# batra-mlp-lab/visdial

Measured on NVIDIA H100. Metric: QA-rounds/sec mn-att-ques-im-hist+disc train step, higher is better.
Workload: dtype f16 operands + f16 saved state for the option LSTM, tf32 operands elsewhere; fp32 accumulate, fp32 cell state / gradients / optimiser

## Files before the change

include/visdial_b200.h:

```cpp
#ifndef VISDIAL_B200_H
#define VISDIAL_B200_H

#include <stddef.h>
#include <stdint.h>

#ifdef __cplusplus
extern "C" {
#endif

#define VD_OK 0
#define VD_E_BADARG (-1)
#define VD_E_SHAPE (-2)
#define VD_E_CUDA (-3)
#define VD_E_COMM (-4)
#define VD_E_OOM (-5)
#define VD_E_STATE (-6)

typedef struct vd_engine vd_engine;

typedef struct vd_params {
  const char* encoder;
  const char* decoder;
  int32_t vocabSize;
  int32_t embedSize;
  int32_t rnnHiddenSize;
  int32_t numLayers;
  int32_t imgFeatureSize;
  int32_t imgSpatialSize;
  int32_t imgEmbedSize;
  int32_t commonEmbeddingSize;
  int32_t numAttentionLayers;
  int32_t maxQuesCount;
  int32_t numOptions;
  float dropout;
  int32_t gpuid;
} vd_params;

typedef struct vd_batch {
  int32_t B;
  int32_t Tq, Th, Ta, To;
  const int32_t* ques_fwd;
  const int32_t* hist;
  const float* img_feat;
  const int32_t* options;
  const int32_t* answer_ind;
  const int32_t* answer_in;
  const int32_t* answer_out;
  const int32_t* option_in;
  const int32_t* option_out;
  int32_t on_device;
} vd_batch;

#define VD_INIT_EMBED 0
#define VD_INIT_LINEAR_W 1
#define VD_INIT_LINEAR_B 2
#define VD_INIT_LSTM_W 3
#define VD_INIT_LSTM_B 4
int vd_layout_count(const vd_params* p, int32_t* n_segments, int64_t* n_params);
int vd_layout_segment(const vd_params* p, int32_t idx, char* name, int32_t name_cap,
                      int64_t* offset, int64_t* rows, int64_t* cols, int32_t* init_kind,
                      int64_t* fan_in);

int vd_create(const vd_params* p, vd_engine** out);
int vd_destroy(vd_engine* e);
const char* vd_last_error(void);

int vd_num_params(vd_engine* e, int64_t* n);
int vd_param_buffers(vd_engine* e, float** W_dev, float** dW_dev);
int vd_optim_buffers(vd_engine* e, float** m_dev, float** v_dev, int64_t* t);
int vd_set_optim_state(vd_engine* e, const float* m_host, const float* v_host, int64_t t);
int vd_set_parameters(vd_engine* e, const float* host_src, int64_t n);
int vd_get_parameters(vd_engine* e, float* host_dst, int64_t n);
int vd_get_gradients(vd_engine* e, float* host_dst, int64_t n);
int vd_zero_grad(vd_engine* e);

int vd_set_training(vd_engine* e, int32_t training);
int vd_set_dropout_seed(vd_engine* e, uint64_t seed, uint64_t iteration);
#define VD_MATH_TF32 0
#define VD_MATH_FP32 1
#define VD_MATH_F16 2
int vd_set_math_mode(vd_engine* e, int32_t mode);
int vd_set_lazy_decout(vd_engine* e, int32_t on);
int vd_set_option_overlap(vd_engine* e, int32_t on, int32_t reserve_sms);

int vd_encoder_forward(vd_engine* e, const vd_batch* b, const float** encOut_dev);
int vd_forward_connect(vd_engine* e);
int vd_decoder_forward(vd_engine* e, const vd_batch* b, const float** decOut_dev);
int vd_criterion_forward(vd_engine* e, const vd_batch* b, float* loss_host);
int vd_criterion_backward(vd_engine* e, const vd_batch* b);
int vd_decoder_backward(vd_engine* e, const vd_batch* b);
int vd_backward_connect(vd_engine* e, const float** gradEncOut_dev);
int vd_encoder_backward(vd_engine* e, const vd_batch* b, const float* gradEncOut_dev);

int vd_forward_backward(vd_engine* e, const vd_batch* b, int32_t only_forward, float* loss_host);
int vd_forward_backward_dense(vd_engine* e, const vd_batch* b, const int32_t* round_host, const float* relevance_host,
                              float* loss_host);
int vd_retrieve(vd_engine* e, const vd_batch* b, int32_t use_gt, int32_t* ranks_host);
int vd_compute_ranks(vd_engine* e, const float* scores_dev, int32_t n_rows,
                     const int32_t* gt_dev_or_null, int32_t* ranks_dev);
int vd_gen_option_lhood(vd_engine* e, const vd_batch* b, const float** lhood_dev);
int vd_encoder_rnn_state(vd_engine* e, int32_t level, const float** h_last_dev, const float** c_last_dev);
int vd_gen_decoder_step(vd_engine* e, int32_t rows, const int32_t* tokens_host, const float* const* h_prev,
                        const float* const* c_prev, const float** logp_dev, const float** h_out, const float** c_out);
int vd_gen_beam_step(vd_engine* e, int32_t rows, const int32_t* tokens_host, const int32_t* parent_host,
                     const float* const* init_h_host, const float* const* init_c_host, int32_t k, float* topv_host,
                     int32_t* topi_host);
int vd_gen_beam_search(vd_engine* e, int32_t beam_size, int32_t beam_len, int32_t start_token, int32_t end_token,
                       int32_t* answer_host, int32_t* length_host, double* score_host);
int vd_gen_sample(vd_engine* e, int32_t beam_len, int32_t start_token, float temperature, uint64_t seed, int64_t row_offset,
                  int32_t* answer_host, float* logp_host);

int vd_clamp_adam_step(vd_engine* e, float learning_rate);

#define VD_COMM_ID_BYTES 128
int vd_comm_unique_id(void* id_out);
int vd_comm_init(vd_engine* e, const void* id, int32_t rank, int32_t world);
int vd_comm_allreduce_grads(vd_engine* e);

int vd_memcpy_d2h(vd_engine* e, void* host_dst, const void* dev_src, size_t bytes);
int vd_memcpy_h2d(vd_engine* e, void* dev_dst, const void* host_src, size_t bytes);
int vd_host_alloc(void** ptr, size_t bytes);
int vd_host_free(void* ptr);
int vd_device_alloc(vd_engine* e, void** ptr, size_t bytes);
int vd_device_free(vd_engine* e, void* ptr);
int vd_synchronize(vd_engine* e);
int vd_stream(vd_engine* e, void** cuda_stream);
int vd_timer_start(vd_engine* e);
int vd_timer_stop(vd_engine* e, float* ms);
int vd_profile_enable(vd_engine* e, int32_t on);
int vd_profile_reset(vd_engine* e);
int vd_launch_count(vd_engine* e, int64_t* n_launches);
int vd_kernel_stats(vd_engine* e, const char* name, int64_t* launches, double* total_ms,
                    double* total_flops, double* total_bytes);
int vd_gemm_tn(vd_engine* e, int32_t M, int32_t N, int32_t K, const float* A, int64_t lda, const float* B, int64_t ldb,
               float* C, int64_t ldc, float beta, const float* bias, int32_t act);
int vd_gemm_atb(vd_engine* e, int32_t M, int32_t N, int64_t K, const float* A, int64_t lda, const float* B, int64_t ldb,
                float* C, int64_t ldc);
int vd_gemm_atb16(vd_engine* e, int32_t M, int32_t N, int64_t K, const float* A, int64_t lda, const float* B, int64_t ldb,
                  float* C, int64_t ldc, float inv_scale);
int vd_lstm_step_fwd(vd_engine* e, int64_t R, int32_t H, const float* h_prev, const float* WhT, int64_t ldw, const float* bias,
                     float* gates, int32_t has_xproj, const float* ptable, int64_t ptable_rows, const int32_t* tok,
                     const float* c_prev, float* c_out, float* h_out, const int32_t* mask_ids, int32_t* path);
int vd_lstm_step_bwd(vd_engine* e, int64_t R, int32_t H, const float* da_next, const float* Wh, const float* gates,
                     const float* c_prev, const float* c_cur, const float* dh_ext, float* dc_carry, const int32_t* mask_ids,
                     float* da, int32_t* path);
int vd_lstm16_step_fwd(vd_engine* e, int64_t R, int32_t H, const void* h_prev16, const void* Wh16, const void* ptable16,
                       const int32_t* tok, const float* bias, const float* c_prev, const int32_t* mask_ids, void* gates16,
                       float* c_out, void* h16_out, float* h32_out);
int vd_lstm16_step_bwd(vd_engine* e, int64_t R, int32_t H, const void* da_next16, const void* Whb16, const void* gates16,
                       const float* c_prev, const float* c_cur, float* dc_carry, const int32_t* mask_ids, void* da16);
int vd_profiler_range(vd_engine* e, int32_t start);
int vd_flush_l2(vd_engine* e);

typedef struct vd_corpus vd_corpus;

typedef struct vd_corpus_desc {
  int32_t numThreads;
  int32_t numRounds;
  int32_t maxQuesLen;
  int32_t maxAnsLen;
  int32_t maxCapLen;
  int32_t numOptions;
  int32_t numOptList;
  int32_t numImages;
  int32_t useHistory;
  int32_t concatHistory;
  int32_t useIm;
  int32_t maxHistoryLen;
  int32_t imgNorm;
  int32_t imgAtt;
  int32_t imgChannels;
  int32_t imgSpatial;
  int32_t startToken, endToken;
  const int32_t* ques;
  const int32_t* ques_len;
  const int32_t* ans;
  const int32_t* ans_len;
  const int32_t* cap;
  const int32_t* cap_len;
  const int32_t* opt;
  const int32_t* opt_list;
  const int32_t* opt_len;
  const int32_t* ans_index;
  const int32_t* img_pos;
  const int32_t* num_rounds;
  const float* images;
} vd_corpus_desc;

int vd_corpus_create(vd_engine* e, const vd_corpus_desc* d, vd_corpus** out);
int vd_corpus_destroy(vd_corpus* c);
int vd_corpus_get_batch(vd_corpus* c, const int64_t* inds, int32_t n, int32_t decoder_gen, vd_batch* out);
int vd_corpus_read(vd_corpus* c, const char* name, void* host_dst, int64_t* elems);
int vd_corpus_batch_bytes(vd_corpus* c, int64_t* bytes, int32_t* launches);

#ifdef __cplusplus
}
#endif
#endif
```

visdial_b200/_lib.py:

```python
from __future__ import annotations

import ctypes as C
import os

_HERE = os.path.dirname(os.path.abspath(__file__))
LIB_PATH = os.path.join(_HERE, "lib", "libvisdial_b200.so")

VD_OK = 0
VD_E_BADARG = -1
VD_E_STATE = -6
VD_MATH_TF32 = 0
VD_MATH_FP32 = 1
VD_MATH_F16 = 2
VD_COMM_ID_BYTES = 128
INIT_EMBED, INIT_LINEAR_W, INIT_LINEAR_B, INIT_LSTM_W, INIT_LSTM_B = range(5)


class VdError(RuntimeError):
    def __init__(self, code, msg):
        super().__init__("visdial_b200 error %d: %s" % (code, msg))
        self.code = code


class vd_params(C.Structure):
    _fields_ = [
        ("encoder", C.c_char_p), ("decoder", C.c_char_p),
        ("vocabSize", C.c_int32), ("embedSize", C.c_int32), ("rnnHiddenSize", C.c_int32),
        ("numLayers", C.c_int32), ("imgFeatureSize", C.c_int32), ("imgSpatialSize", C.c_int32),
        ("imgEmbedSize", C.c_int32), ("commonEmbeddingSize", C.c_int32),
        ("numAttentionLayers", C.c_int32), ("maxQuesCount", C.c_int32), ("numOptions", C.c_int32),
        ("dropout", C.c_float), ("gpuid", C.c_int32),
    ]


class vd_batch(C.Structure):
    _fields_ = [
        ("B", C.c_int32), ("Tq", C.c_int32), ("Th", C.c_int32), ("Ta", C.c_int32), ("To", C.c_int32),
        ("ques_fwd", C.c_void_p), ("hist", C.c_void_p), ("img_feat", C.c_void_p),
        ("options", C.c_void_p), ("answer_ind", C.c_void_p), ("answer_in", C.c_void_p),
        ("answer_out", C.c_void_p), ("option_in", C.c_void_p), ("option_out", C.c_void_p),
        ("on_device", C.c_int32),
    ]


class vd_corpus_desc(C.Structure):
    _fields_ = ([(k, C.c_int32) for k in (
        "numThreads", "numRounds", "maxQuesLen", "maxAnsLen", "maxCapLen", "numOptions", "numOptList", "numImages",
        "useHistory", "concatHistory", "useIm", "maxHistoryLen", "imgNorm", "imgAtt", "imgChannels", "imgSpatial",
        "startToken", "endToken")] +
        [(k, C.c_void_p) for k in (
            "ques", "ques_len", "ans", "ans_len", "cap", "cap_len", "opt", "opt_list", "opt_len", "ans_index",
            "img_pos", "num_rounds", "images")])


_P = C.POINTER
_H = C.c_void_p

SIGNATURES = {
    "vd_layout_count": [_P(vd_params), _P(C.c_int32), _P(C.c_int64)],
    "vd_layout_segment": [_P(vd_params), C.c_int32, C.c_char_p, C.c_int32, _P(C.c_int64), _P(C.c_int64),
                          _P(C.c_int64), _P(C.c_int32), _P(C.c_int64)],
    "vd_create": [_P(vd_params), _P(_H)],
    "vd_destroy": [_H],
    "vd_num_params": [_H, _P(C.c_int64)],
    "vd_param_buffers": [_H, _P(C.c_void_p), _P(C.c_void_p)],
    "vd_optim_buffers": [_H, _P(C.c_void_p), _P(C.c_void_p), _P(C.c_int64)],
    "vd_set_optim_state": [_H, C.c_void_p, C.c_void_p, C.c_int64],
    "vd_set_parameters": [_H, C.c_void_p, C.c_int64],
    "vd_get_parameters": [_H, C.c_void_p, C.c_int64],
    "vd_get_gradients": [_H, C.c_void_p, C.c_int64],
    "vd_zero_grad": [_H],
    "vd_set_training": [_H, C.c_int32],
    "vd_set_dropout_seed": [_H, C.c_uint64, C.c_uint64],
    "vd_set_math_mode": [_H, C.c_int32],
    "vd_set_option_overlap": [_H, C.c_int32, C.c_int32],
    "vd_encoder_forward": [_H, _P(vd_batch), _P(C.c_void_p)],
    "vd_forward_connect": [_H],
    "vd_decoder_forward": [_H, _P(vd_batch), _P(C.c_void_p)],
    "vd_criterion_forward": [_H, _P(vd_batch), _P(C.c_float)],
    "vd_criterion_backward": [_H, _P(vd_batch)],
    "vd_decoder_backward": [_H, _P(vd_batch)],
    "vd_backward_connect": [_H, _P(C.c_void_p)],
    "vd_encoder_backward": [_H, _P(vd_batch), C.c_void_p],
    "vd_forward_backward": [_H, _P(vd_batch), C.c_int32, _P(C.c_float)],
    "vd_forward_backward_dense": [_H, _P(vd_batch), C.c_void_p, C.c_void_p, _P(C.c_float)],
    "vd_retrieve": [_H, _P(vd_batch), C.c_int32, C.c_void_p],
    "vd_compute_ranks": [_H, C.c_void_p, C.c_int32, C.c_void_p, C.c_void_p],
    "vd_gen_option_lhood": [_H, _P(vd_batch), _P(C.c_void_p)],
    "vd_encoder_rnn_state": [_H, C.c_int32, _P(C.c_void_p), _P(C.c_void_p)],
    "vd_gen_decoder_step": [_H, C.c_int32, C.c_void_p, _P(C.c_void_p), _P(C.c_void_p), _P(C.c_void_p), _P(C.c_void_p),
                            _P(C.c_void_p)],
    "vd_clamp_adam_step": [_H, C.c_float],
    "vd_comm_unique_id": [C.c_void_p],
    "vd_comm_init": [_H, C.c_void_p, C.c_int32, C.c_int32],
    "vd_comm_allreduce_grads": [_H],
    "vd_memcpy_d2h": [_H, C.c_void_p, C.c_void_p, C.c_size_t],
    "vd_memcpy_h2d": [_H, C.c_void_p, C.c_void_p, C.c_size_t],
    "vd_host_alloc": [_P(C.c_void_p), C.c_size_t],
    "vd_host_free": [C.c_void_p],
    "vd_device_alloc": [_H, _P(C.c_void_p), C.c_size_t],
    "vd_device_free": [_H, C.c_void_p],
    "vd_synchronize": [_H],
    "vd_stream": [_H, _P(C.c_void_p)],
    "vd_timer_start": [_H],
    "vd_timer_stop": [_H, _P(C.c_float)],
    "vd_profile_enable": [_H, C.c_int32],
    "vd_profile_reset": [_H],
    "vd_launch_count": [_H, _P(C.c_int64)],
    "vd_kernel_stats": [_H, C.c_char_p, _P(C.c_int64), _P(C.c_double), _P(C.c_double), _P(C.c_double)],
    "vd_gemm_tn": [_H, C.c_int32, C.c_int32, C.c_int32, C.c_void_p, C.c_int64, C.c_void_p, C.c_int64, C.c_void_p,
                   C.c_int64, C.c_float, C.c_void_p, C.c_int32],
    "vd_gemm_atb": [_H, C.c_int32, C.c_int32, C.c_int64, C.c_void_p, C.c_int64, C.c_void_p, C.c_int64, C.c_void_p,
                    C.c_int64],
    "vd_set_lazy_decout": [_H, C.c_int32],
    "vd_gen_beam_step": [_H, C.c_int32, C.c_void_p, C.c_void_p, C.c_void_p, C.c_void_p, C.c_int32, C.c_void_p, C.c_void_p],
    "vd_gen_beam_search": [_H, C.c_int32, C.c_int32, C.c_int32, C.c_int32, C.c_void_p, C.c_void_p, C.c_void_p],
    "vd_gen_sample": [_H, C.c_int32, C.c_int32, C.c_float, C.c_uint64, C.c_int64, C.c_void_p, C.c_void_p],
    "vd_gemm_atb16": [_H, C.c_int32, C.c_int32, C.c_int64, C.c_void_p, C.c_int64, C.c_void_p, C.c_int64, C.c_void_p,
                      C.c_int64, C.c_float],
    "vd_lstm_step_fwd": [_H, C.c_int64, C.c_int32, C.c_void_p, C.c_void_p, C.c_int64, C.c_void_p, C.c_void_p, C.c_int32,
                         C.c_void_p, C.c_int64, C.c_void_p, C.c_void_p, C.c_void_p, C.c_void_p, C.c_void_p, _P(C.c_int32)],
    "vd_lstm_step_bwd": [_H, C.c_int64, C.c_int32, C.c_void_p, C.c_void_p, C.c_void_p, C.c_void_p, C.c_void_p, C.c_void_p,
                         C.c_void_p, C.c_void_p, C.c_void_p, _P(C.c_int32)],
    "vd_lstm16_step_fwd": [_H, C.c_int64, C.c_int32] + [C.c_void_p] * 11,
    "vd_lstm16_step_bwd": [_H, C.c_int64, C.c_int32] + [C.c_void_p] * 8,
    "vd_profiler_range": [_H, C.c_int32],
    "vd_flush_l2": [_H],
    "vd_corpus_create": [_H, _P(vd_corpus_desc), _P(C.c_void_p)],
    "vd_corpus_destroy": [C.c_void_p],
    "vd_corpus_get_batch": [C.c_void_p, C.c_void_p, C.c_int32, C.c_int32, _P(vd_batch)],
    "vd_corpus_read": [C.c_void_p, C.c_char_p, C.c_void_p, _P(C.c_int64)],
    "vd_corpus_batch_bytes": [C.c_void_p, _P(C.c_int64), _P(C.c_int32)],
}

_lib = None


def load() -> C.CDLL:
    global _lib
    if _lib is not None:
        return _lib
    if not os.path.exists(LIB_PATH):
        raise VdError(-3, "%s not found: build it with `python __graft_entry__.py` "
                          "(there is no CPU fallback)" % LIB_PATH)
    lib = C.CDLL(LIB_PATH)
    for name, argtypes in SIGNATURES.items():
        fn = getattr(lib, name)
        fn.argtypes = argtypes
        fn.restype = C.c_int
    lib.vd_last_error.argtypes = []
    lib.vd_last_error.restype = C.c_char_p
    _lib = lib
    return lib


def check(rc: int):
    if rc != VD_OK:
        raise VdError(rc, load().vd_last_error().decode("utf-8", "replace"))
```

visdial_b200/csrc/api.cu:

```cuda
#include "engine.h"
#include <string.h>
#include <cuda_profiler_api.h>

namespace vd {
void comm_unique_id(void* out);
void comm_init(Engine* e, const void* idbytes, int rank, int world);
void comm_destroy(Engine* e);
struct Corpus;
Corpus* corpus_create(Engine* eng, const vd_corpus_desc* d);
void corpus_destroy(Corpus* c);
void corpus_get_batch(Corpus* c, const int64_t* inds, int n, int decoder_gen, vd_batch* out);
void corpus_read(Corpus* c, const char* name, void* host_dst, int64_t* elems);
void corpus_batch_bytes(Corpus* c, int64_t* bytes, int32_t* launches);
}

using vd::Engine;

static thread_local char g_err[1024] = "";

static int fail(int code, const char* msg) {
  snprintf(g_err, sizeof(g_err), "%s", msg);
  return code;
}

// ... 3 lines not shown
    return VD_OK;                                               \
  } catch (const vd::CudaError& ex) {                           \
    return fail(ex.code, ex.what());                            \
  } catch (const std::exception& ex) {                          \
    return fail(VD_E_CUDA, ex.what());                          \
  } catch (...) {                                               \
    return fail(VD_E_CUDA, "unknown error");                    \
  }

struct vd_engine { Engine* e; };
#define ENG(h) ((h) ? (h)->e : (throw vd::CudaError(VD_E_BADARG, "engine handle is null"), (Engine*)nullptr))
#define NOTNULL(p) VD_REQUIRE((p) != nullptr, VD_E_BADARG, "null output pointer")

extern "C" {

const char* vd_last_error(void) { return g_err; }

int vd_layout_count(const vd_params* p, int32_t* n_segments, int64_t* n_params) {
  VD_TRY({
    vd::Layout l = vd::build_layout(vd::parse_cfg(p));
    if (n_segments) *n_segments = (int32_t)l.segs.size();
    if (n_params) *n_params = l.total;
  })
}

int vd_layout_segment(const vd_params* p, int32_t idx, char* name, int32_t name_cap, int64_t* offset, int64_t* rows,
                      int64_t* cols, int32_t* init_kind, int64_t* fan_in) {
  VD_TRY({
    vd::Layout l = vd::build_layout(vd::parse_cfg(p));
    VD_REQUIRE(idx >= 0 && idx < (int)l.segs.size(), VD_E_BADARG, "segment index out of range");
    const vd::Seg& s = l.segs[idx];
    if (name && name_cap > 0) snprintf(name, name_cap, "%s", s.name.c_str());
    if (offset) *offset = s.off;
    if (rows) *rows = s.rows;
    if (cols) *cols = s.cols;
    if (init_kind) *init_kind = s.init;
    if (fan_in) *fan_in = s.fan_in;
  })
}

int vd_create(const vd_params* p, vd_engine** out) {
  VD_TRY({
    NOTNULL(out);
    *out = nullptr;
    Engine* e = new Engine(p);
    vd_engine* h = new vd_engine;
    h->e = e;
    *out = h;
  })
}

int vd_destroy(vd_engine* h) {
  VD_TRY({
    if (h) { vd::comm_destroy(h->e); delete h->e; delete h; }
  })
}

int vd_num_params(vd_engine* h, int64_t* n) { VD_TRY({ NOTNULL(n); *n = ENG(h)->nparams; }) }
int vd_param_buffers(vd_engine* h, float** W, float** dW) {
  VD_TRY({ Engine* e = ENG(h); if (W) *W = e->W; if (dW) *dW = e->dW; })
}
int vd_optim_buffers(vd_engine* h, float** m, float** v, int64_t* t) {
  VD_TRY({ Engine* e = ENG(h); if (m) *m = e->m; if (v) *v = e->v; if (t) *t = e->adam_t; })
}
int vd_set_optim_state(vd_engine* h, const float* m_host, const float* v_host, int64_t t) {
  VD_TRY({
    Engine* e = ENG(h);
    VD_REQUIRE(m_host && v_host && t >= 0, VD_E_BADARG, "vd_set_optim_state: m / v null or t < 0");
    VD_CUDA_CHECK(cudaSetDevice(e->cfg.gpuid));
    const size_t bytes = (size_t)e->nparams * sizeof(float);
    VD_CUDA_CHECK(cudaMemcpyAsync(e->m, m_host, bytes, cudaMemcpyHostToDevice, e->cx.stream));
    VD_CUDA_CHECK(cudaMemcpyAsync(e->v, v_host, bytes, cudaMemcpyHostToDevice, e->cx.stream));
    VD_CUDA_CHECK(cudaStreamSynchronize(e->cx.stream));
    e->adam_t = t;
  })
}
int vd_set_parameters(vd_engine* h, const float* src, int64_t n) {
  VD_TRY({
    Engine* e = ENG(h);
    VD_REQUIRE(src && n == e->nparams, VD_E_SHAPE, "vd_set_parameters: n must equal vd_num_params");
    VD_CUDA_CHECK(cudaSetDevice(e->cfg.gpuid));
    VD_CUDA_CHECK(cudaMemcpyAsync(e->W, src, (size_t)n * sizeof(float), cudaMemcpyHostToDevice, e->cx.stream));
    VD_CUDA_CHECK(cudaStreamSynchronize(e->cx.stream));
  })
}
static void copy_out(Engine* e, float* dst, const float* src, int64_t n) {
  VD_REQUIRE(dst && n == e->nparams, VD_E_SHAPE, "n must equal vd_num_params");
  VD_CUDA_CHECK(cudaSetDevice(e->cfg.gpuid));
  e->join_options_backward();
  if (src == e->dW && e->world > 1) {
    bool any = false;
    for (char c : e->seg_reduced) any = any || c;
    if (any) e->reduce_remaining();
  }
  VD_CUDA_CHECK(cudaMemcpyAsync(dst, src, (size_t)n * sizeof(float), cudaMemcpyDeviceToHost, e->cx.stream));
  VD_CUDA_CHECK(cudaStreamSynchronize(e->cx.stream));
}
int vd_get_parameters(vd_engine* h, float* dst, int64_t n) { VD_TRY({ Engine* e = ENG(h); copy_out(e, dst, e->W, n); }) }
int vd_get_gradients(vd_engine* h, float* dst, int64_t n) { VD_TRY({ Engine* e = ENG(h); copy_out(e, dst, e->dW, n); }) }
int vd_zero_grad(vd_engine* h) {
  VD_TRY({
    Engine* e = ENG(h);
    VD_CUDA_CHECK(cudaSetDevice(e->cfg.gpuid));
    e->join_options_backward();
    if (e->comm_pending) e->reduce_remaining();
    VD_CUDA_CHECK(cudaMemsetAsync(e->dW, 0, (size_t)e->nparams * sizeof(float), e->cx.stream));
    e->arm_grad_sync();
  })
}

int vd_set_training(vd_engine* h, int32_t training) {
  VD_TRY({ VD_REQUIRE(training >= 0 && training <= 2, VD_E_BADARG, "training must be 0, 1 or 2"); ENG(h)->training = training; })
}
int vd_set_dropout_seed(vd_engine* h, uint64_t seed, uint64_t iteration) {
  VD_TRY({ Engine* e = ENG(h); e->drop_seed = seed; e->drop_iter = iteration; })
}
int vd_set_option_overlap(vd_engine* h, int32_t on, int32_t reserve_sms) {
  VD_TRY({
    Engine* e = ENG(h);
    e->join_options_backward();
    if (e->opt_fwd_pending) { VD_CUDA_CHECK(cudaStreamSynchronize(e->opt_stream)); e->opt_fwd_pending = false; }
    e->opt_overlap = on != 0;
    if (reserve_sms >= 0) {
      VD_REQUIRE(reserve_sms <= e->cx.sm_count - 16, VD_E_BADARG, "reserve_sms leaves fewer than 16 SMs to the option stream");
      e->opt_reserve_sms = reserve_sms & ~1;
    }
  })
}
int vd_set_math_mode(vd_engine* h, int32_t mode) {
  VD_TRY({ VD_REQUIRE(mode == VD_MATH_TF32 || mode == VD_MATH_FP32 || mode == VD_MATH_F16, VD_E_BADARG, "unknown math mode"); ENG(h)->math_mode = mode; })
}

int vd_encoder_forward(vd_engine* h, const vd_batch* b, const float** encOut) {
  VD_TRY({ Engine* e = ENG(h); e->encoder_forward(b); if (encOut) *encOut = e->encOut; })
}
int vd_forward_connect(vd_engine* h) { VD_TRY({ ENG(h)->forward_connect(); }) }
int vd_decoder_forward(vd_engine* h, const vd_batch* b, const float** decOut) {
  VD_TRY({
    (void)b;
    Engine* e = ENG(h);
    e->decoder_forward();
    if (decOut) *decOut = e->cfg.dec == vd::DEC_DISC ? e->scores : e->logp;
  })
}
int vd_set_lazy_decout(vd_engine* h, int32_t on) { VD_TRY({ ENG(h)->want_logp = on == 0; }) }
int vd_criterion_forward(vd_engine* h, const vd_batch* b, float* loss) {
  VD_TRY({ (void)b; NOTNULL(loss); *loss = ENG(h)->criterion_forward(); })
}
int vd_criterion_backward(vd_engine* h, const vd_batch* b) { VD_TRY({ (void)b; ENG(h)->criterion_backward(); }) }
int vd_decoder_backward(vd_engine* h, const vd_batch* b) { VD_TRY({ (void)b; ENG(h)->decoder_backward(); }) }
int vd_backward_connect(vd_engine* h, const float** gradEncOut) {
  VD_TRY({ const float* g = ENG(h)->backward_connect(); if (gradEncOut) *gradEncOut = g; })
}
int vd_encoder_backward(vd_engine* h, const vd_batch* b, const float* gradEncOut) {
  VD_TRY({ (void)b; ENG(h)->encoder_backward(gradEncOut); })
}

int vd_forward_backward(vd_engine* h, const vd_batch* b, int32_t only_forward, float* loss) {
  VD_TRY({
    Engine* e = ENG(h);
    e->encoder_forward(b);
    e->forward_connect();
    const bool saved_want = e->want_logp;
    e->want_logp = false;
    try { e->decoder_forward(); } catch (...) { e->want_logp = saved_want; throw; }
    e->want_logp = saved_want;
    float l = e->criterion_forward();
    if (loss) *loss = l;
    if (!only_forward) {
      e->criterion_backward();
      e->decoder_backward();
      const float* g = e->backward_connect();
      e->encoder_backward(g);
    }
  })
}

int vd_forward_backward_dense(vd_engine* h, const vd_batch* b, const int32_t* round_host, const float* relevance_host,
                              float* loss_host) {
  VD_TRY({
    const float l = ENG(h)->forward_backward_dense(b, round_host, relevance_host);
    if (loss_host) *loss_host = l;
  })
}

int vd_retrieve(vd_engine* h, const vd_batch* b, int32_t use_gt, int32_t* ranks_host) {
  VD_TRY({ ENG(h)->retrieve(b, use_gt, ranks_host); })
}
int vd_compute_ranks(vd_engine* h, const float* scores_dev, int32_t n_rows, const int32_t* gt_dev, int32_t* ranks_dev) {
  VD_TRY({
    Engine* e = ENG(h);
    VD_REQUIRE(scores_dev && ranks_dev && n_rows >= 0, VD_E_BADARG, "null scores / ranks");
    vd::rank_rows(e->cx, scores_dev, gt_dev, ranks_dev, n_rows, e->cfg.K);
  })
}
int vd_gen_option_lhood(vd_engine* h, const vd_batch* b, const float** lhood_dev) {
  VD_TRY({ (void)b; Engine* e = ENG(h); e->gen_option_lhood(); if (lhood_dev) *lhood_dev = e->lhood; })
}

int vd_encoder_rnn_state(vd_engine* h, int32_t level, const float** h_last, const float** c_last) {
  VD_TRY({
    Engine* e = ENG(h);
    VD_REQUIRE(e->have_fwd, VD_E_STATE, "vd_encoder_rnn_state before vd_encoder_forward");
    VD_REQUIRE(level == 0 || level == 1, VD_E_BADARG, "level must be 0 or 1");
    const bool has_layers = e->cfg.rnn_layers;
    const vd::LstmRun& r = level == 0 ? e->ques1 : e->ques2;
    if (h_last) *h_last = has_layers ? r.h_last() : nullptr;
    if (c_last) *c_last = has_layers ? r.c_last() : nullptr;
  })
}
int vd_gen_decoder_step(vd_engine* h, int32_t rows, const int32_t* tokens_host, const float* const* h_prev,
                        const float* const* c_prev, const float** logp_dev, const float** h_out, const float** c_out) {
  VD_TRY({
    Engine* e = ENG(h);
    e->gen_decoder_step(rows, tokens_host, h_prev, c_prev);
    if (logp_dev) *logp_dev = e->gstep_logp;
    if (h_out) { h_out[0] = e->gstep1.h; h_out[1] = e->gstep2.h; }
    if (c_out) { c_out[0] = e->gstep1.c; c_out[1] = e->gstep2.c; }
  })
}

int vd_gen_beam_step(vd_engine* h, int32_t rows, const int32_t* tokens_host, const int32_t* parent_host,
                     const float* const* init_h_host, const float* const* init_c_host, int32_t k, float* topv_host,
                     int32_t* topi_host) {
  VD_TRY({ ENG(h)->gen_beam_step(rows, tokens_host, parent_host, init_h_host, init_c_host, k, topv_host, topi_host); })
}

int vd_gen_beam_search(vd_engine* h, int32_t beam_size, int32_t beam_len, int32_t start_token, int32_t end_token,
                       int32_t* answer_host, int32_t* length_host, double* score_host) {
  VD_TRY({ ENG(h)->gen_beam_search(beam_size, beam_len, start_token, end_token, answer_host, length_host, score_host); })
}

int vd_gen_sample(vd_engine* h, int32_t beam_len, int32_t start_token, float temperature, uint64_t seed, int64_t row_offset,
                  int32_t* answer_host, float* logp_host) {
  VD_TRY({ ENG(h)->gen_sample(beam_len, start_token, temperature, seed, row_offset, answer_host, logp_host); })
}

int vd_clamp_adam_step(vd_engine* h, float lr) { VD_TRY({ ENG(h)->clamp_adam_step(lr); }) }

int vd_comm_unique_id(void* id_out) { VD_TRY({ NOTNULL(id_out); vd::comm_unique_id(id_out); }) }
int vd_comm_init(vd_engine* h, const void* id, int32_t rank, int32_t world) {
  VD_TRY({ VD_REQUIRE(id != nullptr || world == 1, VD_E_BADARG, "id is null"); vd::comm_init(ENG(h), id, rank, world); })
}
int vd_comm_allreduce_grads(vd_engine* h) { VD_TRY({ ENG(h)->allreduce_grads(); }) }

int vd_memcpy_d2h(vd_engine* h, void* dst, const void* src, size_t bytes) {
  VD_TRY({
    Engine* e = ENG(h);
    VD_REQUIRE(dst && src, VD_E_BADARG, "null pointer");
    VD_CUDA_CHECK(cudaSetDevice(e->cfg.gpuid));
    VD_CUDA_CHECK(cudaMemcpyAsync(dst, src, bytes, cudaMemcpyDeviceToHost, e->cx.stream));
    VD_CUDA_CHECK(cudaStreamSynchronize(e->cx.stream));
  })
}
int vd_memcpy_h2d(vd_engine* h, void* dst, const void* src, size_t bytes) {
  VD_TRY({
    Engine* e = ENG(h);
    VD_REQUIRE(dst && src, VD_E_BADARG, "null pointer");
    VD_CUDA_CHECK(cudaSetDevice(e->cfg.gpuid));
    VD_CUDA_CHECK(cudaMemcpyAsync(dst, src, bytes, cudaMemcpyHostToDevice, e->cx.stream));
    VD_CUDA_CHECK(cudaStreamSynchronize(e->cx.stream));
  })
}
int vd_host_alloc(void** ptr, size_t bytes) {
  VD_TRY({ NOTNULL(ptr); *ptr = nullptr; VD_CUDA_CHECK(cudaHostAlloc(ptr, bytes ? bytes : 1, cudaHostAllocDefault)); })
}
int vd_host_free(void* ptr) { VD_TRY({ if (ptr) VD_CUDA_CHECK(cudaFreeHost(ptr)); }) }
int vd_device_alloc(vd_engine* h, void** ptr, size_t bytes) {
  VD_TRY({
    Engine* e = ENG(h);
    NOTNULL(ptr);
    *ptr = nullptr;
    VD_CUDA_CHECK(cudaSetDevice(e->cfg.gpuid));
    VD_CUDA_CHECK(cudaMalloc(ptr, bytes ? bytes : 1));
  })
}
int vd_device_free(vd_engine* h, void* ptr) {
  VD_TRY({ Engine* e = ENG(h); VD_CUDA_CHECK(cudaSetDevice(e->cfg.gpuid)); if (ptr) VD_CUDA_CHECK(cudaFree(ptr)); })
}
int vd_synchronize(vd_engine* h) {
  VD_TRY({
    Engine* e = ENG(h);
    e->join_options_backward();
    VD_CUDA_CHECK(cudaStreamSynchronize(e->cx.stream));
    if (e->opt_fwd_pending) VD_CUDA_CHECK(cudaStreamSynchronize(e->opt_stream));
  })
}
int vd_stream(vd_engine* h, void** s) { VD_TRY({ NOTNULL(s); *s = (void*)ENG(h)->cx.stream; }) }
int vd_timer_start(vd_engine* h) { VD_TRY({ Engine* e = ENG(h); VD_CUDA_CHECK(cudaEventRecord(e->t0, e->cx.stream)); }) }
int vd_timer_stop(vd_engine* h, float* ms) {
  VD_TRY({
    Engine* e = ENG(h);
    NOTNULL(ms);
    VD_CUDA_CHECK(cudaEventRecord(e->t1, e->cx.stream));
    VD_CUDA_CHECK(cudaEventSynchronize(e->t1));
    VD_CUDA_CHECK(cudaEventElapsedTime(ms, e->t0, e->t1));
  })
}
int vd_profile_enable(vd_engine* h, int32_t on) { VD_TRY({ ENG(h)->cx.profiling = on; }) }
int vd_profile_reset(vd_engine* h) {
  VD_TRY({ Engine* e = ENG(h); e->cx.collect(); e->cx.stats.clear(); e->cx.launches = 0; })
}
int vd_launch_count(vd_engine* h, int64_t* n) { VD_TRY({ NOTNULL(n); *n = ENG(h)->cx.launches; }) }
int vd_kernel_stats(vd_engine* h, const char* name, int64_t* launches, double* total_ms, double* total_flops,
                    double* total_bytes) {
  VD_TRY({
    Engine* e = ENG(h);
    VD_REQUIRE(name != nullptr, VD_E_BADARG, "name is null");
    e->cx.collect();
    auto it = e->cx.stats.find(name);
    vd::KStat z;
    const vd::KStat& s = it == e->cx.stats.end() ? z : it->second;
    if (launches) *launches = s.launches;
    if (total_ms) *total_ms = s.ms;
    if (total_flops) *total_flops = s.flops;
    if (total_bytes) *total_bytes = s.bytes;
  })
}
int vd_gemm_tn(vd_engine* h, int32_t M, int32_t N, int32_t K, const float* A, int64_t lda, const float* B, int64_t ldb,
               float* C, int64_t ldc, float beta, const float* bias, int32_t act) {
  VD_TRY({
    Engine* e = ENG(h);
    VD_REQUIRE(A && B && C, VD_E_BADARG, "null operand");
    VD_CUDA_CHECK(cudaSetDevice(e->cfg.gpuid));
    e->gemm_tn(M, N, K, A, lda, nullptr, B, ldb, C, ldc, beta, bias, act);
  })
}
int vd_gemm_atb(vd_engine* h, int32_t M, int32_t N, int64_t K, const float* A, int64_t lda, const float* B, int64_t ldb,
                float* C, int64_t ldc) {
  VD_TRY({
    Engine* e = ENG(h);
    VD_REQUIRE(A && B && C, VD_E_BADARG, "null operand");
    VD_CUDA_CHECK(cudaSetDevice(e->cfg.gpuid));
    e->gemm_atb(M, N, K, A, lda, nullptr, B, ldb, C, ldc);
  })
}
int vd_gemm_atb16(vd_engine* h, int32_t M, int32_t N, int64_t K, const float* A, int64_t lda, const float* B, int64_t ldb,
                  float* C, int64_t ldc, float inv_scale) {
  VD_TRY({
    Engine* e = ENG(h);
    VD_REQUIRE(A && B && C, VD_E_BADARG, "null operand");
    VD_CUDA_CHECK(cudaSetDevice(e->cfg.gpuid));
    __half* A16 = nullptr; __half* B16 = nullptr; float* sc = nullptr;
    VD_CUDA_CHECK(cudaMalloc((void**)&A16, (size_t)K * M * sizeof(__half)));
    VD_CUDA_CHECK(cudaMalloc((void**)&B16, (size_t)K * N * sizeof(__half)));
    VD_CUDA_CHECK(cudaMalloc((void**)&sc, sizeof(float)));
    VD_CUDA_CHECK(cudaMemcpyAsync(sc, &inv_scale, sizeof(float), cudaMemcpyHostToDevice, e->cx.stream));
    cvt_f32_to_f16(e->cx, A16, M, A, lda, K, M);
    cvt_f32_to_f16(e->cx, B16, N, B, ldb, K, N);
    gemm_atb16(e->cx, M, N, K, A16, M, B16, N, C, ldc, sc);
    VD_CUDA_CHECK(cudaStreamSynchronize(e->cx.stream));
    cudaFree(A16); cudaFree(B16); cudaFree(sc);
  })
}
int vd_lstm_step_fwd(vd_engine* h, int64_t R, int32_t H, const float* h_prev, const float* WhT, int64_t ldw, const float* bias,
                     float* gates, int32_t has_xproj, const float* ptable, int64_t ptable_rows, const int32_t* tok,
                     const float* c_prev, float* c_out, float* h_out, const int32_t* mask_ids, int32_t* path) {
  VD_TRY({
    Engine* e = ENG(h);
    NOTNULL(path);
    VD_REQUIRE(R >= 1 && H > 0 && H % 4 == 0 && WhT && bias && gates && c_out && h_out, VD_E_BADARG, "vd_lstm_step_fwd: arguments");
    VD_REQUIRE((has_xproj != 0) != (ptable != nullptr) && (!ptable || (tok && ptable_rows > 0)), VD_E_BADARG,
               "vd_lstm_step_fwd: the x side is either a dense projection (has_xproj) or a table gather (ptable + tok)");
    VD_CUDA_CHECK(cudaSetDevice(e->cfg.gpuid));
    *path = 0;
    const vd::LstmRoute rt = e->route_lstm(R, H, ptable != nullptr, false, WhT, ldw, nullptr);
    VD_REQUIRE(rt.fwd != vd::LstmPath::Opt16, VD_E_BADARG, "vd_lstm_step_fwd: the fp16 option-LSTM steps (lstm16.cu) have no test hook");
    VD_REQUIRE(rt.fwd == vd::LstmPath::Tc || !ptable, VD_E_BADARG, "vd_lstm_step_fwd: a table gather runs on the tensor-core route only");
    vd::LstmFwdStep s;
    s.R = R; s.H = H; s.WhT = WhT; s.ldw = ldw; s.bias = bias;
    s.h_prev = h_prev; s.c_prev = c_prev; s.gates = gates; s.mask = mask_ids; s.c_out = c_out; s.h_out = h_out;
    float* pt = nullptr;
    if (rt.fwd == vd::LstmPath::Tc) {
      const int64_t n = (ptable ? ptable_rows : R) * 4 * H;
      VD_CUDA_CHECK(cudaMalloc((void**)&pt, (size_t)n * sizeof(float)));
      vd::repeat_rows(e->cx, pt, bias, 1, (int)(n / (4 * H)), 4 * H);
      vd::add_inplace(e->cx, ptable ? pt : gates, ptable ? ptable : pt, n);
      if (ptable) { s.ptable = pt; s.tok = tok; }
    }
    if (rt.fwd == vd::LstmPath::Tc) *path = e->lstm_tc_fwd_step(s); else e->lstm_simt_fwd_step(s);
    VD_CUDA_CHECK(cudaStreamSynchronize(e->cx.stream));
    if (pt) cudaFree(pt);
  })
}

int vd_lstm_step_bwd(vd_engine* h, int64_t R, int32_t H, const float* da_next, const float* Wh, const float* gates,
                     const float* c_prev, const float* c_cur, const float* dh_ext, float* dc_carry, const int32_t* mask_ids,
                     float* da, int32_t* path) {
  VD_TRY({
    Engine* e = ENG(h);
    NOTNULL(path);
    VD_REQUIRE(R >= 1 && H > 0 && Wh && gates && c_cur && dc_carry && da, VD_E_BADARG, "vd_lstm_step_bwd: arguments");
    VD_CUDA_CHECK(cudaSetDevice(e->cfg.gpuid));
    *path = 0;
    const vd::LstmRoute rt = e->route_lstm(R, H, false, false, nullptr, H, Wh);
    vd::LstmBwdStep s;
    s.R = R; s.H = H; s.Wh = Wh; s.da_next = da_next; s.dh_ext = dh_ext;
    s.gates = gates; s.c_prev = c_prev; s.c_cur = c_cur; s.mask = mask_ids; s.dc_carry = dc_carry; s.da = da;
    if (rt.bwd == vd::LstmPath::Simt && da_next) VD_CUDA_CHECK(cudaMalloc((void**)&s.dh_rec, (size_t)R * H * sizeof(float)));
    if (rt.bwd == vd::LstmPath::Tc) *path = e->lstm_tc_bwd_step(s); else e->lstm_simt_bwd_step(s);
    VD_CUDA_CHECK(cudaStreamSynchronize(e->cx.stream));
    if (s.dh_rec) cudaFree(s.dh_rec);
  })
}
int vd_lstm16_step_fwd(vd_engine* h, int64_t R, int32_t H, const void* h_prev16, const void* Wh16, const void* ptable16,
                       const int32_t* tok, const float* bias, const float* c_prev, const int32_t* mask_ids, void* gates16,
                       float* c_out, void* h16_out, float* h32_out) {
  VD_TRY({
    Engine* e = ENG(h);
    VD_REQUIRE(h_prev16 && Wh16 && ptable16 && tok && bias && c_out && h16_out, VD_E_BADARG, "vd_lstm16_step_fwd: arguments");
    VD_REQUIRE(vd::lstm16_shape_ok(R, H), VD_E_BADARG, "vd_lstm16_step_fwd: shape");
    VD_CUDA_CHECK(cudaSetDevice(e->cfg.gpuid));
    vd::lstm16_step_fwd(e->cx, R, H, (const __half*)h_prev16, (const __half*)Wh16, (const __half*)ptable16, tok, bias, c_prev,
                        mask_ids, (__half*)gates16, c_out, (__half*)h16_out, h32_out);
    VD_CUDA_CHECK(cudaStreamSynchronize(e->cx.stream));
  })
}
int vd_lstm16_step_bwd(vd_engine* h, int64_t R, int32_t H, const void* da_next16, const void* Whb16, const void* gates16,
                       const float* c_prev, const float* c_cur, float* dc_carry, const int32_t* mask_ids, void* da16) {
  VD_TRY({
    Engine* e = ENG(h);
    VD_REQUIRE(da_next16 && Whb16 && gates16 && c_cur && dc_carry && da16, VD_E_BADARG, "vd_lstm16_step_bwd: arguments");
    VD_REQUIRE(vd::lstm16_shape_ok(R, H), VD_E_BADARG, "vd_lstm16_step_bwd: shape");
    VD_CUDA_CHECK(cudaSetDevice(e->cfg.gpuid));
    vd::lstm16_step_bwd(e->cx, R, H, (const __half*)da_next16, (const __half*)Whb16, (const __half*)gates16, c_prev, c_cur,
                        dc_carry, mask_ids, (__half*)da16);
    VD_CUDA_CHECK(cudaStreamSynchronize(e->cx.stream));
  })
}

int vd_profiler_range(vd_engine* h, int32_t start) {
  VD_TRY({
    Engine* e = ENG(h);
    VD_CUDA_CHECK(cudaStreamSynchronize(e->cx.stream));
    if (start) VD_CUDA_CHECK(cudaProfilerStart()); else VD_CUDA_CHECK(cudaProfilerStop());
  })
}
int vd_flush_l2(vd_engine* h) {
  VD_TRY({
    Engine* e = ENG(h);
    if (!e->flush_buf) {
      e->flush_n = (int64_t)(192u << 20) / 4;
      VD_CUDA_CHECK(cudaMalloc((void**)&e->flush_buf, (size_t)e->flush_n * 4));
    }
    vd::fill_l2_flush(e->cx, e->flush_buf, e->flush_n);
  })
}

struct vd_corpus { vd::Corpus* c; };
#define CORP(h) ((h) ? (h)->c : (throw vd::CudaError(VD_E_BADARG, "corpus handle is null"), (vd::Corpus*)nullptr))

int vd_corpus_create(vd_engine* h, const vd_corpus_desc* d, vd_corpus** out) {
  VD_TRY({
    NOTNULL(out);
    Engine* e = ENG(h);
    VD_CUDA_CHECK(cudaSetDevice(e->cfg.gpuid));
    vd::Corpus* c = vd::corpus_create(e, d);
    *out = new vd_corpus{c};
  })
}
int vd_corpus_destroy(vd_corpus* h) {
  VD_TRY({
    if (h) { vd::corpus_destroy(h->c); delete h; }
  })
}
int vd_corpus_get_batch(vd_corpus* h, const int64_t* inds, int32_t n, int32_t decoder_gen, vd_batch* out) {
  VD_TRY({ vd::corpus_get_batch(CORP(h), inds, n, decoder_gen, out); })
}
int vd_corpus_read(vd_corpus* h, const char* name, void* host_dst, int64_t* elems) {
  VD_TRY({ vd::corpus_read(CORP(h), name, host_dst, elems); })
}
int vd_corpus_batch_bytes(vd_corpus* h, int64_t* bytes, int32_t* launches) {
  VD_TRY({ vd::corpus_batch_bytes(CORP(h), bytes, launches); })
}

}
```

visdial_b200/csrc/common.cuh:

```cuda
#pragma once
#include <cuda_runtime.h>
#include <stdint.h>
#include <stdio.h>
#include <string.h>
#include <string>
#include <stdexcept>
#include <vector>
#include <map>

namespace vd {

struct CudaError : std::runtime_error {
  int code;
  CudaError(int c, const std::string& m) : std::runtime_error(m), code(c) {}
};

#define VD_CUDA_CHECK(expr)                                                              \
  do {                                                                                   \
    cudaError_t _e = (expr);                                                             \
    if (_e != cudaSuccess) {                                                             \
      char _buf[512];                                                                    \
      snprintf(_buf, sizeof(_buf), "%s:%d: %s -> %s", __FILE__, __LINE__, #expr,         \
               cudaGetErrorString(_e));                                                  \
      throw vd::CudaError(_e == cudaErrorMemoryAllocation ? -5 : -3, _buf);              \
    }                                                                                    \
  } while (0)

#define VD_REQUIRE(cond, code, msg)                                                      \
  do {                                                                                   \
    if (!(cond)) {                                                                       \
      char _buf[512];                                                                    \
      snprintf(_buf, sizeof(_buf), "%s:%d: %s (%s)", __FILE__, __LINE__, msg, #cond);    \
      throw vd::CudaError(code, _buf);                                                   \
    }                                                                                    \
  } while (0)

struct DropCfg {
  uint32_t seed_lo, seed_hi, iter, thresh;
  float scale;
};

__host__ __device__ __forceinline__ void philox4x32_10(uint32_t c0, uint32_t c1, uint32_t c2,
                                                       uint32_t c3, uint32_t k0, uint32_t k1,
                                                       uint32_t out[4]) {
  const uint32_t M0 = 0xD2511F53u, M1 = 0xCD9E8D57u, W0 = 0x9E3779B9u, W1 = 0xBB67AE85u;
#pragma unroll
  for (int r = 0; r < 10; ++r) {
    uint64_t p0 = (uint64_t)M0 * c0, p1 = (uint64_t)M1 * c2;
    uint32_t hi0 = (uint32_t)(p0 >> 32), lo0 = (uint32_t)p0;
    uint32_t hi1 = (uint32_t)(p1 >> 32), lo1 = (uint32_t)p1;
    uint32_t n0 = hi1 ^ c1 ^ k0, n1 = lo1, n2 = hi0 ^ c3 ^ k1, n3 = lo0;
    c0 = n0; c1 = n1; c2 = n2; c3 = n3;
    k0 += W0; k1 += W1;
  }
  out[0] = c0; out[1] = c1; out[2] = c2; out[3] = c3;
}

__device__ __forceinline__ float drop_factor(const DropCfg& d, uint32_t site, uint64_t idx) {
  if (d.thresh == 0) return 1.f;
  uint64_t q = idx >> 2;
  uint32_t o[4];
  philox4x32_10((uint32_t)q, (uint32_t)(q >> 32), site, d.iter, d.seed_lo, d.seed_hi, o);
  return o[idx & 3] >= d.thresh ? d.scale : 0.f;
}
__device__ __forceinline__ void drop_factor4(const DropCfg& d, uint32_t site, uint64_t idx4, float f[4]) {
  if (d.thresh == 0) { f[0] = f[1] = f[2] = f[3] = 1.f; return; }
  uint32_t o[4];
  philox4x32_10((uint32_t)idx4, (uint32_t)(idx4 >> 32), site, d.iter, d.seed_lo, d.seed_hi, o);
#pragma unroll
  for (int i = 0; i < 4; ++i) f[i] = o[i] >= d.thresh ? d.scale : 0.f;
}

enum : uint32_t {
  SITE_QEMBED = 0, SITE_HEMBED = 1, SITE_HATT = 2, SITE_IMG_TR = 3, SITE_U_OUT = 5,
  SITE_FUSION = 6, SITE_IMG_FC7 = 7, SITE_HOP0 = 16,
  SITE_SAMPLE = 64
};

struct SampleCfg {
  uint32_t seed_lo, seed_hi, step;
  float temperature;
  int64_t row_offset;
};
constexpr float GUMBEL_MAX = 17.5f;

__device__ __forceinline__ float gumbel_of_word(uint32_t w) {
  const uint32_t m = w >> 8;
  const float t = m < (1u << 23) ? -logf(((float)m + 0.5f) * 0x1p-24f)
                                 : -log1pf(-(((float)((1u << 24) - m) - 0.5f) * 0x1p-24f));
  return -logf(t);
}
__device__ __forceinline__ void sample_words(const SampleCfg& s, uint64_t q, uint32_t o[4]) {
  philox4x32_10((uint32_t)q, (uint32_t)(q >> 32), SITE_SAMPLE, s.step, s.seed_lo, s.seed_hi, o);
}
__device__ __forceinline__ bool sample_before(float k, int c, float k2, int c2) { return k > k2 || (k == k2 && c < c2); }

struct KStat {
  int64_t launches = 0;
  double flops = 0, bytes = 0;
  std::vector<std::pair<cudaEvent_t, cudaEvent_t>> pending;
  double ms = 0;
};

struct LaunchCtx {
  cudaStream_t stream = nullptr;
  int64_t launches = 0;
  int profiling = 0;
  int sm_count = 132;
  int sm_budget = 0;
  int sms() const { return sm_budget > 0 ? sm_budget : sm_count; }
  std::map<std::string, KStat> stats;
  std::vector<cudaEvent_t> free_events;

  cudaEvent_t get_event() {
    if (!free_events.empty()) { cudaEvent_t e = free_events.back(); free_events.pop_back(); return e; }
    cudaEvent_t e; VD_CUDA_CHECK(cudaEventCreate(&e)); return e;
  }
  struct Scope {
    LaunchCtx* cx; KStat* st; cudaEvent_t a = nullptr, b = nullptr;
    Scope(LaunchCtx* c, const char* name, double flops, double bytes) : cx(c), st(nullptr) {
      if (!cx->profiling) return;
      if (cx->profiling == 2 && strcmp(name, "lstm_step") != 0 && strcmp(name, "lstm_step_bwd") != 0) return;
      st = &cx->stats[name];
      st->launches++; st->flops += flops; st->bytes += bytes;
      a = cx->get_event(); b = cx->get_event();
      cudaEventRecord(a, cx->stream);
    }
    ~Scope() {
      if (!st) return;
      cudaEventRecord(b, cx->stream);
      st->pending.emplace_back(a, b);
    }
  };
  void collect() {
    for (auto& kv : stats) {
      for (auto& p : kv.second.pending) {
        cudaEventSynchronize(p.second);
        float ms = 0; cudaEventElapsedTime(&ms, p.first, p.second);
        kv.second.ms += ms;
        free_events.push_back(p.first); free_events.push_back(p.second);
      }
      kv.second.pending.clear();
    }
  }
};

inline void check_launch(LaunchCtx& cx, const char* what) {
  cx.launches++;
  cudaError_t e = cudaGetLastError();
  if (e != cudaSuccess) {
    char buf[512];
    snprintf(buf, sizeof(buf), "kernel launch failed: %s -> %s", what, cudaGetErrorString(e));
    throw CudaError(-3, buf);
  }
}

static inline int cdiv(int64_t a, int64_t b) { return (int)((a + b - 1) / b); }

}
```

visdial_b200/csrc/enc_lstm.cu:

```cuda
#include <cuda.h>
#include <cuda_fp16.h>
#include "../../include/visdial_b200.h"
#include "kernels.cuh"
#include "tc_ptx.cuh"

namespace vd {
namespace tc {

constexpr int EP_THREADS = 288;
constexpr int EP_STAGES = 5;
constexpr int EP_STAGE_BYTES = 128 * 64 * 2;
constexpr int EP_W_BYTES_MAX = 131072;
constexpr int EP_ACC_BYTES = 32 * ACC_LD * 4;
constexpr int EP_SMEM = EP_W_BYTES_MAX + EP_STAGES * EP_STAGE_BYTES + EP_ACC_BYTES + 1024 + 256;
constexpr int EP_HS = 32;
static_assert(EP_SMEM <= 227 * 1024, "persistent encoder LSTM: shared memory budget");

__device__ __forceinline__ uint32_t ep_pack2(float a, float b) {
  uint32_t r;
  asm("{\n .reg .f16 lo, hi;\n cvt.rn.satfinite.f16.f32 lo, %1;\n cvt.rn.satfinite.f16.f32 hi, %2;\n mov.b32 %0, {lo, hi};\n}"
      : "=r"(r) : "f"(a), "f"(b));
  return r;
}
__device__ __forceinline__ void wait_flag_generic(const int* flag, int want) {
  uint32_t spins = 0;
  for (;;) {
    int v;
    asm volatile("ld.acquire.gpu.global.s32 %0, [%1];" : "=r"(v) : "l"(flag) : "memory");
    if (v >= want) break;
    if (++spins > 64) __nanosleep(40);
    if (spins > (1u << 27)) __trap();
  }
}
__device__ __forceinline__ void wait_flag(const int* flag, int want) {
  wait_flag_generic(flag, want);
  asm volatile("fence.proxy.async;" ::: "memory");
}
constexpr int EP_HW = 16;
__device__ __forceinline__ void ld16g(const float* p, float* d) {
#pragma unroll
  for (int i = 0; i < 4; ++i) {
    const float4 v = *reinterpret_cast<const float4*>(p + 4 * i);
    d[4 * i] = v.x; d[4 * i + 1] = v.y; d[4 * i + 2] = v.z; d[4 * i + 3] = v.w;
  }
}
__device__ __forceinline__ void st16g(float* p, const float* v) {
#pragma unroll
  for (int i = 0; i < 4; ++i) reinterpret_cast<float4*>(p)[i] = make_float4(v[4 * i], v[4 * i + 1], v[4 * i + 2], v[4 * i + 3]);
}
__device__ __forceinline__ void st16h(__half* p, const float* v) {
#pragma unroll
  for (int i = 0; i < 2; ++i)
    reinterpret_cast<uint4*>(p)[i] = make_uint4(ep_pack2(v[8 * i], v[8 * i + 1]), ep_pack2(v[8 * i + 2], v[8 * i + 3]),
                                                ep_pack2(v[8 * i + 4], v[8 * i + 5]), ep_pack2(v[8 * i + 6], v[8 * i + 7]));
}
__device__ __forceinline__ void zero16(float* d) {
#pragma unroll
  for (int e = 0; e < EP_HW; ++e) d[e] = 0.f;
}

enum { EP_CELL1 = 0, EP_PROJ = 1, EP_CELL2 = 2 };

struct EncFwdParams {
  int T, R, H, RB;
  int nS, groups;
  float* gates1; float* c1; float* h1; __half* h1_16;
  float* gates2; float* c2; float* h2; __half* h2_16;
  const float* bias2;
  const int32_t* mask;
  int* flags;
};

struct EpSmem {
  uint8_t* wsm; uint8_t* stages; float* acc; uint64_t* full; uint64_t* empty; uint64_t* wbar;
  __device__ explicit EpSmem(uint8_t* raw) {
    uint8_t* smem = (uint8_t*)(((uintptr_t)raw + 1023) & ~(uintptr_t)1023);
    wsm = smem;
    stages = smem + EP_W_BYTES_MAX;
    acc = (float*)(stages + EP_STAGES * EP_STAGE_BYTES);
    full = (uint64_t*)(stages + EP_STAGES * EP_STAGE_BYTES + EP_ACC_BYTES);
    empty = full + EP_STAGES;
    wbar = empty + EP_STAGES;
  }
  __device__ void init_barriers() {
    for (int s = 0; s < EP_STAGES; ++s) { mbar_init(&full[s], 1); mbar_init(&empty[s], 2); }
    mbar_init(wbar, 1);
    asm volatile("fence.mbarrier_init.release.cluster;" ::: "memory");
  }
};

__device__ __forceinline__ int ep_koff(int role, int slice, int nS, int KB) {
  const int stride = KB >= 2 * nS ? KB / (2 * nS) : 1;
  return ((2 * slice + (role == EP_PROJ ? 1 : 0)) * stride) % KB;
}
template <int N> __device__ __forceinline__ void ep_wgmma(float (&d)[N / 2], uint64_t a, uint64_t b, uint32_t acc) {
  if constexpr (N == 128) wgmma_f16_n128(d, a, b, acc);
  else { static_assert(N == 32, "accumulator width"); wgmma_f16_n32(d, a, b, acc); }
}
template <int N>
__device__ __forceinline__ void ep_mma_step(const EpSmem& sm, float (&d)[N / 2], int wg, int KB, int koff, int& s, uint32_t& ph) {
  int prev = -1;
  for (int kb = 0; kb < KB; ++kb) {
    mbar_wait(&sm.full[s], ph);
    int kr = kb + koff; if (kr >= KB) kr -= KB;
    const uint32_t sa = smem_u32(sm.stages + s * EP_STAGE_BYTES) + wg * 64 * 128;
    const uint32_t sb = smem_u32(sm.wsm + kr * N * 128);
    const uint64_t adesc = make_desc(sa, 16, 1024), bdesc = make_desc(sb, 16, 1024);
    wgmma_fence();
#pragma unroll
    for (int k = 0; k < 4; ++k) ep_wgmma<N>(d, adesc + (uint64_t)(k * 2), bdesc + (uint64_t)(k * 2), (kb | k) ? 1u : 0u);
    wgmma_commit();
    wgmma_wait<1>();
    if (prev >= 0 && (threadIdx.x & 127) == 0) mbar_arrive(&sm.empty[prev]);
    prev = s;
    if (++s == EP_STAGES) { s = 0; ph ^= 1; }
  }
  wgmma_wait<0>();
  wgmma_hold(d);
  if (prev >= 0 && (threadIdx.x & 127) == 0) mbar_arrive(&sm.empty[prev]);
}
template <int NR>
__device__ __forceinline__ void ep_chunk(float* acc, const float (&d)[NR], int wg, int C) {
  bar_named(2 + wg, 128);
  const int lane = threadIdx.x & 31, w = (threadIdx.x >> 5) & 3;
  const int r = wg * 64 + 16 * w + (lane >> 2), c = 2 * (lane & 3);
#pragma unroll
  for (int jj = 0; jj < 4; ++jj) {
    const int j = 4 * C + jj;
    float* p = acc + (c + 8 * jj) * ACC_LD + r;
    p[0] = d[4 * j]; p[ACC_LD] = d[4 * j + 1]; p[8] = d[4 * j + 2]; p[ACC_LD + 8] = d[4 * j + 3];
  }
  bar_named(2 + wg, 128);
}
__device__ __forceinline__ void ep_ld16(const float* arow, float* v) {
#pragma unroll
  for (int e = 0; e < EP_HW; ++e) v[e] = arow[e * ACC_LD];
}

__device__ __forceinline__ void ep_publish(int* flag) {
  bar_named(1, 256);
  if (threadIdx.x == 0) asm volatile("red.release.gpu.global.add.s32 [%0], 1;" ::"l"(flag) : "memory");
}

__global__ void __launch_bounds__(EP_THREADS, 1)
k_enc_pair_fwd(const __grid_constant__ CUtensorMap tmH1, const __grid_constant__ CUtensorMap tmH2,
               const __grid_constant__ CUtensorMap tmW1, const __grid_constant__ CUtensorMap tmW2, const EncFwdParams p) {
  extern __shared__ uint8_t smem_raw[];
  EpSmem sm(smem_raw);
  const int warp = threadIdx.x >> 5, lane = threadIdx.x & 31;
  const int H = p.H, T = p.T;
  const int per_group = 3 * p.nS;
  const int group = blockIdx.x / per_group, idx = blockIdx.x % per_group;
  const int role = idx / p.nS, slice = idx % p.nS;
  constexpr int HS = EP_HS, N = 4 * EP_HS;
  const int KB = H / 64;
  const int koff = ep_koff(role, slice, p.nS, KB);
  int* flagL1 = p.flags;
  int* flagX = p.flags + (size_t)p.RB * T;
  int* flagL2 = p.flags + 2 * (size_t)p.RB * T;

  if (threadIdx.x == 0) sm.init_barriers();
  __syncthreads();

  if (warp == 8) {
    if (lane == 0) {
      const CUtensorMap* tw = role == EP_CELL1 ? &tmW1 : &tmW2;
      const int kofs = role == EP_CELL2 ? H : 0;
      mbar_expect_tx(sm.wbar, (uint32_t)(KB * N * 128));
      for (int kb = 0; kb < KB; ++kb)
        for (int g = 0; g < 4; ++g) tma_load_2d(sm.wsm + kb * N * 128 + g * HS * 128, tw, sm.wbar, kofs + kb * 64, g * H + slice * HS);
      int s = 0; uint32_t ph = 0;
      for (int rb = group; rb < p.RB; rb += p.groups) {
        for (int t = 0; t < T; ++t) {
          const CUtensorMap* tm; int ts;
          if (role == EP_PROJ) { wait_flag(flagL1 + (size_t)rb * T + t, p.nS); tm = &tmH1; ts = t; }
          else {
            if (t == 0) continue;
            wait_flag((role == EP_CELL1 ? flagL1 : flagL2) + (size_t)rb * T + (t - 1), p.nS);
            tm = role == EP_CELL1 ? &tmH1 : &tmH2; ts = t - 1;
          }
          for (int kb = 0; kb < KB; ++kb) {
            int kr = kb + koff; if (kr >= KB) kr -= KB;
            mbar_wait(&sm.empty[s], ph ^ 1);
            mbar_expect_tx(&sm.full[s], EP_STAGE_BYTES);
            tma_load_2d(sm.stages + s * EP_STAGE_BYTES, tm, &sm.full[s], kr * 64, ts * p.R + rb * 128);
            if (++s == EP_STAGES) { s = 0; ph ^= 1; }
          }
        }
      }
    }
  } else if (warp < 8) {
    const int wg = warp >> 2;
    const int hh = (warp >> 1) & 1;
    const int rloc = wg * 64 + (warp & 1) * 32 + lane;
    const float* arow = sm.acc + hh * EP_HW * ACC_LD + rloc;
    const int u0 = slice * HS + hh * EP_HW;
    mbar_wait(sm.wbar, 0);
    int s = 0; uint32_t ph = 0;
    if (role == EP_PROJ) {
      for (int rb = group; rb < p.RB; rb += p.groups) {
        const int64_t row = (int64_t)rb * 128 + rloc;
        const bool row_ok = row < p.R;
        for (int t = 0; t < T; ++t) {
          const int64_t tr = (int64_t)t * p.R + row;
          float d[N / 2];
          ep_mma_step<N>(sm, d, wg, KB, koff, s, ph);
#pragma unroll
          for (int g = 0; g < 4; ++g) {
            ep_chunk(sm.acc, d, wg, g);
            if (row_ok) {
              float a[EP_HW], bb[EP_HW];
              ep_ld16(arow, a);
              ld16g(p.bias2 + g * H + u0, bb);
#pragma unroll
              for (int e = 0; e < EP_HW; ++e) a[e] += bb[e];
              st16g(p.gates2 + tr * 4 * H + g * H + u0, a);
            }
          }
          ep_publish(flagX + (size_t)rb * T + t);
        }
      }
    } else {
      const bool l1 = role == EP_CELL1;
      float* gates = l1 ? p.gates1 : p.gates2;
      float* cst = l1 ? p.c1 : p.c2;
      float* hst = l1 ? p.h1 : p.h2;
      __half* h16 = l1 ? p.h1_16 : p.h2_16;
      int* flag = l1 ? flagL1 : flagL2;
      for (int rb = group; rb < p.RB; rb += p.groups) {
        const int64_t row = (int64_t)rb * 128 + rloc;
        const bool row_ok = row < p.R;
        float c[EP_HW];
        zero16(c);
        for (int t = 0; t < T; ++t) {
          const bool has_acc = t > 0;
          const int64_t tr = (int64_t)t * p.R + row;
          const float keep = (row_ok && p.mask && p.mask[tr] == 0) ? 0.f : 1.f;
          if (!l1 && row_ok) wait_flag_generic(flagX + (size_t)rb * T + t, p.nS);
          float* xrow = gates + tr * 4 * H + u0;
          if (l1 && row_ok && t + 1 < T) {
#pragma unroll
            for (int g = 0; g < 4; ++g) asm volatile("prefetch.global.L2 [%0];" ::"l"(xrow + (int64_t)p.R * 4 * H + g * H) : "memory");
          }
          float d[N / 2];
          if (has_acc) ep_mma_step<N>(sm, d, wg, KB, koff, s, ph);
          float x[EP_HW], a[EP_HW], ig[EP_HW];
          if (has_acc) ep_chunk(sm.acc, d, wg, 0);
          if (row_ok) {
            if (has_acc) ep_ld16(arow, a); else zero16(a);
            ld16g(xrow + 0 * H, x);
#pragma unroll
            for (int e = 0; e < EP_HW; ++e) { a[e] = fsigmoid(a[e] + x[e]) * keep; ig[e] = a[e]; }
            st16g(xrow + 0 * H, a);
          }
          if (has_acc) ep_chunk(sm.acc, d, wg, 3);
          if (row_ok) {
            if (has_acc) ep_ld16(arow, a); else zero16(a);
            ld16g(xrow + 3 * H, x);
#pragma unroll
            for (int e = 0; e < EP_HW; ++e) { a[e] = ftanh(a[e] + x[e]) * keep; ig[e] *= a[e]; }
            st16g(xrow + 3 * H, a);
          }
          if (has_acc) ep_chunk(sm.acc, d, wg, 1);
          if (row_ok) {
            if (has_acc) ep_ld16(arow, a); else zero16(a);
            ld16g(xrow + 1 * H, x);
#pragma unroll
            for (int e = 0; e < EP_HW; ++e) { a[e] = fsigmoid(a[e] + x[e]) * keep; c[e] = (a[e] * c[e] + ig[e]) * keep; }
            st16g(xrow + 1 * H, a);
          }
          if (has_acc) ep_chunk(sm.acc, d, wg, 2);
          if (row_ok) {
            if (has_acc) ep_ld16(arow, a); else zero16(a);
            ld16g(xrow + 2 * H, x);
#pragma unroll
            for (int e = 0; e < EP_HW; ++e) { a[e] = fsigmoid(a[e] + x[e]) * keep; ig[e] = a[e] * ftanh(c[e]) * keep; }
            st16g(xrow + 2 * H, a);
            st16h(h16 + tr * H + u0, ig);
          }
          ep_publish(flag + (size_t)rb * T + t);
          if (row_ok) { st16g(cst + tr * H + u0, c); st16g(hst + tr * H + u0, ig); }
        }
      }
    }
  }
}


struct EncBwdParams {
  int T, R, H, RB;
  int nS, groups;
  const float* gates1; const float* c1; float* da1; __half* da1_16;
  const float* gates2; const float* c2; float* da2; __half* da2_16;
  const float* dh_last1; const float* dc_last1; const float* dh_last2; const float* dc_last2;
  const int32_t* mask;
  int* flags;
  float* dh2; float* dh1;
};

template <bool GS>
__global__ void __launch_bounds__(EP_THREADS, 1)
k_enc_pair_bwd(const __grid_constant__ CUtensorMap tmA1, const __grid_constant__ CUtensorMap tmA2,
               const __grid_constant__ CUtensorMap tmW1, const __grid_constant__ CUtensorMap tmW2, const EncBwdParams p) {
  extern __shared__ uint8_t smem_raw[];
  EpSmem sm(smem_raw);
  const int warp = threadIdx.x >> 5, lane = threadIdx.x & 31;
  const int H = p.H, T = p.T;
  const int per_group = 3 * p.nS;
  const int group = blockIdx.x / per_group, idx = blockIdx.x % per_group;
  const int role = idx / p.nS, slice = idx % p.nS;
  constexpr int HS = EP_HS;
  constexpr int N = GS ? 128 : EP_HS;
  const int nU = H / 128;
  const int gq = GS ? slice / nU : 0, us = GS ? slice % nU : 0;
  const int j0 = GS ? us * 128 + gq * HS : slice * HS;
  const int KB = (GS ? H : 4 * H) / 64;
  const int koff = ep_koff(role, slice, p.nS, KB);
  int* flagT = p.flags;
  int* flagX = p.flags + (size_t)p.RB * T;
  int* flagB = p.flags + 2 * (size_t)p.RB * T;
  int* cntT = p.flags + 3 * (size_t)p.RB * T;
  int* cntB = cntT + (size_t)p.RB * T * nU;

  if (threadIdx.x == 0) sm.init_barriers();
  __syncthreads();

  if (warp == 8) {
    if (lane == 0) {
      const CUtensorMap* tw = role == EP_CELL1 ? &tmW2 : &tmW1;
      const int kofs = role == EP_CELL2 ? 4 * H : 0;
      mbar_expect_tx(sm.wbar, (uint32_t)(KB * N * 128));
      for (int kb = 0; kb < KB; ++kb)
        tma_load_2d(sm.wsm + kb * N * 128, tw, sm.wbar, kofs + (GS ? gq * H : 0) + kb * 64, GS ? us * 128 : slice * HS);
      int s = 0; uint32_t ph = 0;
      for (int rb = group; rb < p.RB; rb += p.groups) {
        for (int t = T - 1; t >= 0; --t) {
          const CUtensorMap* tm; int ts;
          if (role == EP_PROJ) { wait_flag(flagT + (size_t)rb * T + t, p.nS); tm = &tmA2; ts = t; }
          else {
            if (t == T - 1) continue;
            wait_flag((role == EP_CELL1 ? flagT : flagB) + (size_t)rb * T + (t + 1), p.nS);
            tm = role == EP_CELL1 ? &tmA2 : &tmA1; ts = t + 1;
          }
          for (int kb = 0; kb < KB; ++kb) {
            int kr = kb + koff; if (kr >= KB) kr -= KB;
            mbar_wait(&sm.empty[s], ph ^ 1);
            mbar_expect_tx(&sm.full[s], EP_STAGE_BYTES);
            tma_load_2d(sm.stages + s * EP_STAGE_BYTES, tm, &sm.full[s], (GS ? gq * H : 0) + kr * 64, ts * p.R + rb * 128);
            if (++s == EP_STAGES) { s = 0; ph ^= 1; }
          }
        }
      }
    }
  } else if (warp < 8) {
    const int wg = warp >> 2;
    const int hh = (warp >> 1) & 1;
    const int rloc = wg * 64 + (warp & 1) * 32 + lane;
    const float* arow = sm.acc + hh * EP_HW * ACC_LD + rloc;
    const int u0 = j0 + hh * EP_HW;
    mbar_wait(sm.wbar, 0);
    int s = 0; uint32_t ph = 0;
    auto add_partial = [&](const float (&d)[N / 2], float* dhbuf, int* cnt, int rb, int t, int64_t tr, bool row_ok) {
#pragma unroll
      for (int sb = 0; sb < N / 32; ++sb) {
        ep_chunk(sm.acc, d, wg, sb);
        if (row_ok) {
          float a[EP_HW];
          ep_ld16(arow, a);
          float* dst = dhbuf + tr * H + us * 128 + sb * 32 + hh * EP_HW;
#pragma unroll
          for (int e = 0; e < EP_HW; e += 4) red_add_v4(dst + e, a[e], a[e + 1], a[e + 2], a[e + 3]);
        }
      }
      bar_named(1, 256);
      if (threadIdx.x == 0) asm volatile("red.release.gpu.global.add.s32 [%0], 1;" ::"l"(cnt + ((size_t)rb * T + t) * nU + us) : "memory");
    };
    if (role == EP_PROJ) {
      for (int rb = group; rb < p.RB; rb += p.groups) {
        const int64_t row = (int64_t)rb * 128 + rloc;
        const bool row_ok = row < p.R;
        for (int t = T - 1; t >= 0; --t) {
          const int64_t tr = (int64_t)t * p.R + row;
          float d[N / 2];
          ep_mma_step<N>(sm, d, wg, KB, koff, s, ph);
          if constexpr (GS) {
            add_partial(d, p.dh1, cntB, rb, t, tr, row_ok);
          } else {
            ep_chunk(sm.acc, d, wg, 0);
            if (row_ok) { float a[EP_HW]; ep_ld16(arow, a); st16g(p.da1 + tr * 4 * H + u0, a); }
            ep_publish(flagX + (size_t)rb * T + t);
          }
        }
      }
    } else {
      const bool top = role == EP_CELL1;
      const float* gates = top ? p.gates2 : p.gates1;
      const float* cst = top ? p.c2 : p.c1;
      float* da = top ? p.da2 : p.da1;
      __half* da16 = top ? p.da2_16 : p.da1_16;
      const float* dh_last = top ? p.dh_last2 : p.dh_last1;
      const float* dc_last = top ? p.dc_last2 : p.dc_last1;
      int* flag = top ? flagT : flagB;
      float* dhbuf = top ? p.dh2 : p.dh1;
      int* cnt = top ? cntT : cntB;
      for (int rb = group; rb < p.RB; rb += p.groups) {
        const int64_t row = (int64_t)rb * 128 + rloc;
        const bool row_ok = row < p.R;
        float dc[EP_HW];
        zero16(dc);
        for (int t = T - 1; t >= 0; --t) {
          const bool has_acc = t < T - 1;
          const int64_t tr = (int64_t)t * p.R + row;
          const float keep = (row_ok && p.mask && p.mask[tr] == 0) ? 0.f : 1.f;
          const float* grow = gates + tr * 4 * H + u0;
          float* darow = da + tr * 4 * H + u0;
          __half* da16row = da16 + tr * 4 * H + u0;
          float va[EP_HW], vb[EP_HW], dh[EP_HW];
          float d[N / 2];
          if (has_acc) ep_mma_step<N>(sm, d, wg, KB, koff, s, ph);
          if constexpr (GS) {
            if (has_acc) add_partial(d, dhbuf, cnt, rb, t, tr, row_ok);
            const int want = top ? 4 : (has_acc ? 8 : 4);
            if (!row_ok || (top && !has_acc)) zero16(dh);
            else {
              wait_flag_generic(cnt + ((size_t)rb * T + t) * nU + us, want);
              ld16g(dhbuf + tr * H + u0, dh);
            }
          } else {
            if (has_acc) ep_chunk(sm.acc, d, wg, 0);
            if (has_acc && row_ok) ep_ld16(arow, dh); else zero16(dh);
            if (!top && row_ok) {
              wait_flag_generic(flagX + (size_t)rb * T + t, p.nS);
              ld16g(darow, va);
#pragma unroll
              for (int e = 0; e < EP_HW; ++e) dh[e] += va[e];
            }
          }
          if (row_ok) {
            if (t == T - 1) {
              if (dh_last) { ld16g(dh_last + row * H + u0, va);
#pragma unroll
                for (int e = 0; e < EP_HW; ++e) dh[e] += va[e]; }
              if (dc_last) ld16g(dc_last + row * H + u0, dc);
            }
            ld16g(grow + 2 * H, va); ld16g(cst + tr * H + u0, vb);
#pragma unroll
            for (int e = 0; e < EP_HW; ++e) {
              const float tcv = ftanh(vb[e]), go = va[e], dhe = dh[e] * keep;
              dc[e] = (dc[e] + dhe * go * (1.f - tcv * tcv)) * keep;
              dh[e] = dhe * tcv * go * (1.f - go);
            }
            st16h(da16row + 2 * H, dh); st16g(darow + 2 * H, dh);
            ld16g(grow, va); ld16g(grow + 3 * H, vb);
#pragma unroll
            for (int e = 0; e < EP_HW; ++e) dh[e] = dc[e] * vb[e] * va[e] * (1.f - va[e]);
            st16h(da16row, dh); st16g(darow, dh);
#pragma unroll
            for (int e = 0; e < EP_HW; ++e) dh[e] = dc[e] * va[e] * (1.f - vb[e] * vb[e]);
            st16h(da16row + 3 * H, dh); st16g(darow + 3 * H, dh);
            ld16g(grow + 1 * H, va);
            if (t > 0) ld16g(cst + (tr - p.R) * H + u0, vb); else zero16(vb);
#pragma unroll
            for (int e = 0; e < EP_HW; ++e) { dh[e] = dc[e] * vb[e] * va[e] * (1.f - va[e]); dc[e] *= va[e]; }
            st16h(da16row + 1 * H, dh); st16g(darow + 1 * H, dh);
          }
          ep_publish(flag + (size_t)rb * T + t);
        }
      }
    }
  }
}

static CUtensorMap ep_tmap_h(const __half* base, int64_t rows, int64_t cols, int64_t ld, int box_rows) {
  CUtensorMap tm;
  cuuint64_t dims[2] = {(cuuint64_t)cols, (cuuint64_t)rows};
  cuuint64_t strides[1] = {(cuuint64_t)ld * 2};
  cuuint32_t box[2] = {64u, (cuuint32_t)box_rows};
  cuuint32_t estr[2] = {1, 1};
  CUresult r = get_encode()(&tm, CU_TENSOR_MAP_DATA_TYPE_FLOAT16, 2, (void*)base, dims, strides, box, estr, CU_TENSOR_MAP_INTERLEAVE_NONE,
                            CU_TENSOR_MAP_SWIZZLE_128B, CU_TENSOR_MAP_L2_PROMOTION_L2_256B, CU_TENSOR_MAP_FLOAT_OOB_FILL_NONE);
  if (r != CUDA_SUCCESS) {
    char buf[256];
    snprintf(buf, sizeof(buf), "cuTensorMapEncodeTiled (enc_lstm) failed (%d): rows %lld cols %lld ld %lld box %d", (int)r, (long long)rows,
             (long long)cols, (long long)ld, box_rows);
    throw CudaError(-3, buf);
  }
  return tm;
}

}

bool enc_pair_shape_ok(int64_t R, int H, int sm_count) {
  return H % 64 == 0 && H <= 512 && R >= 64 && 3 * (H / 32) <= sm_count;
}

void enc_pair_forward(LaunchCtx& cx, int T, int64_t R, int H, const __half* W1h16, const __half* W2cat16, const float* bias2,
                      const int32_t* mask, float* gates1, float* c1, float* h1, __half* h1_16, float* gates2, float* c2, float* h2,
                      __half* h2_16, int* flags) {
  using namespace tc;
  VD_REQUIRE(enc_pair_shape_ok(R, H, cx.sm_count), VD_E_STATE, "enc_pair_forward: shape");
  EncFwdParams p = {};
  p.T = T; p.R = (int)R; p.H = H; p.RB = cdiv(R, 128);
  p.nS = H / 32;
  p.groups = std::max(1, std::min(p.RB, cx.sm_count / (3 * p.nS)));
  p.gates1 = gates1; p.c1 = c1; p.h1 = h1; p.h1_16 = h1_16;
  p.gates2 = gates2; p.c2 = c2; p.h2 = h2; p.h2_16 = h2_16;
  p.bias2 = bias2; p.mask = mask; p.flags = flags;
  VD_CUDA_CHECK(cudaMemsetAsync(flags, 0, (size_t)3 * p.RB * T * sizeof(int), cx.stream));
  const int64_t TR = (int64_t)T * R;
  CUtensorMap tH1 = ep_tmap_h(h1_16, TR, H, H, 128), tH2 = ep_tmap_h(h2_16, TR, H, H, 128);
  CUtensorMap tW1 = ep_tmap_h(W1h16, 4 * (int64_t)H, H, H, EP_HS), tW2 = ep_tmap_h(W2cat16, 4 * (int64_t)H, 2 * (int64_t)H, 2 * (int64_t)H, EP_HS);
  static bool attr_set = false;
  if (!attr_set) {
    VD_CUDA_CHECK(cudaFuncSetAttribute(k_enc_pair_fwd, cudaFuncAttributeMaxDynamicSharedMemorySize, EP_SMEM));
    attr_set = true;
  }
  k_enc_pair_fwd<<<p.groups * 3 * p.nS, EP_THREADS, EP_SMEM, cx.stream>>>(tH1, tH2, tW1, tW2, p);
  check_launch(cx, "k_enc_pair_fwd");
}


int64_t enc_pair_bwd_flag_ints(int T, int64_t R, int H) { return (int64_t)cdiv(R, 128) * T * (3 + 2 * std::max(1, H / 128)); }
bool enc_pair_gate_split(int H) { return H % 128 == 0; }
void enc_pair_backward(LaunchCtx& cx, int T, int64_t R, int H, const __half* B1cat16, const __half* Whb2_16, const int32_t* mask,
                       const float* gates1, const float* c1, const float* gates2, const float* c2, const float* dh_last1,
                       const float* dc_last1, const float* dh_last2, const float* dc_last2, float* da1, __half* da1_16, float* da2,
                       __half* da2_16, int* flags, float* dh1, float* dh2) {
  using namespace tc;
  VD_REQUIRE(enc_pair_shape_ok(R, H, cx.sm_count), VD_E_STATE, "enc_pair_backward: shape");
  const bool gs = dh1 && dh2 && enc_pair_gate_split(H);
  EncBwdParams p = {};
  p.T = T; p.R = (int)R; p.H = H; p.RB = cdiv(R, 128);
  p.nS = H / 32;
  p.groups = std::max(1, std::min(p.RB, cx.sm_count / (3 * p.nS)));
  p.gates1 = gates1; p.c1 = c1; p.da1 = da1; p.da1_16 = da1_16;
  p.gates2 = gates2; p.c2 = c2; p.da2 = da2; p.da2_16 = da2_16;
  p.dh_last1 = dh_last1; p.dc_last1 = dc_last1; p.dh_last2 = dh_last2; p.dc_last2 = dc_last2;
  p.mask = mask; p.flags = flags; p.dh1 = dh1; p.dh2 = dh2;
  VD_CUDA_CHECK(cudaMemsetAsync(flags, 0, (size_t)enc_pair_bwd_flag_ints(T, R, H) * sizeof(int), cx.stream));
  const int64_t TR = (int64_t)T * R;
  const int64_t G = 4 * (int64_t)H;
  if (gs) {
    VD_CUDA_CHECK(cudaMemsetAsync(dh1, 0, (size_t)TR * H * sizeof(float), cx.stream));
    VD_CUDA_CHECK(cudaMemsetAsync(dh2, 0, (size_t)TR * H * sizeof(float), cx.stream));
  }
  CUtensorMap tA1 = ep_tmap_h(da1_16, TR, G, G, 128), tA2 = ep_tmap_h(da2_16, TR, G, G, 128);
  const int wbox = gs ? 128 : EP_HS;
  CUtensorMap tW1 = ep_tmap_h(B1cat16, H, 2 * G, 2 * G, wbox), tW2 = ep_tmap_h(Whb2_16, H, G, G, wbox);
  static bool attr_set = false;
  if (!attr_set) {
    VD_CUDA_CHECK(cudaFuncSetAttribute(k_enc_pair_bwd<false>, cudaFuncAttributeMaxDynamicSharedMemorySize, EP_SMEM));
    VD_CUDA_CHECK(cudaFuncSetAttribute(k_enc_pair_bwd<true>, cudaFuncAttributeMaxDynamicSharedMemorySize, EP_SMEM));
    attr_set = true;
  }
  if (gs) k_enc_pair_bwd<true><<<p.groups * 3 * p.nS, EP_THREADS, EP_SMEM, cx.stream>>>(tA1, tA2, tW1, tW2, p);
  else k_enc_pair_bwd<false><<<p.groups * 3 * p.nS, EP_THREADS, EP_SMEM, cx.stream>>>(tA1, tA2, tW1, tW2, p);
  check_launch(cx, "k_enc_pair_bwd");
}

}
```

visdial_b200/csrc/engine.cu:

```cuda
#include "engine.h"
#include <string.h>
#include <math.h>
#include <cmath>

namespace vd {

Cfg parse_cfg(const vd_params* p) {
  VD_REQUIRE(p && p->encoder && p->decoder, VD_E_BADARG, "params / encoder / decoder is null");
  Cfg c;
  c.encoder = p->encoder; c.decoder = p->decoder;
  struct { const char* name; int enc; } known[] = {
      {"lf-ques", ENC_LF_QUES}, {"lf-ques-im-hist", ENC_LF_QIH}, {"hrea-ques-im-hist", ENC_HREA}, {"mn-att-ques-im-hist", ENC_MN_ATT},
      {"lf-ques-im", ENC_LF_QI}, {"lf-ques-hist", ENC_LF_QH}, {"hre-ques-hist", ENC_HRE_QH}, {"hre-ques-im-hist", ENC_HRE_QIH},
      {"mn-ques-hist", ENC_MN_QH}, {"mn-ques-im-hist", ENC_MN_QIH}, {"lf-att-ques-im-hist", ENC_LF_ATT}};
  c.enc = -1;
  for (auto& k : known)
    if (c.encoder == k.name) c.enc = k.enc;
  VD_REQUIRE(c.enc >= 0, VD_E_BADARG, "unknown encoder (one of the eleven names of encoders/*.lua)");
  if (c.decoder == "disc") c.dec = DEC_DISC;
  else if (c.decoder == "gen") c.dec = DEC_GEN;
  else VD_REQUIRE(false, VD_E_BADARG, "unknown decoder (disc | gen)");
  c.V = p->vocabSize; c.E = p->embedSize; c.H = p->rnnHiddenSize; c.L = p->numLayers; c.F = p->imgFeatureSize;
  c.S = p->imgSpatialSize; c.IE = p->imgEmbedSize; c.Cm = p->commonEmbeddingSize; c.hops = p->numAttentionLayers;
  c.R = p->maxQuesCount; c.K = p->numOptions; c.dropout = p->dropout; c.gpuid = p->gpuid;
  c.useHist = c.encoder.find("hist") != std::string::npos;
  c.useIm = c.encoder.find("im") != std::string::npos;
  c.att = c.encoder.find("att") != std::string::npos;
  c.fam_lf = c.encoder.compare(0, 3, "lf-") == 0;
  c.fam_hre = c.encoder.compare(0, 3, "hre") == 0;
  c.fam_mn = c.encoder.compare(0, 3, "mn-") == 0;
  c.hre_att = c.enc == ENC_HREA;
  c.san = c.att;
  c.img_in_q = c.fam_hre && c.useIm;
  c.img_drop = c.enc == ENC_HREA;
  c.mn_qi = c.enc == ENC_MN_QIH;
  c.embdrop = c.fam_mn || c.enc == ENC_LF_ATT;
  c.rnn_layers = (c.fam_lf && !c.att) || c.fam_hre;
  if (c.enc == ENC_LF_ATT) c.hops = 1;
  VD_REQUIRE(c.V > 2 && c.E > 0 && c.H > 0, VD_E_BADARG, "vocabSize / embedSize / rnnHiddenSize must be positive");
  VD_REQUIRE(c.L == 2, VD_E_BADARG, "numLayers must be 2");
  VD_REQUIRE(c.E % 4 == 0 && c.H % 32 == 0 && c.IE % 4 == 0 && c.Cm % 4 == 0 && c.F % 4 == 0, VD_E_BADARG,
             "embedSize/imgEmbedSize/commonEmbeddingSize/imgFeatureSize must be multiples of 4, rnnHiddenSize of 32");
  VD_REQUIRE(c.R >= 1 && c.R <= 32 && c.K >= 1 && c.K <= 1024 && c.hops >= 1, VD_E_BADARG, "maxQuesCount/numOptions/numAttentionLayers out of range");
  VD_REQUIRE(c.dropout >= 0.f && c.dropout < 1.f, VD_E_BADARG, "dropout must be in [0,1)");
  return c;
}

int Layout::find(const std::string& name) const {
  for (size_t i = 0; i < segs.size(); ++i)
    if (segs[i].name == name) return (int)i;
  return -1;
}

static void add_seg(Layout& l, const std::string& name, int64_t rows, int64_t cols, int init, int64_t fan_in) {
  Seg s; s.name = name; s.rows = rows; s.cols = cols; s.init = init; s.fan_in = fan_in; s.off = l.total;
  l.segs.push_back(s);
  l.total += (rows * cols + 31) / 32 * 32;
}
static void add_lstm(Layout& l, const std::string& n, int D, int H) {
  add_seg(l, n + ".weight", D + H, 4 * H, VD_INIT_LSTM_W, D + H);
  add_seg(l, n + ".bias", 1, 4 * H, VD_INIT_LSTM_B, D + H);
}
static void add_linear(Layout& l, const std::string& n, int out, int in) {
  add_seg(l, n + ".weight", out, in, VD_INIT_LINEAR_W, in);
  add_seg(l, n + ".bias", 1, out, VD_INIT_LINEAR_B, in);
}

Layout build_layout(const Cfg& c) {
  Layout l;
  add_seg(l, "wordEmbed.weight", c.V + 1, c.E, VD_INIT_EMBED, 0);
  auto add_san = [&]() {
    add_linear(l, "san.img", c.H, c.F);
    for (int h = 1; h <= c.hops; ++h) {
      std::string p = "san.hop" + std::to_string(h) + ".";
      add_linear(l, p + "img_common", c.Cm, c.H);
      add_linear(l, p + "ques_common", c.Cm, c.H);
      add_linear(l, p + "score", 1, c.Cm);
    }
    add_linear(l, "san.out", c.H, c.H);
  };
  if (c.fam_lf && !c.san) {
    add_lstm(l, "ques.lstm1", c.E, c.H); add_lstm(l, "ques.lstm2", c.H, c.H);
    if (c.useHist) { add_lstm(l, "hist.lstm1", c.E, c.H); add_lstm(l, "hist.lstm2", c.H, c.H); }
    add_linear(l, "fusion", c.H, c.H + (c.useIm ? c.F : 0) + (c.useHist ? c.H : 0));
  } else if (c.fam_hre) {
    if (c.img_in_q) add_linear(l, "img.embed", c.IE, c.F);
    add_lstm(l, "hist.lstm1", c.E, c.H); add_lstm(l, "hist.lstm2", c.H, c.H);
    add_lstm(l, "ques.lstm1", c.E + (c.img_in_q ? c.IE : 0), c.H); add_lstm(l, "ques.lstm2", c.H, c.H);
    if (c.hre_att) { add_linear(l, "att.q", 1, c.H); add_linear(l, "att.h", 1, c.H); }
    add_lstm(l, "dialog.lstm", 2 * c.H, c.H);
  } else {
    add_lstm(l, "hist.lstm1", c.E, c.H); add_lstm(l, "hist.lstm2", c.H, c.H);
    add_lstm(l, "ques.lstm1", c.E, c.H); add_lstm(l, "ques.lstm2", c.H, c.H);
    if (c.fam_lf) add_linear(l, "fusion", c.H, 2 * c.H);
    if (c.mn_qi) add_linear(l, "mn.qi", c.H, c.H + c.F);
    if (c.fam_mn) { add_linear(l, "mn.fact", c.H, c.H); add_linear(l, "mn.query", c.H, c.H); }
    if (c.san) add_san();
  }
  if (c.dec == DEC_DISC) {
    add_lstm(l, "opt.lstm", c.E, c.H);
  } else {
    add_lstm(l, "dec.lstm1", c.E, c.H); add_lstm(l, "dec.lstm2", c.H, c.H);
    add_linear(l, "dec.out", c.V, c.H);
  }
  return l;
}

void* Arena::alloc(size_t bytes) {
  bytes = (bytes + 255) & ~(size_t)255;
  if (bytes == 0) bytes = 256;
  while (cur < chunks.size()) {
    Chunk& c = chunks[cur];
    if (c.used + bytes <= c.cap) { void* p = c.p + c.used; c.used += bytes; return p; }
    ++cur;
  }
  Chunk c; c.cap = std::max<size_t>(bytes, (size_t)256 << 20); c.used = bytes;
  VD_CUDA_CHECK(cudaMalloc((void**)&c.p, c.cap));
  chunks.push_back(c);
  cur = chunks.size() - 1;
  return c.p;
}
void Arena::reset() { for (auto& c : chunks) c.used = 0; cur = 0; }
void Arena::release() { for (auto& c : chunks) cudaFree(c.p); chunks.clear(); cur = 0; }
void Arena::rewind(const Mark& m) {
  for (size_t i = m.chunk; i < chunks.size(); ++i) chunks[i].used = i == m.chunk ? m.used : 0;
  cur = m.chunk;
}

void* GrowBuf::ensure(size_t bytes) {
  if (bytes > cap) {
    if (p) cudaFree(p);
    p = nullptr; cap = 0;
    VD_CUDA_CHECK(cudaMalloc(&p, bytes));
    cap = bytes;
  }
  return p;
}
void GrowBuf::release() { if (p) cudaFree(p); p = nullptr; cap = 0; }

Engine::Engine(const vd_params* p) {
  cfg = parse_cfg(p);
  lay = build_layout(cfg);
  nparams = lay.total;
  int ndev = 0;
  VD_CUDA_CHECK(cudaGetDeviceCount(&ndev));
  VD_REQUIRE(cfg.gpuid >= 0 && cfg.gpuid < ndev, VD_E_BADARG, "gpuid out of range");
  VD_CUDA_CHECK(cudaSetDevice(cfg.gpuid));
  cudaDeviceProp prop;
  VD_CUDA_CHECK(cudaGetDeviceProperties(&prop, cfg.gpuid));
  VD_REQUIRE(prop.major == 9 && prop.minor == 0, VD_E_CUDA, "visdial_b200 is built for sm_90a (H100) only");
  cx.sm_count = prop.multiProcessorCount;
  int prio_lo = 0, prio_hi = 0;
  VD_CUDA_CHECK(cudaDeviceGetStreamPriorityRange(&prio_lo, &prio_hi));
  VD_CUDA_CHECK(cudaStreamCreateWithPriority(&cx.stream, cudaStreamNonBlocking, prio_hi));
  main_stream = cx.stream;
  VD_CUDA_CHECK(cudaStreamCreateWithPriority(&side_stream, cudaStreamNonBlocking, prio_hi));
  main_chain.a = main_stream; side_chain.a = side_stream;
  for (cudaStream_t* s : {&main_chain.b, &side_chain.b, &main_chain.c, &side_chain.c})
    VD_CUDA_CHECK(cudaStreamCreateWithPriority(s, cudaStreamNonBlocking, prio_hi));
  VD_CUDA_CHECK(cudaStreamCreateWithPriority(&opt_stream, cudaStreamNonBlocking, prio_lo));
  VD_CUDA_CHECK(cudaEventCreateWithFlags(&ev_fork, cudaEventDisableTiming));
  VD_CUDA_CHECK(cudaEventCreateWithFlags(&ev_join, cudaEventDisableTiming));
  VD_CUDA_CHECK(cudaEventCreateWithFlags(&ev_opt_fork, cudaEventDisableTiming));
  VD_CUDA_CHECK(cudaEventCreateWithFlags(&ev_opt_done, cudaEventDisableTiming));
  size_t bytes = (size_t)nparams * sizeof(float);
  VD_CUDA_CHECK(cudaMalloc((void**)&W, bytes));
  VD_CUDA_CHECK(cudaMalloc((void**)&dW, bytes));
  VD_CUDA_CHECK(cudaMalloc((void**)&m, bytes));
  VD_CUDA_CHECK(cudaMalloc((void**)&v, bytes));
  VD_CUDA_CHECK(cudaMalloc((void**)&Wt, bytes));
  VD_CUDA_CHECK(cudaMemsetAsync(W, 0, bytes, cx.stream));
  VD_CUDA_CHECK(cudaMemsetAsync(dW, 0, bytes, cx.stream));
  VD_CUDA_CHECK(cudaMemsetAsync(m, 0, bytes, cx.stream));
  VD_CUDA_CHECK(cudaMemsetAsync(v, 0, bytes, cx.stream));
  VD_CUDA_CHECK(cudaMemsetAsync(Wt, 0, bytes, cx.stream));
  VD_CUDA_CHECK(cudaMalloc((void**)&scalars_dev, 64 * sizeof(float)));
  std::vector<int64_t> tab;
  for (auto& s : lay.segs) {
    if (s.init == VD_INIT_LSTM_W || s.init == VD_INIT_LINEAR_W) {
      tab.push_back(s.off); tab.push_back(s.rows); tab.push_back(s.cols);
      max2d = std::max(max2d, s.rows * s.cols);
    }
  }
  nseg2d = (int)tab.size() / 3;
  VD_CUDA_CHECK(cudaMalloc((void**)&segtab_dev, tab.size() * sizeof(int64_t)));
  VD_CUDA_CHECK(cudaMemcpyAsync(segtab_dev, tab.data(), tab.size() * sizeof(int64_t), cudaMemcpyHostToDevice, cx.stream));
  VD_CUDA_CHECK(cudaStreamSynchronize(cx.stream));
  VD_CUDA_CHECK(cudaEventCreate(&t0));
  VD_CUDA_CHECK(cudaEventCreate(&t1));
}

Engine::~Engine() {
  cudaSetDevice(cfg.gpuid);
  cudaStreamSynchronize(cx.stream);
  if (opt_stream) cudaStreamSynchronize(opt_stream);
  arena.release();
  for (auto& g : stage) g.release();
  for (auto& g : dense_buf) g.release();
  if (copy_stream) {
    cudaStreamSynchronize(copy_stream); cudaStreamDestroy(copy_stream);
    cudaEventDestroy(ev_img_ready); cudaEventDestroy(ev_copy_fork);
    for (auto ev : ev_img_free) cudaEventDestroy(ev);
  }
  for (auto& g : stage_img) g.release();
  cudaFree(W); cudaFree(dW); cudaFree(m); cudaFree(v); cudaFree(Wt); cudaFree(scalars_dev); cudaFree(segtab_dev);
  if (flush_buf) cudaFree(flush_buf);
  cx.collect();
  for (auto e : cx.free_events) cudaEventDestroy(e);
  if (t0) cudaEventDestroy(t0);
  if (t1) cudaEventDestroy(t1);
  if (ev_fork) cudaEventDestroy(ev_fork);
  if (ev_join) cudaEventDestroy(ev_join);
  if (side_stream) { cudaStreamSynchronize(side_stream); cudaStreamDestroy(side_stream); }
  for (cudaStream_t s : {main_chain.b, side_chain.b, main_chain.c, side_chain.c})
    if (s) { cudaStreamSynchronize(s); cudaStreamDestroy(s); }
  if (opt_stream) { cudaStreamSynchronize(opt_stream); cudaStreamDestroy(opt_stream); }
  if (ev_opt_fork) cudaEventDestroy(ev_opt_fork);
  if (ev_opt_done) cudaEventDestroy(ev_opt_done);
  for (auto e : ev_pool) cudaEventDestroy(e);
  cudaStreamDestroy(main_stream);
}

int Engine::seg(const char* name) const {
  int i = lay.find(name);
  VD_REQUIRE(i >= 0, VD_E_STATE, name);
  return i;
}

DropCfg Engine::dropcfg(float p) const {
  DropCfg d;
  d.seed_lo = (uint32_t)drop_seed; d.seed_hi = (uint32_t)(drop_seed >> 32); d.iter = (uint32_t)drop_iter;
  if (training == 1 && p > 0.f) {
    double t = (double)p * 4294967296.0;
    d.thresh = (uint32_t)std::min(t, 4294967295.0);
    d.scale = 1.f / (1.f - p);
  } else { d.thresh = 0; d.scale = 1.f; }
  return d;
}

void Engine::gemm_tn(int M, int N, int K, const float* A, int64_t lda, const int32_t* gather, const float* B, int64_t ldb,
                     float* C, int64_t ldc, float beta, const float* bias, int act) {
  LaunchCtx::Scope sc(&cx, "gemm", 2.0 * M * N * K, 4.0 * ((double)M * K + (double)N * K + (double)M * N));
  if (tcmode() && gemm_tn_tc(cx, M, N, K, A, lda, gather, B, ldb, C, ldc, beta, bias, act)) return;
  gemm_tn_simt(cx, M, N, K, A, lda, gather, B, ldb, C, ldc, beta, bias, act);
}
void Engine::gemm_atb(int M, int N, int64_t K, const float* A, int64_t lda, const int32_t* gather, const float* B,
                      int64_t ldb, float* C, int64_t ldc) {
  LaunchCtx::Scope sc(&cx, "gemm_wgrad", 2.0 * M * N * K, 4.0 * ((double)M * K + (double)N * K + (double)M * N));
  if (tcmode() && gemm_atb_tc(cx, M, N, K, A, lda, gather, B, ldb, C, ldc)) return;
  gemm_atb_simt(cx, M, N, K, A, lda, gather, B, ldb, C, ldc);
}

void Engine::linear_fwd(int wseg, const float* x, int64_t rows, float* y, int act) {
  const Seg& s = lay.segs[wseg];
  gemm_tn((int)rows, (int)s.rows, (int)s.cols, x, s.cols, nullptr, Wp(wseg), s.cols, y, s.rows, 0.f, Wp(wseg + 1), act);
}
void Engine::linear_bwd(int wseg, const float* x, const float* dy, int64_t rows, float* dx, float beta_dx) {
  const Seg& s = lay.segs[wseg];
  int out = (int)s.rows, in = (int)s.cols;
  gemm_atb(out, in, rows, dy, out, nullptr, x, in, dWp(wseg), in);
  colsum_add(cx, dWp(wseg + 1), dy, rows, out, out);
  if (dx) gemm_tn((int)rows, in, out, dy, out, nullptr, Wtp(wseg), out, dx, in, beta_dx, nullptr, 0);
}

void Engine::refresh_shadows() {
  VD_CUDA_CHECK(cudaMemsetAsync(W, 0, (size_t)cfg.E * sizeof(float), cx.stream));
  transpose_segments(cx, W, Wt, segtab_dev, nseg2d, max2d);
}

void Engine::stage_batch(const vd_batch* b) {
  VD_REQUIRE(b != nullptr, VD_E_BADARG, "batch is null");
  VD_REQUIRE(b->B > 0, VD_E_SHAPE, "batch B must be > 0");
  db = DevBatch();
  db.B = b->B; db.N = (int64_t)b->B * cfg.R;
  db.Tq = b->Tq; db.Th = b->Th; db.Ta = b->Ta; db.To = b->To;
  VD_REQUIRE(b->ques_fwd && b->Tq > 0, VD_E_SHAPE, "ques_fwd / Tq missing");
  if (cfg.useHist) VD_REQUIRE(b->hist && b->Th > 0, VD_E_SHAPE, "encoder uses history: hist / Th missing");
  if (cfg.useIm) VD_REQUIRE(b->img_feat, VD_E_SHAPE, "encoder uses the image: img_feat missing");
  int64_t img_elems = cfg.att ? (int64_t)b->B * cfg.S * cfg.S * cfg.F : (int64_t)b->B * cfg.F;
  struct Item { const void* src; size_t bytes; const void** dst; } items[9] = {
      {b->ques_fwd, (size_t)db.N * b->Tq * 4, (const void**)&db.ques},
      {cfg.useHist ? b->hist : nullptr, (size_t)db.N * b->Th * 4, (const void**)&db.hist},
      {cfg.useIm ? b->img_feat : nullptr, (size_t)img_elems * 4, (const void**)&db.img},
      {b->options, (size_t)db.N * cfg.K * b->To * 4, (const void**)&db.options},
      {b->answer_ind, (size_t)db.N * 4, (const void**)&db.answer_ind},
      {b->answer_in, (size_t)db.N * b->Ta * 4, (const void**)&db.answer_in},
      {b->answer_out, (size_t)db.N * b->Ta * 4, (const void**)&db.answer_out},
      {b->option_in, (size_t)db.N * cfg.K * b->To * 4, (const void**)&db.option_in},
      {b->option_out, (size_t)db.N * cfg.K * b->To * 4, (const void**)&db.option_out}};
  img_copy_pending = false;
  for (int i = 0; i < 9; ++i) {
    if (!items[i].src || items[i].bytes == 0) { *items[i].dst = nullptr; continue; }
    if (b->on_device) { *items[i].dst = items[i].src; continue; }
    if (i == 2 && items[i].bytes >= ((size_t)1 << 20)) {
      if (!copy_stream) {
        VD_CUDA_CHECK(cudaStreamCreateWithFlags(&copy_stream, cudaStreamNonBlocking));
        VD_CUDA_CHECK(cudaEventCreateWithFlags(&ev_img_ready, cudaEventDisableTiming));
        VD_CUDA_CHECK(cudaEventCreateWithFlags(&ev_copy_fork, cudaEventDisableTiming));
        for (int k = 0; k < 2; ++k) VD_CUDA_CHECK(cudaEventCreateWithFlags(&ev_img_free[k], cudaEventDisableTiming));
      }
      img_slot ^= 1;
      if (items[i].bytes > stage_img[img_slot].cap) VD_CUDA_CHECK(cudaStreamSynchronize(copy_stream));
      void* d = stage_img[img_slot].ensure(items[i].bytes);
      VD_CUDA_CHECK(cudaEventRecord(ev_copy_fork, cx.stream));
      VD_CUDA_CHECK(cudaStreamWaitEvent(copy_stream, ev_copy_fork, 0));
      if (img_free_recorded[img_slot]) VD_CUDA_CHECK(cudaStreamWaitEvent(copy_stream, ev_img_free[img_slot], 0));
      VD_CUDA_CHECK(cudaMemcpyAsync(d, items[i].src, items[i].bytes, cudaMemcpyHostToDevice, copy_stream));
      VD_CUDA_CHECK(cudaEventRecord(ev_img_ready, copy_stream));
      img_copy_pending = true;
      *items[i].dst = d;
      continue;
    }
    void* d = stage[i].ensure(items[i].bytes);
    VD_CUDA_CHECK(cudaMemcpyAsync(d, items[i].src, items[i].bytes, cudaMemcpyHostToDevice, cx.stream));
    *items[i].dst = d;
  }
}

void Engine::wait_img() {
  if (!img_copy_pending) return;
  VD_CUDA_CHECK(cudaStreamWaitEvent(cx.stream, ev_img_ready, 0));
  if (cx.stream != main_stream) VD_CUDA_CHECK(cudaStreamWaitEvent(main_stream, ev_img_ready, 0));
  img_copy_pending = false;
}
void Engine::release_img() {
  if (!copy_stream || !db.img || db.img != stage_img[img_slot].p) return;
  VD_CUDA_CHECK(cudaEventRecord(ev_img_free[img_slot], cx.stream));
  img_free_recorded[img_slot] = true;
}

constexpr int64_t kWavefrontMinRows = 64;

LstmRoute Engine::route_lstm(int64_t R, int H, bool gathered, bool has_h0, const float* WhT, int64_t ldw, const float* Wh) const {
  LstmRoute rt;
  if (math_mode == VD_MATH_F16 && gathered && !has_h0 && lstm16_shape_ok(R, H)) {
    rt.fwd = rt.bwd = LstmPath::Opt16;
  } else {
    rt.fwd = tcmode() && lstm_step_fwd_tc_ok(H, WhT, ldw) ? LstmPath::Tc : LstmPath::Simt;
    rt.bwd = tcmode() && lstm_step_bwd_tc_ok(H, Wh) ? LstmPath::Tc : LstmPath::Simt;
  }
  rt.table_grad = gathered && tcmode();
  return rt;
}

void Engine::route_lstm_pair(LstmRun& l1, LstmRun& l2) const {
  if (math_mode == VD_MATH_F16 && !l1.h0 && !l1.c0 && !l2.h0 && !l2.c0 && !l1.gather && l1.x && l1.H == l2.H &&
      l2.D == l1.H && l1.R == l2.R && l1.T == l2.T && l1.mask == l2.mask && enc_pair_shape_ok(l1.R, l1.H, cx.sm_count)) {
    l1.route = l2.route = LstmRoute();
    l1.route.fwd = l1.route.bwd = l2.route.fwd = l2.route.bwd = LstmPath::Pair16;
    return;
  }
  l1.route = route_lstm(l1);
  l2.route = route_lstm(l2);
  l1.route.wave_fwd = l2.route.wave_fwd = l2.route.fwd == LstmPath::Tc && l2.R >= kWavefrontMinRows;
  l1.route.wave_bwd = l2.route.wave_bwd = l1.route.bwd == LstmPath::Tc && l2.route.bwd == LstmPath::Tc && l2.R >= kWavefrontMinRows;
}

void Engine::lstm_simt_fwd_step(const LstmFwdStep& s) {
  const int G = 4 * s.H;
  if (s.h_prev) gemm_tn((int)s.R, G, s.H, s.h_prev, s.H, nullptr, s.WhT, s.ldw, s.gates, G, 1.f, nullptr, 0);
  lstm_pointwise_fwd(cx, s.gates, s.bias, s.c_prev, s.mask, s.c_out, s.h_out, s.R, s.H);
}

int Engine::lstm_tc_fwd_step(const LstmFwdStep& s) {
  if (!s.h_prev) {
    lstm_first_step_fwd(cx, s.gates, s.ptable, s.tok, nullptr, s.c_prev, s.mask, s.c_out, s.h_out, s.R, s.H);
    return 0;
  }
  int tile = 0;
  const bool ok = lstm_step_fwd_tc(cx, s.R, s.H, s.h_prev, s.WhT, s.ldw, nullptr, s.gates, s.ptable == nullptr, s.ptable, s.tok,
                                   s.c_prev, s.c_out, s.h_out, s.mask, &tile);
  VD_REQUIRE(ok, VD_E_STATE, "lstm_step_fwd_tc refused a shape the engine routed to it");
  return tile;
}

void Engine::lstm_simt_bwd_step(const LstmBwdStep& s) {
  const int G = 4 * s.H;
  if (s.da_next) gemm_tn((int)s.R, s.H, G, s.da_next, G, nullptr, s.Wh, G, s.dh_rec, s.H, 0.f, nullptr, 0);
  lstm_pointwise_bwd(cx, s.gates, s.c_prev, s.c_cur, s.da_next ? s.dh_rec : s.dh_last, s.dh_ext, nullptr, s.dc_carry, s.mask, s.da,
                     s.R, s.H);
}

int Engine::lstm_tc_bwd_step(const LstmBwdStep& s) {
  if (!s.da_next) { lstm_simt_bwd_step(s); return 0; }
  int tile = 0;
  const bool ok = lstm_step_bwd_tc(cx, s.R, s.H, s.da_next, s.Wh, s.gates, s.c_prev, s.c_cur, s.dh_ext, s.dc_carry, s.mask,
                                   s.da, &tile);
  VD_REQUIRE(ok, VD_E_STATE, "lstm_step_bwd_tc refused a shape the engine routed to it");
  return tile;
}

void Engine::lstm_xproj(const LstmRun& r, int t0, int nt, float* gates) {
  const int64_t off = (int64_t)t0 * r.R;
  gemm_tn((int)(nt * r.R), 4 * r.H, r.D, r.x ? r.x + off * r.D : Wp(0), r.x ? r.D : cfg.E, r.gather ? r.gather + off : nullptr,
          Wtp(r.wseg), r.D + r.H, gates, 4 * r.H, 0.f, r.route.fwd == LstmPath::Simt ? nullptr : Wp(r.wseg + 1), 0);
}

void Engine::lstm_forward_begin(LstmRun& r, bool save, bool xproj_by_caller) {
  const Seg& ws = lay.segs[r.wseg];
  VD_REQUIRE(ws.rows == r.D + r.H && ws.cols == 4 * r.H, VD_E_STATE, "lstm weight shape");
  VD_REQUIRE(!r.gather || r.D == cfg.E, VD_E_STATE, "gathered LSTM input must be the word embedding");
  const int H = r.H, D = r.D, G = 4 * r.H;
  const int64_t R = r.R;
  const float* WtS = Wtp(r.wseg);
  r.saved = save;
  r.ptable = nullptr;
  if (r.route.fwd == LstmPath::Opt16) {
    float* pt = arena.get<float>((int64_t)(cfg.V + 1) * G);
    gemm_tn(cfg.V + 1, G, D, Wp(0), cfg.E, nullptr, WtS, D + H, pt, G, 0.f, nullptr, 0);
    r.P16 = arena.get<__half>((int64_t)(cfg.V + 1) * G);
    cvt_f32_to_f16(cx, r.P16, G, pt, G, cfg.V + 1, G);
    r.Wh16 = arena.get<__half>((int64_t)G * H);
    cvt_f32_to_f16(cx, r.Wh16, H, WtS + D, D + H, G, H);
    r.Whb16 = nullptr;
    if (save) {
      r.Whb16 = arena.get<__half>((int64_t)H * G);
      cvt_f32_to_f16(cx, r.Whb16, G, Wp(r.wseg) + (int64_t)D * G, G, H, G);
    }
    const int64_t slots = save ? r.T : 2;
    r.h16 = arena.get<__half>(slots * R * H);
    r.c = arena.get<float>(slots * R * H);
    r.gates16 = save ? arena.get<__half>((int64_t)r.T * R * G) : nullptr;
    r.h32_last = arena.get<float>(R * H);
    r.h = nullptr; r.gates = nullptr;
    return;
  }
  if (r.route.fwd == LstmPath::Tc && r.gather) {
    float* pt = arena.get<float>((int64_t)(cfg.V + 1) * G);
    gemm_tn(cfg.V + 1, G, D, Wp(0), cfg.E, nullptr, WtS, D + H, pt, G, 0.f, Wp(r.wseg + 1), 0);
    r.ptable = pt;
  }
  const int64_t slots = save ? r.T : 2;
  r.h = arena.get<float>(slots * R * H);
  r.c = arena.get<float>(slots * R * H);
  r.gates = arena.get<float>((save ? r.T : 1) * R * G);
  if (save && !r.ptable && !xproj_by_caller) lstm_xproj(r, 0, r.T, r.gates);
}

void Engine::lstm_forward_step(LstmRun& r, int t, bool xproj_by_caller) {
  const int H = r.H, G = 4 * r.H;
  const int64_t R = r.R, RH = R * H;
  const int64_t slot = r.saved ? t : (t & 1), pslot = r.saved ? t - 1 : ((t - 1) & 1);
  const float* bias = Wp(r.wseg + 1);
  const float* cp = t > 0 ? r.c + pslot * RH : r.c0;
  const int32_t* mk = r.mask ? r.mask + (int64_t)t * R : nullptr;
  if (r.route.fwd == LstmPath::Opt16) {
    __half* g16 = r.saved ? r.gates16 + (int64_t)t * R * G : nullptr;
    const int32_t* tok = r.gather + (int64_t)t * R;
    float* h32 = t == r.T - 1 ? r.h32_last : nullptr;
    if (t == 0) {
      LaunchCtx::Scope sc(&cx, "lstm_step_first", 0.0, R * (2.0 * G + 2.0 * G + 6.0 * H));
      lstm16_first_step(cx, R, H, r.P16, tok, bias, cp, mk, g16, r.c + slot * RH, r.h16 + slot * RH, h32);
    } else {
      LaunchCtx::Scope sc(&cx, "lstm_step", 2.0 * R * G * H, R * (2.0 * G + 4.0 * H + 4.0 * H + 2.0 * H + 2.0 * H));
      lstm16_step_fwd(cx, R, H, r.h16 + pslot * RH, r.Wh16, r.P16, tok, bias, cp, mk, g16, r.c + slot * RH, r.h16 + slot * RH, h32);
    }
    return;
  }
  LstmFwdStep s;
  s.R = R; s.H = H; s.WhT = Wtp(r.wseg) + r.D; s.ldw = r.D + H; s.bias = bias; s.c_prev = cp; s.mask = mk;
  s.h_prev = t > 0 ? r.h + pslot * RH : r.h0;
  s.gates = r.saved ? r.gates + (int64_t)t * R * G : r.ptable ? nullptr : r.gates;
  if (r.ptable) { s.ptable = r.ptable; s.tok = r.gather + (int64_t)t * R; }
  s.c_out = r.c + slot * RH; s.h_out = r.h + slot * RH;
  const bool tc = r.route.fwd == LstmPath::Tc;
  const bool x_per_step = !r.ptable && (!r.saved || xproj_by_caller);
  const bool first_no_rec = tc && !s.h_prev;
  LaunchCtx::Scope sc(&cx, first_no_rec ? "lstm_step_first" : (R >= 4096 ? "lstm_step" : "lstm_step_small"),
                      first_no_rec ? 0.0 : 2.0 * R * G * (H + (x_per_step ? r.D : 0)), 4.0 * R * (G + 4.0 * H));
  if (x_per_step && !r.saved) lstm_xproj(r, t, 1, s.gates);
  if (tc) lstm_tc_fwd_step(s); else lstm_simt_fwd_step(s);
}

void Engine::lstm_forward(LstmRun& r, bool save) {
  r.route = route_lstm(r);
  lstm_forward_begin(r, save);
  for (int t = 0; t < r.T; ++t) lstm_forward_step(r, t);
}

cudaEvent_t Engine::pool_event(size_t i) {
  while (ev_pool.size() <= i) {
    cudaEvent_t e;
    VD_CUDA_CHECK(cudaEventCreateWithFlags(&e, cudaEventDisableTiming));
    ev_pool.push_back(e);
  }
  return ev_pool[i];
}

void Engine::lstm_pair_forward(LstmRun& l1, LstmRun& l2, const PairStreams& s) {
  cx.stream = s.a;
  if (l1.route.fwd == LstmPath::Pair16) {
    const int H = l1.H, G = 4 * H, T = l1.T;
    const int64_t R = l1.R;
    lstm_forward_begin(l1, true);
    l2.x = l1.h;
    lstm_forward_begin(l2, true, true);
    l1.h16 = arena.get<__half>((int64_t)T * R * H);
    l2.h16 = arena.get<__half>((int64_t)T * R * H);
    l2.x16 = l1.h16;
    __half* W1h = arena.get<__half>((int64_t)G * H);
    __half* W2c = arena.get<__half>((int64_t)G * 2 * H);
    cvt_f32_to_f16(cx, W1h, H, Wtp(l1.wseg) + l1.D, l1.D + H, G, H);
    cvt_f32_to_f16(cx, W2c, 2 * H, Wtp(l2.wseg), 2 * H, G, 2 * H);
    int* flags = arena.get<int>(3 * (int64_t)cdiv(R, 128) * T);
    LaunchCtx::Scope sc2(&cx, "enc_pair_fwd", 2.0 * T * R * G * 3.0 * H, 4.0 * T * R * (2.0 * G + 2.0 * G + 6.0 * H));
    enc_pair_forward(cx, T, R, H, W1h, W2c, Wp(l2.wseg + 1), l1.mask, l1.gates, l1.c, l1.h, l1.h16, l2.gates, l2.c, l2.h, l2.h16, flags);
    return;
  }
  if (!l1.route.wave_fwd) {
    lstm_forward_begin(l1, true);
    for (int t = 0; t < l1.T; ++t) lstm_forward_step(l1, t);
    l2.x = l1.h;
    lstm_forward_begin(l2, true);
    for (int t = 0; t < l2.T; ++t) lstm_forward_step(l2, t);
    return;
  }
  lstm_forward_begin(l1, true);
  l2.x = l1.h;
  cudaEvent_t e0 = pool_event(0);
  VD_CUDA_CHECK(cudaEventRecord(e0, s.a));
  VD_CUDA_CHECK(cudaStreamWaitEvent(s.b, e0, 0));
  cx.stream = s.b;
  lstm_forward_begin(l2, true, true);
  for (int t = 0; t < l1.T; ++t) {
    cx.stream = s.a;
    lstm_forward_step(l1, t);
    cudaEvent_t e = pool_event(1 + t);
    VD_CUDA_CHECK(cudaEventRecord(e, s.a));
    VD_CUDA_CHECK(cudaStreamWaitEvent(s.c, e, 0));
    if (t == 0) VD_CUDA_CHECK(cudaStreamWaitEvent(s.c, e0, 0));
    cx.stream = s.c;
    lstm_xproj(l2, t, 1, l2.gates + (int64_t)t * l2.R * 4 * l2.H);
    cudaEvent_t ex = pool_event(1 + l1.T + t);
    VD_CUDA_CHECK(cudaEventRecord(ex, s.c));
    VD_CUDA_CHECK(cudaStreamWaitEvent(s.b, ex, 0));
    cx.stream = s.b;
    lstm_forward_step(l2, t, true);
  }
  VD_CUDA_CHECK(cudaEventRecord(e0, s.b));
  VD_CUDA_CHECK(cudaStreamWaitEvent(s.a, e0, 0));
  cx.stream = s.a;
}

void Engine::lstm_backward_begin(LstmRun& r, const float* dh_all, const float* dh_last, const float* dc_last) {
  VD_REQUIRE(r.saved, VD_E_STATE, "lstm_backward needs a forward run in training mode");
  const int H = r.H, G = 4 * r.H;
  const int64_t R = r.R, TR = (int64_t)r.T * R;
  r.dc_carry = arena.get<float>(R * H);
  r.bw_dh_all = dh_all; r.bw_dh_last = dh_last;
  if (r.route.bwd == LstmPath::Opt16) {
    VD_REQUIRE(dh_last && !dh_all && !dc_last, VD_E_STATE, "fp16 BPTT takes its gradient from the last step only");
    r.da16 = arena.get<__half>(TR * G);
    r.scale2 = arena.get<float>(4);
    pick_grad_scale(cx, dh_last, R * H, reinterpret_cast<uint32_t*>(r.scale2 + 2), r.scale2);
    return;
  }
  r.da = arena.get<float>(TR * G);
  r.dh_rec = arena.get<float>(R * H);
  if (dc_last)
    VD_CUDA_CHECK(cudaMemcpyAsync(r.dc_carry, dc_last, (size_t)R * H * sizeof(float), cudaMemcpyDeviceToDevice, cx.stream));
  else
    VD_CUDA_CHECK(cudaMemsetAsync(r.dc_carry, 0, (size_t)R * H * sizeof(float), cx.stream));
}

void Engine::lstm_backward_step(LstmRun& r, int t) {
  const int H = r.H, G = 4 * r.H;
  const int64_t R = r.R, RH = R * H, RG = R * G;
  const bool last = t == r.T - 1;
  const float* cp = t > 0 ? r.c + (t - 1) * RH : r.c0;
  const int32_t* mk = r.mask ? r.mask + (int64_t)t * R : nullptr;
  if (r.route.bwd == LstmPath::Opt16) {
    const __half* g16 = r.gates16 + t * RG;
    __half* da16_t = r.da16 + t * RG;
    if (last) {
      LaunchCtx::Scope sc(&cx, "lstm_step_bwd_last", 0.0, R * (2.0 * G + 2.0 * G + 16.0 * H));
      lstm16_bwd_last(cx, R, H, g16, cp, r.c + t * RH, r.bw_dh_last, r.scale2, mk, r.dc_carry, da16_t);
    } else {
      LaunchCtx::Scope sc(&cx, "lstm_step_bwd", 2.0 * R * G * H, R * (3.0 * 2.0 * G + 16.0 * H));
      lstm16_step_bwd(cx, R, H, r.da16 + (t + 1) * RG, r.Whb16, g16, cp, r.c + t * RH, r.dc_carry, mk, da16_t);
    }
    return;
  }
  LstmBwdStep s;
  s.R = R; s.H = H; s.Wh = Wp(r.wseg) + (int64_t)r.D * G; s.dc_carry = r.dc_carry; s.dh_rec = r.dh_rec; s.mask = mk;
  s.da_next = last ? nullptr : r.da + (t + 1) * RG; s.dh_last = last ? r.bw_dh_last : nullptr;
  s.dh_ext = r.bw_dh_all ? r.bw_dh_all + t * RH : nullptr;
  s.gates = r.gates + t * RG; s.c_prev = cp; s.c_cur = r.c + t * RH; s.da = r.da + t * RG;
  const bool tc = r.route.bwd == LstmPath::Tc;
  LaunchCtx::Scope sc(&cx, (last && tc) ? "lstm_step_bwd_last" : (R >= 4096 ? "lstm_step_bwd" : "lstm_step_bwd_small"),
                      last ? 0.0 : 2.0 * R * G * H, 4.0 * R * (2.0 * G + 5.0 * H));
  if (tc) lstm_tc_bwd_step(s); else lstm_simt_bwd_step(s);
}

void Engine::lstm_backward_end(LstmRun& r, float* dx_out, float* dh0_out, float* dc0_out) {
  const int H = r.H, D = r.D, G = 4 * r.H;
  const int64_t R = r.R, TR = (int64_t)r.T * R;
  const float* Ws = Wp(r.wseg);
  float* dWs = dWp(r.wseg);
  const bool opt16 = r.route.bwd == LstmPath::Opt16;
  if (opt16) VD_REQUIRE(!dh0_out && !dc0_out && !dx_out && !r.h0, VD_E_STATE, "fp16 BPTT: no initial-state / input gradients");
  if (dh0_out) gemm_tn((int)R, H, G, r.da, G, nullptr, Ws + (int64_t)D * G, G, dh0_out, H, 0.f, nullptr, 0);
  if (dc0_out) VD_CUDA_CHECK(cudaMemcpyAsync(dc0_out, r.dc_carry, (size_t)R * H * sizeof(float), cudaMemcpyDeviceToDevice, cx.stream));
  const bool wgrad16 = opt16 || (r.route.bwd == LstmPath::Pair16 && TR - R >= 256);
  if (r.T > 1) {
    if (wgrad16) {
      LaunchCtx::Scope sc(&cx, "gemm_wgrad", 2.0 * H * G * (double)(TR - R), 2.0 * (double)(TR - R) * (H + G));
      gemm_atb16(cx, H, G, TR - R, r.h16, H, r.da16 + R * G, G, dWs + (int64_t)D * G, G, opt16 ? r.scale2 + 1 : nullptr);
    } else gemm_atb(H, G, TR - R, r.h, H, nullptr, r.da + R * G, G, dWs + (int64_t)D * G, G);
  }
  if (r.h0) gemm_atb(H, G, R, r.h0, H, nullptr, r.da, G, dWs + (int64_t)D * G, G);
  if (r.route.table_grad) {
    VD_REQUIRE(dx_out == nullptr, VD_E_STATE, "projected-space embedding gradient: caller must not ask for dx");
    const int V1 = cfg.V + 1;
    float* dP = arena.get<float>((int64_t)V1 * G);
    VD_CUDA_CHECK(cudaMemsetAsync(dP, 0, (size_t)V1 * G * sizeof(float), cx.stream));
    int32_t* scratch = arena.get<int32_t>(3 * (int64_t)V1);
    int32_t* perm = arena.get<int32_t>(TR);
    int32_t* stok = arena.get<int32_t>(TR);
    {
      LaunchCtx::Scope sc(&cx, "embed_grad_segsum", 0.0, (opt16 ? 2.0 : 4.0) * TR * G);
      group_rows_by_token(cx, r.gather, TR, V1, scratch, perm, stok);
      if (opt16) segsum_rows16(cx, r.da16, G, perm, stok, TR, dP, G, r.scale2 + 1);
      else segsum_rows(cx, r.da, G, perm, stok, TR, dP, G);
    }
    gemm_atb(D, G, V1, Wp(0), cfg.E, nullptr, dP, G, dWs, G);
    colsum_add(cx, dWp(r.wseg + 1), dP, V1, G, G);
    if (r.demb_out) gemm_tn(V1, D, G, dP, G, nullptr, Ws, G, r.demb_out, cfg.E, 0.f, nullptr, 0);
    else gemm_tn(V1, D, G, dP, G, nullptr, Ws, G, dWp(0), cfg.E, 1.f, nullptr, 0);
    return;
  }
  if (wgrad16 && r.x16) {
    LaunchCtx::Scope sc(&cx, "gemm_wgrad", 2.0 * D * G * (double)TR, 2.0 * (double)TR * (D + G));
    gemm_atb16(cx, D, G, TR, r.x16, D, r.da16, G, dWs, G, nullptr);
  } else gemm_atb(D, G, TR, r.x ? r.x : Wp(0), r.x ? D : cfg.E, r.gather, r.da, G, dWs, G);
  colsum_add(cx, dWp(r.wseg + 1), r.da, TR, G, G);
  if (dx_out) gemm_tn((int)TR, D, G, r.da, G, nullptr, Ws, G, dx_out, D, 0.f, nullptr, 0);
}

void Engine::lstm_backward(LstmRun& r, const float* dh_all, const float* dh_last, const float* dc_last, float* dx_out,
                           float* dh0_out, float* dc0_out) {
  lstm_backward_begin(r, dh_all, dh_last, dc_last);
  for (int t = r.T - 1; t >= 0; --t) lstm_backward_step(r, t);
  lstm_backward_end(r, dx_out, dh0_out, dc0_out);
}

void Engine::lstm_pair_backward(LstmRun& l1, LstmRun& l2, const float* dh_last2, const float* dc_last2, const float* dh_last1,
                                const float* dc_last1, float* dx1_out, const PairStreams& s) {
  const int H = l2.H, G = 4 * l2.H;
  const int64_t R = l2.R;
  cx.stream = s.a;
  if (l1.route.bwd == LstmPath::Pair16) {
    const int T = l2.T;
    const int64_t TR = (int64_t)T * R;
    l1.da = arena.get<float>(TR * G); l2.da = arena.get<float>(TR * G);
    l1.da16 = arena.get<__half>(TR * G); l2.da16 = arena.get<__half>(TR * G);
    __half* Whb2 = arena.get<__half>((int64_t)H * G);
    __half* B1cat = arena.get<__half>((int64_t)H * 2 * G);
    cvt_f32_to_f16(cx, Whb2, G, Wp(l2.wseg) + (int64_t)l2.D * G, G, H, G);
    cvt_f32_to_f16(cx, B1cat, 2 * G, Wp(l2.wseg), G, H, G);
    cvt_f32_to_f16(cx, B1cat + G, 2 * G, Wp(l1.wseg) + (int64_t)l1.D * G, G, H, G);
    int* flags = arena.get<int>(enc_pair_bwd_flag_ints(T, R, H));
    float* dh1 = nullptr; float* dh2 = nullptr;
    if (enc_pair_gate_split(H)) { dh1 = arena.get<float>(TR * H); dh2 = arena.get<float>(TR * H); }
    {
      LaunchCtx::Scope sc2(&cx, "enc_pair_bwd", 2.0 * T * R * (double)H * 3.0 * G, 4.0 * T * R * (4.0 * G + 4.0 * H));
      enc_pair_backward(cx, T, R, H, B1cat, Whb2, l1.mask, l1.gates, l1.c, l2.gates, l2.c, dh_last1, dc_last1, dh_last2, dc_last2,
                        l1.da, l1.da16, l2.da, l2.da16, flags, dh1, dh2);
    }
    lstm_backward_end(l2, nullptr, nullptr, nullptr);
    lstm_backward_end(l1, dx1_out, nullptr, nullptr);
    return;
  }
  float* dx2 = arena.get<float>((int64_t)l2.T * R * l2.D);
  if (!l1.route.wave_bwd) {
    lstm_backward(l2, nullptr, dh_last2, dc_last2, dx2, nullptr, nullptr);
    lstm_backward(l1, dx2, dh_last1, dc_last1, dx1_out, nullptr, nullptr);
    return;
  }
  const float* Wx2 = Wp(l2.wseg);
  cudaEvent_t e0 = pool_event(0);
  VD_CUDA_CHECK(cudaEventRecord(e0, s.a));
  VD_CUDA_CHECK(cudaStreamWaitEvent(s.b, e0, 0));
  cx.stream = s.b;
  lstm_backward_begin(l2, nullptr, dh_last2, dc_last2);
  cx.stream = s.a;
  lstm_backward_begin(l1, dx2, dh_last1, dc_last1);
  for (int t = l2.T - 1; t >= 0; --t) {
    cx.stream = s.b;
    lstm_backward_step(l2, t);
    cudaEvent_t e = pool_event(1 + t);
    VD_CUDA_CHECK(cudaEventRecord(e, s.b));
    VD_CUDA_CHECK(cudaStreamWaitEvent(s.c, e, 0));
    cx.stream = s.c;
    gemm_tn((int)R, l2.D, G, l2.da + (int64_t)t * R * G, G, nullptr, Wx2, G, dx2 + (int64_t)t * R * l2.D, l2.D, 0.f, nullptr, 0);
    cudaEvent_t ex = pool_event(1 + l2.T + t);
    VD_CUDA_CHECK(cudaEventRecord(ex, s.c));
    VD_CUDA_CHECK(cudaStreamWaitEvent(s.a, ex, 0));
    cx.stream = s.a;
    lstm_backward_step(l1, t);
  }
  cx.stream = s.b;
  lstm_backward_end(l2, nullptr, nullptr, nullptr);
  VD_CUDA_CHECK(cudaEventRecord(e0, s.b));
  cx.stream = s.a;
  lstm_backward_end(l1, dx1_out, nullptr, nullptr);
  VD_CUDA_CHECK(cudaStreamWaitEvent(s.a, e0, 0));
}

static LstmRun make_run(int T, int64_t R, int D, int H, int wseg, const float* x, const int32_t* gather, const int32_t* mask) {
  LstmRun r; r.T = T; r.R = R; r.D = D; r.H = H; r.wseg = wseg; r.x = x; r.gather = gather; r.mask = mask;
  return r;
}

void Engine::mn_block_fwd(const float* qin, const float* h3, float* out) {
  const int H = cfg.H, R = cfg.R, B = db.B;
  const int64_t N = db.N;
  const DropCfg d05 = dropcfg(0.5f);
  probs = arena.get<float>((int64_t)B * R * R);
  hAtt = arena.get<float>(N * H);
  mn_attention_fwd(cx, qin, h3, probs, hAtt, B, R, H);
  hAtt_d = arena.get<float>(N * H);
  dropout_apply(cx, hAtt_d, hAtt, N * H, d05, SITE_HATT);
  hAttTr = arena.get<float>(N * H);
  linear_fwd(seg("mn.fact.weight"), hAtt_d, N, hAttTr, 1);
  sum1 = arena.get<float>(N * H);
  add_out(cx, sum1, hAttTr, qin, N * H);
  linear_fwd(seg("mn.query.weight"), sum1, N, out, 1);
}
void Engine::mn_block_bwd(const float* dout, const float* out, float* dqin, float* dh3) {
  const int H = cfg.H, R = cfg.R, B = db.B;
  const int64_t N = db.N;
  const DropCfg d05 = dropcfg(0.5f);
  float* dpre = arena.get<float>(N * H);
  tanh_bwd(cx, dpre, dout, out, N * H);
  float* dsum1 = arena.get<float>(N * H);
  linear_bwd(seg("mn.query.weight"), sum1, dpre, N, dsum1, 0.f);
  tanh_bwd(cx, dpre, dsum1, hAttTr, N * H);
  float* dhAtt = arena.get<float>(N * H);
  linear_bwd(seg("mn.fact.weight"), hAtt_d, dpre, N, dhAtt, 0.f);
  dropout_apply(cx, dhAtt, dhAtt, N * H, d05, SITE_HATT);
  mn_attention_bwd(cx, mn_query_in, hist2.h_last(), probs, dhAtt, dqin, dh3, B, R, H);
  add_inplace(cx, dqin, dsum1, N * H);
}
void Engine::san_block_fwd(const float* u0) {
  const int H = cfg.H, R = cfg.R, B = db.B;
  const int64_t N = db.N;
  const int P = cfg.S * cfg.S, Cm = cfg.Cm;
  const DropCfg d05 = dropcfg(0.5f);
  t_img = arena.get<float>((int64_t)B * P * H);
  wait_img();
  linear_fwd(seg("san.img.weight"), db.img, (int64_t)B * P, t_img, 1);
  img_tr = arena.get<float>(N * P * H);
  san_expand_dropout(cx, img_tr, t_img, B, R, P, H, d05, SITE_IMG_TR);
  img_common.assign(cfg.hops, nullptr); ques_common.assign(cfg.hops, nullptr);
  sc.assign(cfg.hops, nullptr); pr.assign(cfg.hops, nullptr); u_hop.assign(cfg.hops + 1, nullptr);
  u_hop[0] = const_cast<float*>(u0);
  for (int hop = 0; hop < cfg.hops; ++hop) {
    std::string pre = "san.hop" + std::to_string(hop + 1) + ".";
    int w_ic = seg((pre + "img_common.weight").c_str()), w_qc = seg((pre + "ques_common.weight").c_str()),
        w_s = seg((pre + "score.weight").c_str());
    img_common[hop] = arena.get<float>(N * P * Cm);
    linear_fwd(w_ic, img_tr, N * P, img_common[hop], 0);
    ques_common[hop] = arena.get<float>(N * Cm);
    linear_fwd(w_qc, u_hop[hop], N, ques_common[hop], 0);
    sc[hop] = arena.get<float>(N * P);
    san_score_fwd(cx, img_common[hop], ques_common[hop], Wp(w_s), Wp(w_s + 1), sc[hop], N, P, Cm, d05, SITE_HOP0 + hop);
    pr[hop] = arena.get<float>(N * P);
    u_hop[hop + 1] = arena.get<float>(N * H);
    san_softmax_att_fwd(cx, sc[hop], pr[hop], img_tr, u_hop[hop], u_hop[hop + 1], N, P, H);
  }
  u_d = arena.get<float>(N * H);
  dropout_apply(cx, u_d, u_hop[cfg.hops], N * H, d05, SITE_U_OUT);
  linear_fwd(seg("san.out.weight"), u_d, N, encOut, 1);
}
void Engine::san_block_bwd(const float* dEnc, float* du) {
  const int H = cfg.H, R = cfg.R, B = db.B;
  const int64_t N = db.N;
  const int P = cfg.S * cfg.S, Cm = cfg.Cm;
  const DropCfg d05 = dropcfg(0.5f);
  float* dpre = arena.get<float>(N * H);
  tanh_bwd(cx, dpre, dEnc, encOut, N * H);
  linear_bwd(seg("san.out.weight"), u_d, dpre, N, du, 0.f);
  dropout_apply(cx, du, du, N * H, d05, SITE_U_OUT);
  float* dimg_tr = arena.get<float>(N * P * H);
  float* ds = arena.get<float>(N * P);
  float* dic = arena.get<float>(N * P * Cm);
  float* dqc = arena.get<float>(N * Cm);
  for (int hop = cfg.hops - 1; hop >= 0; --hop) {
    std::string pre = "san.hop" + std::to_string(hop + 1) + ".";
    int w_ic = seg((pre + "img_common.weight").c_str()), w_qc = seg((pre + "ques_common.weight").c_str()),
        w_s = seg((pre + "score.weight").c_str());
    if (hop == cfg.hops - 1) {
      san_att_bwd(cx, du, pr[hop], img_tr, ds, dimg_tr, N, P, H);
    } else {
      float* tmp = arena.get<float>(N * P * H);
      san_att_bwd(cx, du, pr[hop], img_tr, ds, tmp, N, P, H);
      add_inplace(cx, dimg_tr, tmp, N * P * H);
    }
    san_score_bwd(cx, ds, img_common[hop], ques_common[hop], Wp(w_s), dic, dqc, dWp(w_s), dWp(w_s + 1), N, P, Cm, d05,
                  SITE_HOP0 + hop);
    linear_bwd(w_ic, img_tr, dic, N * P, dimg_tr, 1.f);
    linear_bwd(w_qc, u_hop[hop], dqc, N, du, 1.f);
  }
  float* dt_pre = arena.get<float>((int64_t)B * P * H);
  san_collapse_bwd(cx, dimg_tr, t_img, dt_pre, B, R, P, H, d05, SITE_IMG_TR);
  linear_bwd(seg("san.img.weight"), db.img, dt_pre, (int64_t)B * P, nullptr, 0.f);
  release_img();
// ... 766 lines not shown
```

visdial_b200/csrc/kernels.cuh:

```cuda
#pragma once
#include <algorithm>
#include <cuda_fp16.h>
#include "common.cuh"

namespace vd {

void gemm_tn_simt(LaunchCtx& cx, int M, int N, int K, const float* A, int64_t lda, const int32_t* a_gather,
                  const float* B, int64_t ldb, float* C, int64_t ldc, float beta, const float* bias, int act);
void gemm_atb_simt(LaunchCtx& cx, int M, int N, int64_t K, const float* A, int64_t lda, const int32_t* a_gather,
                   const float* B, int64_t ldb, float* C, int64_t ldc);
bool gemm_tn_tc(LaunchCtx& cx, int M, int N, int K, const float* A, int64_t lda, const int32_t* a_gather,
                const float* B, int64_t ldb, float* C, int64_t ldc, float beta, const float* bias, int act);
bool gemm_atb_tc(LaunchCtx& cx, int M, int N, int64_t K, const float* A, int64_t lda, const int32_t* a_gather,
                 const float* B, int64_t ldb, float* C, int64_t ldc);

int vocab_lse_nparts(int N);
bool vocab_tc_ok(int M, int N, int K, const float* A, int64_t lda, const float* B, int64_t ldb);
bool vocab_lse_tc(LaunchCtx& cx, int M, int N, int K, const float* A, int64_t lda, const float* B, int64_t ldb, const float* bias,
                  const int32_t* tgt, float* part_max, float* part_sum, float* tgt_logit);
bool vocab_dlogits_tc(LaunchCtx& cx, int M, int N, int K, const float* A, int64_t lda, const float* B, int64_t ldb, const float* bias,
                      const int32_t* tgt, const int32_t* row_ids, const float* lse, float* C, int64_t ldc);
void vocab_lse_finish(LaunchCtx& cx, const float* part_max, const float* part_sum, int nparts, const float* tgt_logit,
                      const int32_t* tgt, const int32_t* row_ids, float* lse, float* out, float sign, int accumulate, int64_t rows);
bool vocab_sample_tc(LaunchCtx& cx, int M, int N, int K, const float* A, int64_t lda, const float* B, int64_t ldb, const float* bias,
                     const SampleCfg& smp, float* part_max, float* part_sum, float* part_key, int32_t* part_cls, float* part_x);
void vocab_sample_finish(LaunchCtx& cx, const float* part_max, const float* part_sum, const float* part_key, const int32_t* part_cls,
                         const float* part_x, int nparts, int64_t rows, int step, int L, int32_t* tokens, int32_t* answer, float* logp);

void transpose_ids(LaunchCtx& cx, const int32_t* src, int32_t* dst, int64_t rows, int T);
void transpose_ids_rounds(LaunchCtx& cx, const int32_t* src, const int32_t* round, int32_t* dst, int64_t B, int R, int K, int T);
void gather_round_rows(LaunchCtx& cx, const float* src, const int32_t* round, float* dst, int64_t B, int R, int H);
void scatter_round_rows(LaunchCtx& cx, const float* src, const int32_t* round, float* dst, int64_t B, int R, int H);
void embed_rows(LaunchCtx& cx, float* out, const float* emb, const int32_t* ids, int64_t rows, int E,
                DropCfg d, uint32_t site);
void embed_scatter_add(LaunchCtx& cx, float* demb, const float* dx, int64_t ldx, const int32_t* ids,
                       int64_t rows, int E, DropCfg d, uint32_t site);

void lstm_pointwise_fwd(LaunchCtx& cx, float* gates, const float* bias, const float* c_prev,
                        const int32_t* mask_ids, float* c_out, float* h_out, int64_t R, int H);
void lstm_first_step_fwd(LaunchCtx& cx, float* gates, const float* ptable, const int32_t* tok, const float* bias,
                         const float* c_prev, const int32_t* mask_ids, float* c_out, float* h_out, int64_t R, int H);
void lstm_pointwise_bwd(LaunchCtx& cx, const float* gates, const float* c_prev, const float* c,
                        const float* dh_rec, const float* dh_ext, const float* dc_ext, float* dc_carry,
                        const int32_t* mask_ids, float* da, int64_t R, int H);

void colsum_add(LaunchCtx& cx, float* out, const float* X, int64_t rows, int cols, int64_t ldx);
void dropout_apply(LaunchCtx& cx, float* out, const float* in, int64_t n, DropCfg d, uint32_t site);
void tanh_bwd(LaunchCtx& cx, float* dpre, const float* dy, const float* y, int64_t n);
void add_inplace(LaunchCtx& cx, float* a, const float* b, int64_t n);
void add_out(LaunchCtx& cx, float* out, const float* a, const float* b, int64_t n);
void copy_cols(LaunchCtx& cx, float* dst, int64_t ldd, const float* src, int64_t lds, int64_t rows, int cols);
void repeat_rows(LaunchCtx& cx, float* dst, const float* src, int64_t B, int R, int64_t cols);
void sum_repeated_rows(LaunchCtx& cx, float* dst, const float* src, int64_t B, int R, int64_t cols);
void transpose_segments(LaunchCtx& cx, const float* W, float* Wt, const int64_t* seg_table_dev, int nseg,
                        int64_t max_elems);
void rowdot_fwd(LaunchCtx& cx, float* out, const float* x, const float* w, const float* b, int64_t rows, int H);
void rowdot_bwd(LaunchCtx& cx, const float* ds, const float* x, const float* w, float* dx, int accumulate_dx,
                float* dw, float* db, int64_t rows, int H);

void mn_attention_fwd(LaunchCtx& cx, const float* q, const float* h, float* probs, float* hAtt, int B, int R, int H);
void mn_attention_bwd(LaunchCtx& cx, const float* q, const float* h, const float* probs, const float* dhAtt,
                      float* dq, float* dh, int B, int R, int H);
void hrea_attention_fwd(LaunchCtx& cx, const float* sq, const float* sh, const float* Hs, float* probs, float* att,
                        int B, int R, int H);
void hrea_attention_bwd(LaunchCtx& cx, const float* sq, const float* sh, const float* Hs, const float* probs,
                        const float* datt, float* dsq, float* dsh, float* dHs, int B, int R, int H);
void masktime_concat_fwd(LaunchCtx& cx, float* out, const float* wemb, const float* img, const int32_t* ids_tm,
                         int T, int64_t N, int E, int I);
void masktime_bwd(LaunchCtx& cx, const float* dx, int64_t ldx, int off, const int32_t* ids_tm, float* dimg,
                  int T, int64_t N, int I);

void san_expand_dropout(LaunchCtx& cx, float* img_tr, const float* t, int B, int R, int P, int H, DropCfg d, uint32_t site);
void san_score_fwd(LaunchCtx& cx, const float* img_common, const float* ques_common, const float* w, const float* b,
                   float* s, int64_t N, int P, int Cm, DropCfg d, uint32_t site);
void san_softmax_att_fwd(LaunchCtx& cx, const float* s, float* p, const float* img_tr, const float* u_in, float* u_out,
                         int64_t N, int P, int H);
void san_att_bwd(LaunchCtx& cx, const float* du, const float* p, const float* img_tr, float* ds, float* dimg_tr,
                 int64_t N, int P, int H);
void san_score_bwd(LaunchCtx& cx, const float* ds, const float* img_common, const float* ques_common, const float* w,
                   float* d_img_common, float* d_ques_common, float* dw, float* db, int64_t N, int P, int Cm,
                   DropCfg d, uint32_t site);
void san_collapse_bwd(LaunchCtx& cx, const float* dimg_tr, const float* t, float* dt_pre, int B, int R, int P, int H,
                      DropCfg d, uint32_t site);

void disc_scores_fwd(LaunchCtx& cx, const float* feat, const float* encOut, float* scores, int64_t N, int K, int H);
void disc_scores_bwd(LaunchCtx& cx, const float* dscores, const float* feat, const float* encOut, float* dfeat,
                     float* dencOut, int64_t N, int K, int H);
void xent_fwd(LaunchCtx& cx, const float* scores, const int32_t* gt, float* row_loss, int64_t N, int K);
void xent_bwd(LaunchCtx& cx, const float* scores, const int32_t* gt, float* dscores, int64_t N, int K);
void soft_xent(LaunchCtx& cx, const float* scores, const float* rel, float* row_loss, float* dscores, int64_t N, int K);
void reduce_sum(LaunchCtx& cx, const float* x, float* out, int64_t n, float scale);
void rank_rows(LaunchCtx& cx, const float* scores, const int32_t* gt, int32_t* ranks, int64_t N, int K);
void logsoftmax_rows(LaunchCtx& cx, float* logits, const int32_t* mask_ids, int64_t rows, int V);
void nll_fwd(LaunchCtx& cx, const float* logp, const int32_t* tgt, const int32_t* mask_ids, float* row_loss, int64_t rows, int V);
void nll_bwd(LaunchCtx& cx, const float* logp, const int32_t* tgt, const int32_t* mask_ids, float* dlogits, int64_t rows, int V);
void lhood_accumulate(LaunchCtx& cx, const float* logits, const int32_t* tgt, const int32_t* mask_ids, float* lh,
                      int64_t rows, int V);

void topk_rows(LaunchCtx& cx, const float* x, int64_t rows, int V, int k, float* topv, int32_t* topi);
void beam_gather(LaunchCtx& cx, float* dst, const float* out_prev, const float* in_prev, const int32_t* parent, int64_t rows, int H);
void logsoftmax_topk_rows(LaunchCtx& cx, const float* logits, const int32_t* mask_ids, int64_t rows, int V, int k, float* topv,
                          int32_t* topi);
void beam_init(LaunchCtx& cx, int64_t rows, int L, int start_token, int32_t* beams, int32_t* tokens, double* scores);
void beam_merge(LaunchCtx& cx, int64_t N, int stp, int k, int L, int end_token, const float* topv, const int32_t* topi,
                const double* scores_in, double* scores_out, const int32_t* beams_in, int32_t* beams_out, int32_t* tokens,
                int32_t* parent, int32_t* ans, int32_t* ans_len, double* ans_score);
void logsoftmax_sample_rows(LaunchCtx& cx, const float* logits, int64_t rows, int V, const SampleCfg& smp, int L, int32_t* tokens,
                            int32_t* answer, float* logp);

void clamp_adam(LaunchCtx& cx, float* W, float* dW, float* m, float* v, int64_t n, float step, float beta1,
                float beta2, float eps, float grad_scale);
void fill_l2_flush(LaunchCtx& cx, float* buf, int64_t n);
void group_rows_by_token(LaunchCtx& cx, const int32_t* ids, int64_t n, int nv, int32_t* scratch3nv, int32_t* perm,
                         int32_t* sorted_tok);
void segsum_rows(LaunchCtx& cx, const float* X, int64_t ldx, const int32_t* perm, const int32_t* sorted_tok, int64_t n,
                 float* out, int ncols);

}

namespace vd {
bool lstm_step_fwd_tc_ok(int H, const float* WtS_h, int64_t ldw);
bool lstm_step_bwd_tc_ok(int H, const float* Wh);
bool lstm_step_fwd_tc(LaunchCtx& cx, int64_t R, int H, const float* h_prev, const float* WtS_h, int64_t ldw, const float* bias,
                      float* gates, int has_xproj, const float* ptable, const int32_t* tok, const float* c_prev, float* c_out,
                      float* h_out, const int32_t* mask_ids, int* tile = nullptr);
bool lstm_step_bwd_tc(LaunchCtx& cx, int64_t R, int H, const float* da_next, const float* Wh, const float* gsave,
                      const float* c_prev, const float* c_cur, const float* dh_ext, float* dc_carry, const int32_t* mask_ids,
                      float* da, int* tile = nullptr);
}

namespace vd {
bool lstm16_shape_ok(int64_t R, int H);
void lstm16_step_fwd(LaunchCtx& cx, int64_t R, int H, const __half* h_prev16, const __half* Wh16, const __half* ptable16,
                     const int32_t* tok, const float* bias, const float* c_prev, const int32_t* mask_ids, __half* gates16,
                     float* c_out, __half* h16_out, float* h32_out);
void lstm16_step_bwd(LaunchCtx& cx, int64_t R, int H, const __half* da_next16, const __half* Whb16, const __half* gates16,
                     const float* c_prev, const float* c_cur, float* dc_carry, const int32_t* mask_ids, __half* da16);
void lstm16_first_step(LaunchCtx& cx, int64_t R, int H, const __half* ptable16, const int32_t* tok, const float* bias,
                       const float* c_prev, const int32_t* mask_ids, __half* gates16, float* c_out, __half* h16_out, float* h32_out);
void lstm16_bwd_last(LaunchCtx& cx, int64_t R, int H, const __half* gates16, const float* c_prev, const float* c_cur,
                     const float* dh_last, const float* scale, const int32_t* mask_ids, float* dc_carry, __half* da16);
void cvt_f32_to_f16(LaunchCtx& cx, __half* dst, int64_t ldd, const float* src, int64_t lds, int64_t rows, int cols);
void pick_grad_scale(LaunchCtx& cx, const float* x, int64_t n, uint32_t* bits, float* scale2);
void segsum_rows16(LaunchCtx& cx, const __half* X, int64_t ldx, const int32_t* perm, const int32_t* sorted_tok, int64_t n,
                   float* out, int ncols, const float* inv_scale);
void gemm_atb16(LaunchCtx& cx, int M, int N, int64_t K, const __half* A, int64_t lda, const __half* B, int64_t ldb, float* C,
                int64_t ldc, const float* inv_scale);
bool enc_pair_shape_ok(int64_t R, int H, int sm_count);
void enc_pair_forward(LaunchCtx& cx, int T, int64_t R, int H, const __half* W1h16, const __half* W2cat16, const float* bias2,
                      const int32_t* mask, float* gates1, float* c1, float* h1, __half* h1_16, float* gates2, float* c2, float* h2,
                      __half* h2_16, int* flags);
void enc_pair_backward(LaunchCtx& cx, int T, int64_t R, int H, const __half* B1cat16, const __half* Whb2_16, const int32_t* mask,
                       const float* gates1, const float* c1, const float* gates2, const float* c2, const float* dh_last1,
                       const float* dc_last1, const float* dh_last2, const float* dc_last2, float* da1, __half* da1_16, float* da2,
                       __half* da2_16, int* flags, float* dh1, float* dh2);
int64_t enc_pair_bwd_flag_ints(int T, int64_t R, int H);
bool enc_pair_gate_split(int H);
}
```

visdial_b200/csrc/lstm16.cu:

```cuda
#include <cuda.h>
#include <cuda_fp16.h>
#include "../../include/visdial_b200.h"
#include "kernels.cuh"
#include "tc_ptx.cuh"

namespace vd {
namespace tc {

constexpr int BM16 = 128;
constexpr int BK16 = 64;
constexpr int UK16 = 16;
constexpr int BN16 = 128;
constexpr int EW16 = 8;
constexpr int STAGE16 = 32768;

__device__ __forceinline__ float tanh16(float x) { float y; asm("tanh.approx.f32 %0, %1;" : "=f"(y) : "f"(x)); return y; }
__device__ __forceinline__ float sig16(float x) { return fmaf(0.5f, tanh16(0.5f * x), 0.5f); }

__device__ __forceinline__ uint32_t pack2(float a, float b) {
  uint32_t r;
  asm("{\n .reg .f16 lo, hi;\n cvt.rn.satfinite.f16.f32 lo, %1;\n cvt.rn.satfinite.f16.f32 hi, %2;\n mov.b32 %0, {lo, hi};\n}"
      : "=r"(r) : "f"(a), "f"(b));
  return r;
}
__device__ __forceinline__ uint4 pack8(const float* v) {
  return make_uint4(pack2(v[0], v[1]), pack2(v[2], v[3]), pack2(v[4], v[5]), pack2(v[6], v[7]));
}
__device__ __forceinline__ void unpack8(const uint4 u, float* v) {
  const __half2* h = reinterpret_cast<const __half2*>(&u);
#pragma unroll
  for (int i = 0; i < 4; ++i) { const float2 f = __half22float2(h[i]); v[2 * i] = f.x; v[2 * i + 1] = f.y; }
}

constexpr int T16_BYTES = 1024, T32_BYTES = 2048;
__device__ __forceinline__ uint8_t* t16_at(uint8_t* base, int row, int unit) {
  return base + row * 64 + (((unit >> 3) ^ ((row >> 1) & 3)) << 4) + (unit & 7) * 2;
}
__device__ __forceinline__ uint8_t* t32_at(uint8_t* base, int row, int unit) {
  return base + row * 128 + (((unit >> 2) ^ (row & 7)) << 4) + (unit & 3) * 4;
}
__device__ __forceinline__ const void* shfl_vptr(const void* p, int src_lane) {
  unsigned long long v = (unsigned long long)p;
  unsigned lo = __shfl_sync(0xffffffffu, (unsigned)v, src_lane), hi = __shfl_sync(0xffffffffu, (unsigned)(v >> 32), src_lane);
  return (const void*)(((unsigned long long)hi << 32) | lo);
}
__device__ __forceinline__ void cp16(void* dst, const void* src) {
  asm volatile("cp.async.cg.shared.global [%0], [%1], 16;" ::"r"(smem_u32(dst)), "l"(src) : "memory");
}
__device__ __forceinline__ void t16_load(uint8_t* base, const void* mine, int lane) {
#pragma unroll
  for (int ps = 0; ps < 2; ++ps) {
    const int row = ps * 8 + (lane >> 2), c = lane & 3;
    const uint8_t* src = (const uint8_t*)shfl_vptr(mine, row);
    uint8_t* dst = base + row * 64 + ((c ^ ((row >> 1) & 3)) << 4);
    if (src) cp16(dst, src + c * 16); else *reinterpret_cast<uint4*>(dst) = make_uint4(0, 0, 0, 0);
  }
}
__device__ __forceinline__ void t32_load(uint8_t* base, const void* mine, int lane) {
#pragma unroll
  for (int ps = 0; ps < 4; ++ps) {
    const int row = ps * 4 + (lane >> 3), c = lane & 7;
    const uint8_t* src = (const uint8_t*)shfl_vptr(mine, row);
    uint8_t* dst = base + row * 128 + ((c ^ (row & 7)) << 4);
    if (src) cp16(dst, src + c * 16); else *reinterpret_cast<float4*>(dst) = make_float4(0.f, 0.f, 0.f, 0.f);
  }
}
__device__ __forceinline__ void cp_wait_all() {
  asm volatile("cp.async.wait_all;" ::: "memory");
  __syncwarp();
}
__device__ __forceinline__ float2 ld_h2(uint8_t* p) { return __half22float2(*reinterpret_cast<const __half2*>(p)); }
__device__ __forceinline__ void st_h2(uint8_t* p, float a, float b) { *reinterpret_cast<uint32_t*>(p) = pack2(a, b); }

struct Lstm16Params {
  int R, H;
  const __half* ptable; const int32_t* tok;
  const float* bias;
  const float* c_prev;
  const int32_t* mask_ids;
  float* h32_out;
  int save_gates;
  const __half* gsave; const float* c_cur; float* dc_carry;
};
struct Lstm16Maps { CUtensorMap g16, c, h16; };

template <int MODE>
struct Cfg16 {
  static constexpr int THREADS = 128 + 32 * EW16;
  static constexpr int STG_PER_WARP = MODE == 0 ? (5 * T16_BYTES + T32_BYTES) : (4 * T16_BYTES + 3 * T32_BYTES);
  static constexpr int STG_BYTES = EW16 * STG_PER_WARP;
  static constexpr int STAGES = (232448 - 1024 - 256 - STG_BYTES) / STAGE16;
  static constexpr int TOTAL = STAGES * STAGE16 + STG_BYTES + 1024 + 256;
};

template <int MODE>
__global__ void __launch_bounds__(Cfg16<MODE>::THREADS, 1)
k_lstm16(const __grid_constant__ CUtensorMap tmA, const __grid_constant__ CUtensorMap tmB,
         const __grid_constant__ Lstm16Maps em, const Lstm16Params p) {
  using C = Cfg16<MODE>;
  constexpr int STAGES = C::STAGES;
  extern __shared__ uint8_t smem_raw[];
  uint8_t* smem = (uint8_t*)(((uintptr_t)smem_raw + 1023) & ~(uintptr_t)1023);
  uint8_t* stg_all = smem + STAGES * STAGE16;
  uint64_t* full = (uint64_t*)(stg_all + C::STG_BYTES);
  uint64_t* empty = full + STAGES;

  const int warp = threadIdx.x >> 5, lane = threadIdx.x & 31;
  const int H = p.H;
  const int num_m = (p.R + BM16 - 1) / BM16;
  const int num_n = MODE == 0 ? H / 32 : H / BN16;
  const int num_tiles = num_m * num_n;
  const int num_kb = (MODE == 0 ? H : 4 * H) / BK16;

  if (threadIdx.x == 0) {
    for (int s = 0; s < STAGES; ++s) { mbar_init(&full[s], 1); mbar_init(&empty[s], 2); }
    asm volatile("fence.mbarrier_init.release.cluster;" ::: "memory");
  }
  __syncthreads();

  if (warp < 4) {
    if (threadIdx.x == 0) {
      int s = 0; uint32_t ph = 0;
      for (int tile = blockIdx.x; tile < num_tiles; tile += gridDim.x) {
        const int m0 = (tile / num_n) * BM16;
        const int nt = tile % num_n;
        for (int kb = 0; kb < num_kb; ++kb) {
          mbar_wait(&empty[s], ph ^ 1);
          uint8_t* sa = smem + s * STAGE16;
          uint8_t* sb = sa + 16384;
          mbar_expect_tx(&full[s], STAGE16);
          tma_load_2d(sa, &tmA, &full[s], kb * BK16, m0);
          if (MODE == 0) {
#pragma unroll
            for (int g = 0; g < 4; ++g) tma_load_2d(sb + g * 4096, &tmB, &full[s], kb * BK16, g * H + nt * 32);
          } else {
            tma_load_2d(sb, &tmB, &full[s], kb * BK16, nt * BN16);
          }
          if (++s == STAGES) { s = 0; ph ^= 1; }
        }
      }
    }
  } else {
    const int cw = warp - 4, wg = cw >> 2;
    uint8_t* stg = stg_all + cw * C::STG_PER_WARP;
    const int fr = lane >> 2, fu = 2 * (lane & 3);
    int s = 0; uint32_t ph = 0;
    auto contract = [&](float (&d)[BN16 / 2]) {
#pragma unroll
      for (int i = 0; i < BN16 / 2; ++i) d[i] = 0.f;
      int prev = -1;
      for (int kb = 0; kb < num_kb; ++kb) {
        mbar_wait(&full[s], ph);
        const uint32_t sa = smem_u32(smem + s * STAGE16);
        const uint64_t adesc = make_desc(sa + wg * 64 * 128, 16, 1024), bdesc = make_desc(sa + 16384, 16, 1024);
        wgmma_fence();
#pragma unroll
        for (int k = 0; k < BK16 / UK16; ++k)
          wgmma_f16_n128(d, adesc + (uint64_t)(k * 2), bdesc + (uint64_t)(k * 2), (kb | k) ? 1u : 0u);
        wgmma_commit();
        wgmma_wait<1>();
        if (prev >= 0 && (threadIdx.x & 127) == 0) mbar_arrive(&empty[prev]);
        prev = s;
        if (++s == STAGES) { s = 0; ph ^= 1; }
      }
      wgmma_wait<0>();
      wgmma_hold(d);
      if (prev >= 0 && (threadIdx.x & 127) == 0) mbar_arrive(&empty[prev]);
    };
    if constexpr (MODE == 0) {
      uint8_t* sG = stg; uint8_t* sH = stg + 4 * T16_BYTES; uint8_t* sC = sH + T16_BYTES;
      for (int tile = blockIdx.x; tile < num_tiles; tile += gridDim.x) {
        const int m0 = (tile / num_n) * BM16;
        const int nt = tile % num_n;
        const int r0 = m0 + wg * 64 + (cw & 3) * 16;
        const int j0 = nt * 32;
        const int64_t row = (int64_t)r0 + (lane & 15);
        const bool row_ok = row < p.R;
        const float keep = (row_ok && p.mask_ids && p.mask_ids[row] == 0) ? 0.f : 1.f;
        const int32_t tk = row_ok ? __ldg(p.tok + row) : 0;
        const __half* prow = tk != 0 ? p.ptable + (int64_t)tk * 4 * H + j0 : nullptr;
        const float* cprow = (row_ok && p.c_prev) ? p.c_prev + row * H + j0 : nullptr;
        if (lane == 0) bulk_wait_read0();
        __syncwarp();
#pragma unroll
        for (int g = 0; g < 4; ++g) t16_load(sG + g * T16_BYTES, prow ? prow + g * H : nullptr, lane);
        t32_load(sC, cprow, lane);
        float d[BN16 / 2];
        contract(d);
        cp_wait_all();
#pragma unroll
        for (int hh = 0; hh < 2; ++hh) {
          const int r = fr + 8 * hh;
          const float kp = __shfl_sync(0xffffffffu, keep, r);
          const int64_t grow = (int64_t)r0 + r;
#pragma unroll
          for (int jj = 0; jj < 4; ++jj) {
            const int u = 8 * jj + fu;
            float a[4][2], cp[2], hn[2];
#pragma unroll
            for (int g = 0; g < 4; ++g) {
              const float2 x = ld_h2(t16_at(sG + g * T16_BYTES, r, u));
              const float2 b = __ldg(reinterpret_cast<const float2*>(p.bias + g * H + j0 + u));
              a[g][0] = d[4 * (jj + 4 * g) + 2 * hh] + (x.x + b.x);
              a[g][1] = d[4 * (jj + 4 * g) + 2 * hh + 1] + (x.y + b.y);
            }
            const float2 c2 = *reinterpret_cast<const float2*>(t32_at(sC, r, u));
            cp[0] = c2.x; cp[1] = c2.y;
#pragma unroll
            for (int e = 0; e < 2; ++e) {
              const float gi = sig16(a[0][e]), gf = sig16(a[1][e]), go = sig16(a[2][e]), gg = tanh16(a[3][e]);
              const float c_ = (gf * cp[e] + gi * gg) * kp;
              a[0][e] = gi * kp; a[1][e] = gf * kp; a[2][e] = go * kp; a[3][e] = gg * kp;
              cp[e] = c_; hn[e] = go * tanh16(c_) * kp;
            }
#pragma unroll
            for (int g = 0; g < 4; ++g) st_h2(t16_at(sG + g * T16_BYTES, r, u), a[g][0], a[g][1]);
            *reinterpret_cast<float2*>(t32_at(sC, r, u)) = make_float2(cp[0], cp[1]);
            st_h2(t16_at(sH, r, u), hn[0], hn[1]);
            if (p.h32_out && grow < p.R)
              *reinterpret_cast<float2*>(p.h32_out + grow * H + j0 + u) = make_float2(hn[0], hn[1]);
          }
        }
        fence_proxy_async_smem();
        __syncwarp();
        if (lane == 0) {
          if (p.save_gates) {
#pragma unroll
            for (int g = 0; g < 4; ++g) tma_store_2d(&em.g16, sG + g * T16_BYTES, g * H + j0, r0);
          }
          tma_store_2d(&em.c, sC, j0, r0);
          tma_store_2d(&em.h16, sH, j0, r0);
          bulk_commit();
        }
        __syncwarp();
      }
    } else {
      uint8_t* sG = stg; uint8_t* sCP = stg + 4 * T16_BYTES; uint8_t* sCC = sCP + T32_BYTES; uint8_t* sDC = sCC + T32_BYTES;
      for (int tile = blockIdx.x; tile < num_tiles; tile += gridDim.x) {
        const int m0 = (tile / num_n) * BM16;
        const int nt = tile % num_n;
        const int r0 = m0 + wg * 64 + (cw & 3) * 16;
        const int64_t row = (int64_t)r0 + (lane & 15);
        const bool row_ok = row < p.R;
        const float keep = (row_ok && p.mask_ids && p.mask_ids[row] == 0) ? 0.f : 1.f;
        const __half* grow = row_ok ? p.gsave + row * 4 * H : nullptr;
        const float* cprow = (row_ok && p.c_prev) ? p.c_prev + row * H : nullptr;
        const float* ccrow = row_ok ? p.c_cur + row * H : nullptr;
        const float* dcrow = row_ok ? p.dc_carry + row * H : nullptr;
        auto fetch = [&](int j) {
          if (lane == 0) bulk_wait_read0();
          __syncwarp();
#pragma unroll
          for (int g = 0; g < 4; ++g) t16_load(sG + g * T16_BYTES, grow ? grow + g * H + j : nullptr, lane);
          t32_load(sCP, cprow ? cprow + j : nullptr, lane);
          t32_load(sCC, ccrow ? ccrow + j : nullptr, lane);
          t32_load(sDC, dcrow ? dcrow + j : nullptr, lane);
        };
        fetch(nt * BN16);
        float d[BN16 / 2];
        contract(d);
#pragma unroll
        for (int grp = 0; grp < BN16 / 32; ++grp) {
          const int j = nt * BN16 + grp * 32;
          if (grp > 0) fetch(j);
          cp_wait_all();
#pragma unroll
          for (int hh = 0; hh < 2; ++hh) {
            const int r = fr + 8 * hh;
            const float keep_r = __shfl_sync(0xffffffffu, keep, r);
#pragma unroll
            for (int jj = 0; jj < 4; ++jj) {
              const int u = 8 * jj + fu;
              float g[4][2], cp[2], cc[2], dc[2], out[4][2], dcn[2];
#pragma unroll
              for (int gg = 0; gg < 4; ++gg) {
                const float2 x = ld_h2(t16_at(sG + gg * T16_BYTES, r, u));
                g[gg][0] = x.x; g[gg][1] = x.y;
              }
              const float2 cp2 = *reinterpret_cast<const float2*>(t32_at(sCP, r, u));
              const float2 cc2 = *reinterpret_cast<const float2*>(t32_at(sCC, r, u));
              const float2 dc2 = *reinterpret_cast<const float2*>(t32_at(sDC, r, u));
              cp[0] = cp2.x; cp[1] = cp2.y; cc[0] = cc2.x; cc[1] = cc2.y; dc[0] = dc2.x; dc[1] = dc2.y;
#pragma unroll
              for (int e = 0; e < 2; ++e) {
                const float dh = d[4 * (4 * grp + jj) + 2 * hh + e];
                const float gi = g[0][e], gf = g[1][e], go = g[2][e], gg_ = g[3][e];
                const float tcv = tanh16(cc[e]);
                const float dd = (dc[e] + dh * go * (1.f - tcv * tcv)) * keep_r;
                const float dhe = dh * keep_r;
                out[0][e] = dd * gg_ * gi * (1.f - gi);
                out[1][e] = dd * cp[e] * gf * (1.f - gf);
                out[2][e] = dhe * tcv * go * (1.f - go);
                out[3][e] = dd * gi * (1.f - gg_ * gg_);
                dcn[e] = dd * gf;
              }
#pragma unroll
              for (int gg = 0; gg < 4; ++gg) st_h2(t16_at(sG + gg * T16_BYTES, r, u), out[gg][0], out[gg][1]);
              *reinterpret_cast<float2*>(t32_at(sDC, r, u)) = make_float2(dcn[0], dcn[1]);
            }
          }
          fence_proxy_async_smem();
          __syncwarp();
          if (lane == 0) {
#pragma unroll
            for (int gg = 0; gg < 4; ++gg) tma_store_2d(&em.g16, sG + gg * T16_BYTES, gg * H + j, r0);
            tma_store_2d(&em.c, sDC, j, r0);
            bulk_commit();
          }
          __syncwarp();
        }
      }
    }
    if (lane == 0) asm volatile("cp.async.bulk.wait_group 0;" ::: "memory");
  }
}

constexpr int A16_KB = 64;
constexpr int A16_BN = 128;
constexpr int A16_THREADS = 384;
constexpr int A16_A_BYTES = 2 * A16_KB * 128;
constexpr int A16_B_BYTES = (A16_BN / 64) * A16_KB * 128;
constexpr int A16_STAGE = A16_A_BYTES + A16_B_BYTES;
constexpr int A16_STAGES = 6;
constexpr int A16_TOTAL = A16_STAGES * A16_STAGE + 1024 + 256;
struct Atb16Params { int M, N; int64_t K, k_per_split; float* C; int64_t ldc; const float* inv_scale; };

__global__ void __launch_bounds__(A16_THREADS, 1)
k_atb16(const __grid_constant__ CUtensorMap tmA, const __grid_constant__ CUtensorMap tmB, const Atb16Params p) {
  extern __shared__ uint8_t smem_raw[];
  uint8_t* smem = (uint8_t*)(((uintptr_t)smem_raw + 1023) & ~(uintptr_t)1023);
  uint64_t* full = (uint64_t*)(smem + A16_STAGES * A16_STAGE);
  uint64_t* empty = full + A16_STAGES;
  const int warp = threadIdx.x >> 5;
  const int num_n = (p.N + A16_BN - 1) / A16_BN;
  const int m0 = (blockIdx.x / num_n) * BM16, n0 = (blockIdx.x % num_n) * A16_BN;
  const int64_t kbeg = (int64_t)blockIdx.y * p.k_per_split;
  const int64_t kend = min(p.K, kbeg + p.k_per_split);
  const int num_kb = (int)((kend - kbeg + A16_KB - 1) / A16_KB);

  if (threadIdx.x == 0) {
    for (int s = 0; s < A16_STAGES; ++s) { mbar_init(&full[s], 1); mbar_init(&empty[s], 2); }
    asm volatile("fence.mbarrier_init.release.cluster;" ::: "memory");
  }
  __syncthreads();

  if (warp < 4) {
    if (threadIdx.x == 0) {
      int s = 0; uint32_t ph = 0;
      for (int kb = 0; kb < num_kb; ++kb) {
        mbar_wait(&empty[s], ph ^ 1);
        uint8_t* sa = smem + s * A16_STAGE;
        uint8_t* sb = sa + A16_A_BYTES;
        mbar_expect_tx(&full[s], A16_STAGE);
        const int krow = (int)(kbeg + (int64_t)kb * A16_KB);
#pragma unroll
        for (int g = 0; g < 2; ++g) tma_load_2d(sa + g * A16_KB * 128, &tmA, &full[s], m0 + g * 64, krow);
#pragma unroll
        for (int g = 0; g < A16_BN / 64; ++g) tma_load_2d(sb + g * A16_KB * 128, &tmB, &full[s], n0 + g * 64, krow);
        if (++s == A16_STAGES) { s = 0; ph ^= 1; }
      }
    }
  } else if (num_kb > 0) {
    const int wg = (warp - 4) >> 2;
    float d[A16_BN / 2];
#pragma unroll
    for (int i = 0; i < A16_BN / 2; ++i) d[i] = 0.f;
    int s = 0; uint32_t ph = 0; int prev = -1;
    for (int kb = 0; kb < num_kb; ++kb) {
      mbar_wait(&full[s], ph);
      const uint32_t sa = smem_u32(smem + s * A16_STAGE);
      const uint32_t sb = sa + A16_A_BYTES;
      wgmma_fence();
#pragma unroll
      for (int k = 0; k < A16_KB / UK16; ++k)
        wgmma_f16_n128_mn(d, make_desc(sa + wg * A16_KB * 128 + k * 2048, A16_KB * 128, 1024),
                          make_desc(sb + k * 2048, A16_KB * 128, 1024), (kb | k) ? 1u : 0u);
      wgmma_commit();
      wgmma_wait<1>();
      if (prev >= 0 && (threadIdx.x & 127) == 0) mbar_arrive(&empty[prev]);
      prev = s;
      if (++s == A16_STAGES) { s = 0; ph ^= 1; }
    }
    wgmma_wait<0>();
    wgmma_hold(d);
    const float sc = p.inv_scale ? __ldg(p.inv_scale) : 1.f;
    const int lane = threadIdx.x & 31, w = warp & 3;
    const int r0 = m0 + wg * 64 + 16 * w + (lane >> 2), c0 = n0 + 2 * (lane & 3);
#pragma unroll
    for (int j = 0; j < A16_BN / 8; ++j) {
#pragma unroll
      for (int h = 0; h < 2; ++h) {
        const int m = r0 + 8 * h, n = c0 + 8 * j;
        if (m < p.M && n < p.N) {
          float* crow = p.C + (int64_t)m * p.ldc + n;
          atomicAdd(crow, d[4 * j + 2 * h] * sc);
          atomicAdd(crow + 1, d[4 * j + 2 * h + 1] * sc);
        }
      }
    }
  }
}

__global__ void __launch_bounds__(256)
k_lstm16_first(const __half* __restrict__ ptable, const int32_t* __restrict__ tok, const float* __restrict__ bias,
               const float* __restrict__ c_prev, const int32_t* __restrict__ mask_ids, __half* __restrict__ gates,
               float* __restrict__ c_out, __half* __restrict__ h16, float* __restrict__ h32, int64_t R, int H) {
  const int64_t idx = (int64_t)blockIdx.x * blockDim.x + threadIdx.x;
  const int H8 = H >> 3;
  if (idx >= R * H8) return;
  const int64_t r = idx / H8;
  const int j = (int)(idx % H8) * 8;
  const float keep = (mask_ids && mask_ids[r] == 0) ? 0.f : 1.f;
  const int32_t tk = tok[r];
  const __half* src = ptable + (int64_t)tk * 4 * H;
  float a[4][8], cp[8], cn[8], hn[8];
#pragma unroll
  for (int g = 0; g < 4; ++g) {
    unpack8(tk != 0 ? __ldg(reinterpret_cast<const uint4*>(src + g * H + j)) : make_uint4(0, 0, 0, 0), a[g]);
    const float4 b0 = __ldg(reinterpret_cast<const float4*>(bias + g * H + j)), b1 = __ldg(reinterpret_cast<const float4*>(bias + g * H + j) + 1);
    a[g][0] += b0.x; a[g][1] += b0.y; a[g][2] += b0.z; a[g][3] += b0.w; a[g][4] += b1.x; a[g][5] += b1.y; a[g][6] += b1.z; a[g][7] += b1.w;
  }
  if (c_prev) {
    const float4 c0 = *reinterpret_cast<const float4*>(c_prev + r * H + j), c1 = *(reinterpret_cast<const float4*>(c_prev + r * H + j) + 1);
    cp[0] = c0.x; cp[1] = c0.y; cp[2] = c0.z; cp[3] = c0.w; cp[4] = c1.x; cp[5] = c1.y; cp[6] = c1.z; cp[7] = c1.w;
  } else {
#pragma unroll
    for (int e = 0; e < 8; ++e) cp[e] = 0.f;
  }
#pragma unroll
  for (int e = 0; e < 8; ++e) {
    const float gi = fsigmoid(a[0][e]), gf = fsigmoid(a[1][e]), go = fsigmoid(a[2][e]), gg = ftanh(a[3][e]);
    const float c_ = gf * cp[e] + gi * gg;
    a[0][e] = gi * keep; a[1][e] = gf * keep; a[2][e] = go * keep; a[3][e] = gg * keep;
    cn[e] = c_ * keep; hn[e] = go * ftanh(c_) * keep;
  }
  if (gates) {
#pragma unroll
    for (int g = 0; g < 4; ++g) __stcs(reinterpret_cast<uint4*>(gates + r * 4 * H + g * H + j), pack8(a[g]));
  }
  float4* co = reinterpret_cast<float4*>(c_out + r * H + j);
  co[0] = make_float4(cn[0], cn[1], cn[2], cn[3]); co[1] = make_float4(cn[4], cn[5], cn[6], cn[7]);
  *reinterpret_cast<uint4*>(h16 + r * H + j) = pack8(hn);
  if (h32) {
    float4* ho = reinterpret_cast<float4*>(h32 + r * H + j);
    ho[0] = make_float4(hn[0], hn[1], hn[2], hn[3]); ho[1] = make_float4(hn[4], hn[5], hn[6], hn[7]);
  }
}

__global__ void __launch_bounds__(256)
k_lstm16_bwd_last(const __half* __restrict__ gates, const float* __restrict__ c_prev, const float* __restrict__ c_cur,
                  const float* __restrict__ dh_last, const float* __restrict__ scale, const int32_t* __restrict__ mask_ids,
                  float* __restrict__ dc_carry, __half* __restrict__ da, int64_t R, int H) {
  const int64_t idx = (int64_t)blockIdx.x * blockDim.x + threadIdx.x;
  const int H8 = H >> 3;
  if (idx >= R * H8) return;
  const int64_t r = idx / H8;
  const int j = (int)(idx % H8) * 8;
  const float keep = (mask_ids && mask_ids[r] == 0) ? 0.f : 1.f;
  const float s = __ldg(scale);
  float g[4][8], cp[8], cc[8], dh[8], out[4][8], dcn[8];
#pragma unroll
  for (int gg = 0; gg < 4; ++gg) unpack8(__ldcs(reinterpret_cast<const uint4*>(gates + r * 4 * H + gg * H + j)), g[gg]);
  auto ld8f = [](const float* p, float* d) {
    const float4 x0 = *reinterpret_cast<const float4*>(p), x1 = *(reinterpret_cast<const float4*>(p) + 1);
    d[0] = x0.x; d[1] = x0.y; d[2] = x0.z; d[3] = x0.w; d[4] = x1.x; d[5] = x1.y; d[6] = x1.z; d[7] = x1.w;
  };
  if (c_prev) ld8f(c_prev + r * H + j, cp);
  else {
#pragma unroll
    for (int e = 0; e < 8; ++e) cp[e] = 0.f;
  }
  ld8f(c_cur + r * H + j, cc);
  ld8f(dh_last + r * H + j, dh);
#pragma unroll
  for (int e = 0; e < 8; ++e) {
    const float gi = g[0][e], gf = g[1][e], go = g[2][e], gg_ = g[3][e];
    const float dhe = dh[e] * s * keep;
    const float tcv = tanh16(cc[e]);
    const float d = dhe * go * (1.f - tcv * tcv);
    out[0][e] = d * gg_ * gi * (1.f - gi);
    out[1][e] = d * cp[e] * gf * (1.f - gf);
    out[2][e] = dhe * tcv * go * (1.f - go);
    out[3][e] = d * gi * (1.f - gg_ * gg_);
    dcn[e] = d * gf;
  }
#pragma unroll
  for (int gg = 0; gg < 4; ++gg) *reinterpret_cast<uint4*>(da + r * 4 * H + gg * H + j) = pack8(out[gg]);
  float4* o = reinterpret_cast<float4*>(dc_carry + r * H + j);
  o[0] = make_float4(dcn[0], dcn[1], dcn[2], dcn[3]); o[1] = make_float4(dcn[4], dcn[5], dcn[6], dcn[7]);
}

__global__ void k_cvt16(__half* __restrict__ dst, int64_t ldd, const float* __restrict__ src, int64_t lds, int64_t rows, int cols) {
  const int64_t idx = (int64_t)blockIdx.x * blockDim.x + threadIdx.x;
  const int c4 = cols >> 2;
  if (idx >= rows * c4) return;
  const int64_t r = idx / c4;
  const int c = (int)(idx % c4) * 4;
  const float4 v = *reinterpret_cast<const float4*>(src + r * lds + c);
  *reinterpret_cast<uint2*>(dst + r * ldd + c) = make_uint2(pack2(v.x, v.y), pack2(v.z, v.w));
}

__global__ void __launch_bounds__(256) k_amax(const float* __restrict__ x, int64_t n4, uint32_t* __restrict__ bits) {
  float m = 0.f;
  for (int64_t i = (int64_t)blockIdx.x * blockDim.x + threadIdx.x; i < n4; i += (int64_t)gridDim.x * blockDim.x) {
    const float4 v = __ldg(reinterpret_cast<const float4*>(x) + i);
    m = fmaxf(m, fmaxf(fmaxf(fabsf(v.x), fabsf(v.y)), fmaxf(fabsf(v.z), fabsf(v.w))));
  }
#pragma unroll
  for (int o = 16; o > 0; o >>= 1) m = fmaxf(m, __shfl_xor_sync(0xffffffffu, m, o));
  if ((threadIdx.x & 31) == 0 && m > 0.f) atomicMax(bits, __float_as_uint(m));
}
__global__ void k_pick_scale(const uint32_t* __restrict__ bits, float* __restrict__ out2) {
  const float amax = __uint_as_float(bits[0]);
  float s = 1.f;
  if (amax > 0.f && isfinite(amax)) {
    int e; frexpf(amax, &e);
    int k = 10 - e;
    k = max(-60, min(60, k));
    s = ldexpf(1.f, k);
  }
  out2[0] = s; out2[1] = 1.f / s;
}

constexpr int SEG16_ROWS = 64;
__global__ void __launch_bounds__(256)
k_segsum16(const __half* __restrict__ X, int64_t ldx, const int32_t* __restrict__ perm, const int32_t* __restrict__ sorted_tok,
           int64_t n, float* __restrict__ out, int ncols, const float* __restrict__ inv_scale) {
  const int64_t p0 = (int64_t)blockIdx.x * SEG16_ROWS, p1 = min(n, p0 + SEG16_ROWS);
  const float sc = inv_scale ? __ldg(inv_scale) : 1.f;
  for (int c0 = threadIdx.x * 8; c0 < ncols; c0 += blockDim.x * 8) {
    float acc[8];
#pragma unroll
    for (int e = 0; e < 8; ++e) acc[e] = 0.f;
    int cur = sorted_tok[p0];
    auto flush = [&](int tok) {
      float* o = out + (int64_t)tok * ncols + c0;
      red_add_v4(o, acc[0] * sc, acc[1] * sc, acc[2] * sc, acc[3] * sc);
      red_add_v4(o + 4, acc[4] * sc, acc[5] * sc, acc[6] * sc, acc[7] * sc);
    };
    for (int64_t p = p0; p < p1; ++p) {
      const int tok = sorted_tok[p];
      if (tok != cur) {
        flush(cur);
#pragma unroll
        for (int e = 0; e < 8; ++e) acc[e] = 0.f;
        cur = tok;
      }
      float v[8];
      unpack8(__ldcs(reinterpret_cast<const uint4*>(X + (int64_t)perm[p] * ldx + c0)), v);
#pragma unroll
      for (int e = 0; e < 8; ++e) acc[e] += v[e];
    }
    flush(cur);
  }
}

static CUtensorMap make_tmap16(const void* base, CUtensorMapDataType dt, int esize, int64_t rows, int64_t cols, int64_t ld,
                               int box_rows, int box_cols, CUtensorMapSwizzle swz) {
  CUtensorMap tm;
  cuuint64_t dims[2] = {(cuuint64_t)cols, (cuuint64_t)rows};
  cuuint64_t strides[1] = {(cuuint64_t)ld * esize};
  cuuint32_t box[2] = {(cuuint32_t)box_cols, (cuuint32_t)box_rows};
  cuuint32_t estr[2] = {1, 1};
  CUresult r = get_encode()(&tm, dt, 2, (void*)base, dims, strides, box, estr, CU_TENSOR_MAP_INTERLEAVE_NONE, swz,
                            CU_TENSOR_MAP_L2_PROMOTION_L2_256B, CU_TENSOR_MAP_FLOAT_OOB_FILL_NONE);
  if (r != CUDA_SUCCESS) {
    char buf[256];
    snprintf(buf, sizeof(buf), "cuTensorMapEncodeTiled (lstm16) failed (%d): base %p rows %lld cols %lld ld %lld box %dx%d", (int)r, base,
             (long long)rows, (long long)cols, (long long)ld, box_rows, box_cols);
    throw CudaError(-3, buf);
  }
  return tm;
}
static CUtensorMap tmap_h(const __half* base, int64_t rows, int64_t cols, int64_t ld, int box_rows, int box_cols,
                          CUtensorMapSwizzle swz) {
  return make_tmap16(base, CU_TENSOR_MAP_DATA_TYPE_FLOAT16, 2, rows, cols, ld, box_rows, box_cols, swz);
}
static CUtensorMap tmap_f(const float* base, int64_t rows, int64_t cols, int64_t ld, int box_rows, int box_cols,
                          CUtensorMapSwizzle swz) {
  return make_tmap16(base, CU_TENSOR_MAP_DATA_TYPE_FLOAT32, 4, rows, cols, ld, box_rows, box_cols, swz);
}

template <int MODE>
static void launch16(LaunchCtx& cx, const CUtensorMap& tA, const CUtensorMap& tB, const Lstm16Maps& em, const Lstm16Params& p,
                     int num_tiles) {
  using C = Cfg16<MODE>;
  static bool attr_set = false;
  if (!attr_set) {
    VD_CUDA_CHECK(cudaFuncSetAttribute(k_lstm16<MODE>, cudaFuncAttributeMaxDynamicSharedMemorySize, C::TOTAL));
    attr_set = true;
  }
  const int pmax = cx.sms();
  int grid = num_tiles;
  if (num_tiles > pmax) { const int rounds = cdiv(num_tiles, pmax); grid = cdiv(num_tiles, rounds); }
  k_lstm16<MODE><<<grid, C::THREADS, C::TOTAL, cx.stream>>>(tA, tB, em, p);
  check_launch(cx, "k_lstm16");
}

}

bool lstm16_shape_ok(int64_t R, int H) { return H % 256 == 0 && H <= 512 && R >= 1024; }

void lstm16_step_fwd(LaunchCtx& cx, int64_t R, int H, const __half* h_prev16, const __half* Wh16, const __half* ptable16,
                     const int32_t* tok, const float* bias, const float* c_prev, const int32_t* mask_ids, __half* gates16,
                     float* c_out, __half* h16_out, float* h32_out) {
  using namespace tc;
  VD_REQUIRE(lstm16_shape_ok(R, H), VD_E_STATE, "lstm16_step_fwd: shape");
  Lstm16Params p = {};
  p.R = (int)R; p.H = H; p.ptable = ptable16; p.tok = tok; p.bias = bias; p.c_prev = c_prev; p.mask_ids = mask_ids;
  p.h32_out = h32_out; p.save_gates = gates16 != nullptr;
  CUtensorMap tA = tmap_h(h_prev16, R, H, H, BM16, BK16, CU_TENSOR_MAP_SWIZZLE_128B);
  CUtensorMap tB = tmap_h(Wh16, 4 * (int64_t)H, H, H, 32, BK16, CU_TENSOR_MAP_SWIZZLE_128B);
  Lstm16Maps em;
  em.g16 = gates16 ? tmap_h(gates16, R, 4 * (int64_t)H, 4 * (int64_t)H, 16, 32, CU_TENSOR_MAP_SWIZZLE_64B)
                   : tmap_h(h16_out, R, H, H, 16, 32, CU_TENSOR_MAP_SWIZZLE_64B);
  em.c = tmap_f(c_out, R, H, H, 16, 32, CU_TENSOR_MAP_SWIZZLE_128B);
  em.h16 = tmap_h(h16_out, R, H, H, 16, 32, CU_TENSOR_MAP_SWIZZLE_64B);
  launch16<0>(cx, tA, tB, em, p, cdiv(R, BM16) * (H / 32));
}

void lstm16_step_bwd(LaunchCtx& cx, int64_t R, int H, const __half* da_next16, const __half* Whb16, const __half* gates16,
                     const float* c_prev, const float* c_cur, float* dc_carry, const int32_t* mask_ids, __half* da16) {
  using namespace tc;
  VD_REQUIRE(lstm16_shape_ok(R, H), VD_E_STATE, "lstm16_step_bwd: shape");
  Lstm16Params p = {};
  p.R = (int)R; p.H = H; p.gsave = gates16; p.c_prev = c_prev; p.c_cur = c_cur; p.dc_carry = dc_carry; p.mask_ids = mask_ids;
  CUtensorMap tA = tmap_h(da_next16, R, 4 * (int64_t)H, 4 * (int64_t)H, BM16, BK16, CU_TENSOR_MAP_SWIZZLE_128B);
  CUtensorMap tB = tmap_h(Whb16, H, 4 * (int64_t)H, 4 * (int64_t)H, 128, BK16, CU_TENSOR_MAP_SWIZZLE_128B);
  Lstm16Maps em;
  em.g16 = tmap_h(da16, R, 4 * (int64_t)H, 4 * (int64_t)H, 16, 32, CU_TENSOR_MAP_SWIZZLE_64B);
  em.c = tmap_f(dc_carry, R, H, H, 16, 32, CU_TENSOR_MAP_SWIZZLE_128B);
  em.h16 = em.c;
  launch16<1>(cx, tA, tB, em, p, cdiv(R, BM16) * (H / BN16));
}

void lstm16_first_step(LaunchCtx& cx, int64_t R, int H, const __half* ptable16, const int32_t* tok, const float* bias,
                       const float* c_prev, const int32_t* mask_ids, __half* gates16, float* c_out, __half* h16_out, float* h32_out) {
  const int64_t n = R * (H / 8);
  tc::k_lstm16_first<<<(unsigned)((n + 255) / 256), 256, 0, cx.stream>>>(ptable16, tok, bias, c_prev, mask_ids, gates16, c_out,
                                                                          h16_out, h32_out, R, H);
  check_launch(cx, "k_lstm16_first");
}

void lstm16_bwd_last(LaunchCtx& cx, int64_t R, int H, const __half* gates16, const float* c_prev, const float* c_cur,
                     const float* dh_last, const float* scale, const int32_t* mask_ids, float* dc_carry, __half* da16) {
  const int64_t n = R * (H / 8);
  tc::k_lstm16_bwd_last<<<(unsigned)((n + 255) / 256), 256, 0, cx.stream>>>(gates16, c_prev, c_cur, dh_last, scale, mask_ids,
                                                                             dc_carry, da16, R, H);
  check_launch(cx, "k_lstm16_bwd_last");
}

void cvt_f32_to_f16(LaunchCtx& cx, __half* dst, int64_t ldd, const float* src, int64_t lds, int64_t rows, int cols) {
  VD_REQUIRE(cols % 4 == 0 && lds % 4 == 0 && ldd % 4 == 0, VD_E_STATE, "cvt_f32_to_f16: alignment");
  const int64_t n = rows * (cols / 4);
  if (n == 0) return;
  tc::k_cvt16<<<(unsigned)((n + 255) / 256), 256, 0, cx.stream>>>(dst, ldd, src, lds, rows, cols);
  check_launch(cx, "k_cvt16");
}

void pick_grad_scale(LaunchCtx& cx, const float* x, int64_t n, uint32_t* bits, float* scale2) {
  VD_REQUIRE(n % 4 == 0, VD_E_STATE, "pick_grad_scale: n % 4");
  VD_CUDA_CHECK(cudaMemsetAsync(bits, 0, sizeof(uint32_t), cx.stream));
  const int blocks = (int)std::min<int64_t>((n / 4 + 255) / 256, 4 * cx.sm_count);
  tc::k_amax<<<blocks, 256, 0, cx.stream>>>(x, n / 4, bits);
  check_launch(cx, "k_amax");
  tc::k_pick_scale<<<1, 1, 0, cx.stream>>>(bits, scale2);
  check_launch(cx, "k_pick_scale");
}

void segsum_rows16(LaunchCtx& cx, const __half* X, int64_t ldx, const int32_t* perm, const int32_t* sorted_tok, int64_t n,
                   float* out, int ncols, const float* inv_scale) {
  VD_REQUIRE(ncols % 8 == 0 && ldx % 8 == 0, VD_E_STATE, "segsum_rows16: alignment");
  if (n == 0) return;
  tc::k_segsum16<<<(unsigned)((n + tc::SEG16_ROWS - 1) / tc::SEG16_ROWS), 256, 0, cx.stream>>>(X, ldx, perm, sorted_tok, n, out, ncols,
                                                                                               inv_scale);
  check_launch(cx, "k_segsum16");
}

void gemm_atb16(LaunchCtx& cx, int M, int N, int64_t K, const __half* A, int64_t lda, const __half* B, int64_t ldb, float* C,
                int64_t ldc, const float* inv_scale) {
  using namespace tc;
  VD_REQUIRE(M % 64 == 0 && N % 64 == 0 && K >= A16_KB && lda % 8 == 0 && ldb % 8 == 0, VD_E_STATE, "gemm_atb16: shape");
  const int tiles = cdiv(M, BM16) * cdiv(N, A16_BN);
  const int64_t cta_cap = cx.sm_budget > 0 ? cx.sm_budget : 2LL * cx.sm_count;
  int64_t splits = std::max<int64_t>(1, std::min<int64_t>(cta_cap / tiles, K / (A16_KB * 4)));
  int64_t kps = ((K + splits - 1) / splits + A16_KB - 1) / A16_KB * A16_KB;
  splits = (K + kps - 1) / kps;
  Atb16Params p = {M, N, K, kps, C, ldc, inv_scale};
  CUtensorMap tA = tmap_h(A, K, M, lda, A16_KB, 64, CU_TENSOR_MAP_SWIZZLE_128B),
              tB = tmap_h(B, K, N, ldb, A16_KB, 64, CU_TENSOR_MAP_SWIZZLE_128B);
  static bool attr_set = false;
  if (!attr_set) {
    VD_CUDA_CHECK(cudaFuncSetAttribute(k_atb16, cudaFuncAttributeMaxDynamicSharedMemorySize, A16_TOTAL));
    attr_set = true;
  }
  dim3 grid(tiles, (unsigned)splits);
  k_atb16<<<grid, A16_THREADS, A16_TOTAL, cx.stream>>>(tA, tB, p);
  check_launch(cx, "k_atb16");
}

}
```

Baseline: 12610.

## Widen encoder LSTM row tile to 192 and add dynamic tile queue for lstm16

The persistent encoder LSTM kernels now use 192-row blocks with three consumer warpgroups instead of two. Registers are rebalanced with setmaxnreg between the producer and consumer roles, and the TMA pipeline drops from 5 to 3 stages to fit shared memory. Separately, the f16 option-LSTM kernel switches from static strided tile assignment to an atomic work queue. The producer hands each tile index to consumers through shared memory, and the last CTA to finish resets the counters. The intent is better reuse of the weight slice per row block and better load balance, at the cost of a shallower pipeline, fewer row blocks to spread across groups, and global atomics whose shared counters could conflict if launches run concurrently.

```diff
diff --git a/include/visdial_b200.h b/include/visdial_b200.h
--- a/include/visdial_b200.h
+++ b/include/visdial_b200.h
@@ -132,6 +132,7 @@
 int vd_launch_count(vd_engine* e, int64_t* n_launches);
 int vd_kernel_stats(vd_engine* e, const char* name, int64_t* launches, double* total_ms,
                     double* total_flops, double* total_bytes);
+int vd_enc_pair_geometry(int64_t rows, int32_t hidden, int32_t sm_count, int32_t* row_blocks, int32_t* groups);
 int vd_gemm_tn(vd_engine* e, int32_t M, int32_t N, int32_t K, const float* A, int64_t lda, const float* B, int64_t ldb,
                float* C, int64_t ldc, float beta, const float* bias, int32_t act);
 int vd_gemm_atb(vd_engine* e, int32_t M, int32_t N, int64_t K, const float* A, int64_t lda, const float* B, int64_t ldb,
diff --git a/visdial_b200/_lib.py b/visdial_b200/_lib.py
--- a/visdial_b200/_lib.py
+++ b/visdial_b200/_lib.py
@@ -108,6 +108,7 @@
     "vd_profile_reset": [_H],
     "vd_launch_count": [_H, _P(C.c_int64)],
     "vd_kernel_stats": [_H, C.c_char_p, _P(C.c_int64), _P(C.c_double), _P(C.c_double), _P(C.c_double)],
+    "vd_enc_pair_geometry": [C.c_int64, C.c_int32, C.c_int32, _P(C.c_int32), _P(C.c_int32)],
     "vd_gemm_tn": [_H, C.c_int32, C.c_int32, C.c_int32, C.c_void_p, C.c_int64, C.c_void_p, C.c_int64, C.c_void_p,
                    C.c_int64, C.c_float, C.c_void_p, C.c_int32],
     "vd_gemm_atb": [_H, C.c_int32, C.c_int32, C.c_int64, C.c_void_p, C.c_int64, C.c_void_p, C.c_int64, C.c_void_p,
diff --git a/visdial_b200/csrc/api.cu b/visdial_b200/csrc/api.cu
--- a/visdial_b200/csrc/api.cu
+++ b/visdial_b200/csrc/api.cu
@@ -329,6 +329,17 @@
   VD_TRY({ Engine* e = ENG(h); e->cx.collect(); e->cx.stats.clear(); e->cx.launches = 0; })
 }
 int vd_launch_count(vd_engine* h, int64_t* n) { VD_TRY({ NOTNULL(n); *n = ENG(h)->cx.launches; }) }
+int vd_enc_pair_geometry(int64_t rows, int32_t hidden, int32_t sm_count, int32_t* row_blocks, int32_t* groups) {
+  VD_TRY({
+    NOTNULL(row_blocks); NOTNULL(groups);
+    VD_REQUIRE(rows > 0 && hidden > 0 && sm_count > 0 && vd::enc_pair_shape_ok(rows, hidden, sm_count), VD_E_BADARG,
+               "vd_enc_pair_geometry: shape the persistent encoder kernels do not take");
+    int rb = 0;
+    int g = 0;
+    vd::enc_pair_geometry(rows, hidden, sm_count, &rb, &g);
+    *row_blocks = rb; *groups = g;
+  })
+}
 int vd_kernel_stats(vd_engine* h, const char* name, int64_t* launches, double* total_ms, double* total_flops,
                     double* total_bytes) {
   VD_TRY({
diff --git a/visdial_b200/csrc/common.cuh b/visdial_b200/csrc/common.cuh
--- a/visdial_b200/csrc/common.cuh
+++ b/visdial_b200/csrc/common.cuh
@@ -109,6 +109,7 @@
   int sm_count = 132;
   int sm_budget = 0;
   int sms() const { return sm_budget > 0 ? sm_budget : sm_count; }
+  int* tile_counters = nullptr;
   std::map<std::string, KStat> stats;
   std::vector<cudaEvent_t> free_events;
 
diff --git a/visdial_b200/csrc/enc_lstm.cu b/visdial_b200/csrc/enc_lstm.cu
--- a/visdial_b200/csrc/enc_lstm.cu
+++ b/visdial_b200/csrc/enc_lstm.cu
@@ -7,14 +7,23 @@
 namespace vd {
 namespace tc {
 
-constexpr int EP_THREADS = 288;
-constexpr int EP_STAGES = 5;
-constexpr int EP_STAGE_BYTES = 128 * 64 * 2;
+constexpr int EP_BM = 192;
+constexpr int EP_CWG = EP_BM / 64;
+constexpr int EP_CONSUMERS = 128 * EP_CWG;
+constexpr int EP_THREADS = EP_CONSUMERS + 128;
+constexpr int EP_REG_CONSUMER = 160, EP_REG_PRODUCER = 32;
+constexpr int EP_STAGES = 3;
+constexpr int EP_STAGE_BYTES = EP_BM * 64 * 2;
 constexpr int EP_W_BYTES_MAX = 131072;
-constexpr int EP_ACC_BYTES = 32 * ACC_LD * 4;
+constexpr int EP_ACC_LD = EP_BM + 4;
+constexpr int EP_ACC_BYTES = 32 * EP_ACC_LD * 4;
 constexpr int EP_SMEM = EP_W_BYTES_MAX + EP_STAGES * EP_STAGE_BYTES + EP_ACC_BYTES + 1024 + 256;
 constexpr int EP_HS = 32;
 static_assert(EP_SMEM <= 227 * 1024, "persistent encoder LSTM: shared memory budget");
+static_assert(EP_CWG * EP_REG_CONSUMER + EP_REG_PRODUCER <= 512 && EP_THREADS * 128 <= 65536, "persistent encoder LSTM: registers");
+
+template <int R> __device__ __forceinline__ void ep_setmaxnreg_inc() { asm volatile("setmaxnreg.inc.sync.aligned.u32 %0;" ::"n"(R)); }
+template <int R> __device__ __forceinline__ void ep_setmaxnreg_dec() { asm volatile("setmaxnreg.dec.sync.aligned.u32 %0;" ::"n"(R)); }
 
 __device__ __forceinline__ uint32_t ep_pack2(float a, float b) {
   uint32_t r;
@@ -83,7 +92,7 @@
     wbar = empty + EP_STAGES;
   }
   __device__ void init_barriers() {
-    for (int s = 0; s < EP_STAGES; ++s) { mbar_init(&full[s], 1); mbar_init(&empty[s], 2); }
+    for (int s = 0; s < EP_STAGES; ++s) { mbar_init(&full[s], 1); mbar_init(&empty[s], EP_CWG); }
     mbar_init(wbar, 1);
     asm volatile("fence.mbarrier_init.release.cluster;" ::: "memory");
   }
@@ -127,18 +136,18 @@
 #pragma unroll
   for (int jj = 0; jj < 4; ++jj) {
     const int j = 4 * C + jj;
-    float* p = acc + (c + 8 * jj) * ACC_LD + r;
-    p[0] = d[4 * j]; p[ACC_LD] = d[4 * j + 1]; p[8] = d[4 * j + 2]; p[ACC_LD + 8] = d[4 * j + 3];
+    float* p = acc + (c + 8 * jj) * EP_ACC_LD + r;
+    p[0] = d[4 * j]; p[EP_ACC_LD] = d[4 * j + 1]; p[8] = d[4 * j + 2]; p[EP_ACC_LD + 8] = d[4 * j + 3];
   }
   bar_named(2 + wg, 128);
 }
 __device__ __forceinline__ void ep_ld16(const float* arow, float* v) {
 #pragma unroll
-  for (int e = 0; e < EP_HW; ++e) v[e] = arow[e * ACC_LD];
+  for (int e = 0; e < EP_HW; ++e) v[e] = arow[e * EP_ACC_LD];
 }
 
 __device__ __forceinline__ void ep_publish(int* flag) {
-  bar_named(1, 256);
+  bar_named(1, EP_CONSUMERS);
   if (threadIdx.x == 0) asm volatile("red.release.gpu.global.add.s32 [%0], 1;" ::"l"(flag) : "memory");
 }
 
@@ -162,8 +171,9 @@
   if (threadIdx.x == 0) sm.init_barriers();
   __syncthreads();
 
-  if (warp == 8) {
-    if (lane == 0) {
+  if (warp >= 4 * EP_CWG) {
+    ep_setmaxnreg_dec<EP_REG_PRODUCER>();
+    if (threadIdx.x == EP_CONSUMERS) {
       const CUtensorMap* tw = role == EP_CELL1 ? &tmW1 : &tmW2;
       const int kofs = role == EP_CELL2 ? H : 0;
       mbar_expect_tx(sm.wbar, (uint32_t)(KB * N * 128));
@@ -183,23 +193,24 @@
             int kr = kb + koff; if (kr >= KB) kr -= KB;
             mbar_wait(&sm.empty[s], ph ^ 1);
             mbar_expect_tx(&sm.full[s], EP_STAGE_BYTES);
-            tma_load_2d(sm.stages + s * EP_STAGE_BYTES, tm, &sm.full[s], kr * 64, ts * p.R + rb * 128);
+            tma_load_2d(sm.stages + s * EP_STAGE_BYTES, tm, &sm.full[s], kr * 64, ts * p.R + rb * EP_BM);
             if (++s == EP_STAGES) { s = 0; ph ^= 1; }
           }
         }
       }
     }
-  } else if (warp < 8) {
+  } else {
+    ep_setmaxnreg_inc<EP_REG_CONSUMER>();
     const int wg = warp >> 2;
     const int hh = (warp >> 1) & 1;
     const int rloc = wg * 64 + (warp & 1) * 32 + lane;
-    const float* arow = sm.acc + hh * EP_HW * ACC_LD + rloc;
+    const float* arow = sm.acc + hh * EP_HW * EP_ACC_LD + rloc;
     const int u0 = slice * HS + hh * EP_HW;
     mbar_wait(sm.wbar, 0);
     int s = 0; uint32_t ph = 0;
     if (role == EP_PROJ) {
       for (int rb = group; rb < p.RB; rb += p.groups) {
-        const int64_t row = (int64_t)rb * 128 + rloc;
+        const int64_t row = (int64_t)rb * EP_BM + rloc;
         const bool row_ok = row < p.R;
         for (int t = 0; t < T; ++t) {
           const int64_t tr = (int64_t)t * p.R + row;
@@ -228,7 +239,7 @@
       __half* h16 = l1 ? p.h1_16 : p.h2_16;
       int* flag = l1 ? flagL1 : flagL2;
       for (int rb = group; rb < p.RB; rb += p.groups) {
-        const int64_t row = (int64_t)rb * 128 + rloc;
+        const int64_t row = (int64_t)rb * EP_BM + rloc;
         const bool row_ok = row < p.R;
         float c[EP_HW];
         zero16(c);
@@ -325,8 +336,9 @@
   if (threadIdx.x == 0) sm.init_barriers();
   __syncthreads();
 
-  if (warp == 8) {
-    if (lane == 0) {
+  if (warp >= 4 * EP_CWG) {
+    ep_setmaxnreg_dec<EP_REG_PRODUCER>();
+    if (threadIdx.x == EP_CONSUMERS) {
       const CUtensorMap* tw = role == EP_CELL1 ? &tmW2 : &tmW1;
       const int kofs = role == EP_CELL2 ? 4 * H : 0;
       mbar_expect_tx(sm.wbar, (uint32_t)(KB * N * 128));
@@ -346,17 +358,18 @@
             int kr = kb + koff; if (kr >= KB) kr -= KB;
             mbar_wait(&sm.empty[s], ph ^ 1);
             mbar_expect_tx(&sm.full[s], EP_STAGE_BYTES);
-            tma_load_2d(sm.stages + s * EP_STAGE_BYTES, tm, &sm.full[s], (GS ? gq * H : 0) + kr * 64, ts * p.R + rb * 128);
+            tma_load_2d(sm.stages + s * EP_STAGE_BYTES, tm, &sm.full[s], (GS ? gq * H : 0) + kr * 64, ts * p.R + rb * EP_BM);
             if (++s == EP_STAGES) { s = 0; ph ^= 1; }
           }
         }
       }
     }
-  } else if (warp < 8) {
+  } else {
+    ep_setmaxnreg_inc<EP_REG_CONSUMER>();
     const int wg = warp >> 2;
     const int hh = (warp >> 1) & 1;
     const int rloc = wg * 64 + (warp & 1) * 32 + lane;
-    const float* arow = sm.acc + hh * EP_HW * ACC_LD + rloc;
+    const float* arow = sm.acc + hh * EP_HW * EP_ACC_LD + rloc;
     const int u0 = j0 + hh * EP_HW;
     mbar_wait(sm.wbar, 0);
     int s = 0; uint32_t ph = 0;
@@ -372,12 +385,12 @@
           for (int e = 0; e < EP_HW; e += 4) red_add_v4(dst + e, a[e], a[e + 1], a[e + 2], a[e + 3]);
         }
       }
-      bar_named(1, 256);
+      bar_named(1, EP_CONSUMERS);
       if (threadIdx.x == 0) asm volatile("red.release.gpu.global.add.s32 [%0], 1;" ::"l"(cnt + ((size_t)rb * T + t) * nU + us) : "memory");
     };
     if (role == EP_PROJ) {
       for (int rb = group; rb < p.RB; rb += p.groups) {
-        const int64_t row = (int64_t)rb * 128 + rloc;
+        const int64_t row = (int64_t)rb * EP_BM + rloc;
         const bool row_ok = row < p.R;
         for (int t = T - 1; t >= 0; --t) {
           const int64_t tr = (int64_t)t * p.R + row;
@@ -404,7 +417,7 @@
       float* dhbuf = top ? p.dh2 : p.dh1;
       int* cnt = top ? cntT : cntB;
       for (int rb = group; rb < p.RB; rb += p.groups) {
-        const int64_t row = (int64_t)rb * 128 + rloc;
+        const int64_t row = (int64_t)rb * EP_BM + rloc;
         const bool row_ok = row < p.R;
         float dc[EP_HW];
         zero16(dc);
@@ -490,8 +503,15 @@
 
 }
 
+int64_t enc_pair_fwd_flag_ints(int T, int64_t R) { return 3 * (int64_t)cdiv(R, tc::EP_BM) * T; }
+
 bool enc_pair_shape_ok(int64_t R, int H, int sm_count) {
   return H % 64 == 0 && H <= 512 && R >= 64 && 3 * (H / 32) <= sm_count;
+}
+
+void enc_pair_geometry(int64_t R, int H, int sm_count, int* row_blocks, int* groups) {
+  *row_blocks = cdiv(R, tc::EP_BM);
+  *groups = std::max(1, std::min(*row_blocks, sm_count / (3 * (H / 32))));
 }
 
 void enc_pair_forward(LaunchCtx& cx, int T, int64_t R, int H, const __half* W1h16, const __half* W2cat16, const float* bias2,
@@ -500,15 +520,15 @@
   using namespace tc;
   VD_REQUIRE(enc_pair_shape_ok(R, H, cx.sm_count), VD_E_STATE, "enc_pair_forward: shape");
   EncFwdParams p = {};
-  p.T = T; p.R = (int)R; p.H = H; p.RB = cdiv(R, 128);
+  p.T = T; p.R = (int)R; p.H = H;
   p.nS = H / 32;
-  p.groups = std::max(1, std::min(p.RB, cx.sm_count / (3 * p.nS)));
+  enc_pair_geometry(R, H, cx.sm_count, &p.RB, &p.groups);
   p.gates1 = gates1; p.c1 = c1; p.h1 = h1; p.h1_16 = h1_16;
   p.gates2 = gates2; p.c2 = c2; p.h2 = h2; p.h2_16 = h2_16;
   p.bias2 = bias2; p.mask = mask; p.flags = flags;
-  VD_CUDA_CHECK(cudaMemsetAsync(flags, 0, (size_t)3 * p.RB * T * sizeof(int), cx.stream));
+  VD_CUDA_CHECK(cudaMemsetAsync(flags, 0, (size_t)enc_pair_fwd_flag_ints(T, R) * sizeof(int), cx.stream));
   const int64_t TR = (int64_t)T * R;
-  CUtensorMap tH1 = ep_tmap_h(h1_16, TR, H, H, 128), tH2 = ep_tmap_h(h2_16, TR, H, H, 128);
+  CUtensorMap tH1 = ep_tmap_h(h1_16, TR, H, H, EP_BM), tH2 = ep_tmap_h(h2_16, TR, H, H, EP_BM);
   CUtensorMap tW1 = ep_tmap_h(W1h16, 4 * (int64_t)H, H, H, EP_HS), tW2 = ep_tmap_h(W2cat16, 4 * (int64_t)H, 2 * (int64_t)H, 2 * (int64_t)H, EP_HS);
   static bool attr_set = false;
   if (!attr_set) {
@@ -520,7 +540,7 @@
 }
 
 
-int64_t enc_pair_bwd_flag_ints(int T, int64_t R, int H) { return (int64_t)cdiv(R, 128) * T * (3 + 2 * std::max(1, H / 128)); }
+int64_t enc_pair_bwd_flag_ints(int T, int64_t R, int H) { return (int64_t)cdiv(R, tc::EP_BM) * T * (3 + 2 * std::max(1, H / 128)); }
 bool enc_pair_gate_split(int H) { return H % 128 == 0; }
 void enc_pair_backward(LaunchCtx& cx, int T, int64_t R, int H, const __half* B1cat16, const __half* Whb2_16, const int32_t* mask,
                        const float* gates1, const float* c1, const float* gates2, const float* c2, const float* dh_last1,
@@ -530,9 +550,9 @@
   VD_REQUIRE(enc_pair_shape_ok(R, H, cx.sm_count), VD_E_STATE, "enc_pair_backward: shape");
   const bool gs = dh1 && dh2 && enc_pair_gate_split(H);
   EncBwdParams p = {};
-  p.T = T; p.R = (int)R; p.H = H; p.RB = cdiv(R, 128);
+  p.T = T; p.R = (int)R; p.H = H;
   p.nS = H / 32;
-  p.groups = std::max(1, std::min(p.RB, cx.sm_count / (3 * p.nS)));
+  enc_pair_geometry(R, H, cx.sm_count, &p.RB, &p.groups);
   p.gates1 = gates1; p.c1 = c1; p.da1 = da1; p.da1_16 = da1_16;
   p.gates2 = gates2; p.c2 = c2; p.da2 = da2; p.da2_16 = da2_16;
   p.dh_last1 = dh_last1; p.dc_last1 = dc_last1; p.dh_last2 = dh_last2; p.dc_last2 = dc_last2;
@@ -544,7 +564,7 @@
     VD_CUDA_CHECK(cudaMemsetAsync(dh1, 0, (size_t)TR * H * sizeof(float), cx.stream));
     VD_CUDA_CHECK(cudaMemsetAsync(dh2, 0, (size_t)TR * H * sizeof(float), cx.stream));
   }
-  CUtensorMap tA1 = ep_tmap_h(da1_16, TR, G, G, 128), tA2 = ep_tmap_h(da2_16, TR, G, G, 128);
+  CUtensorMap tA1 = ep_tmap_h(da1_16, TR, G, G, EP_BM), tA2 = ep_tmap_h(da2_16, TR, G, G, EP_BM);
   const int wbox = gs ? 128 : EP_HS;
   CUtensorMap tW1 = ep_tmap_h(B1cat16, H, 2 * G, 2 * G, wbox), tW2 = ep_tmap_h(Whb2_16, H, G, G, wbox);
   static bool attr_set = false;
diff --git a/visdial_b200/csrc/engine.cu b/visdial_b200/csrc/engine.cu
--- a/visdial_b200/csrc/engine.cu
+++ b/visdial_b200/csrc/engine.cu
@@ -203,7 +203,7 @@
     for (auto ev : ev_img_free) cudaEventDestroy(ev);
   }
   for (auto& g : stage_img) g.release();
-  cudaFree(W); cudaFree(dW); cudaFree(m); cudaFree(v); cudaFree(Wt); cudaFree(scalars_dev); cudaFree(segtab_dev);
+  cudaFree(W); cudaFree(dW); cudaFree(m); cudaFree(v); cudaFree(Wt); cudaFree(scalars_dev); cudaFree(segtab_dev); cudaFree(cx.tile_counters);
   if (flush_buf) cudaFree(flush_buf);
   cx.collect();
   for (auto e : cx.free_events) cudaEventDestroy(e);
@@ -502,7 +502,7 @@
     __half* W2c = arena.get<__half>((int64_t)G * 2 * H);
     cvt_f32_to_f16(cx, W1h, H, Wtp(l1.wseg) + l1.D, l1.D + H, G, H);
     cvt_f32_to_f16(cx, W2c, 2 * H, Wtp(l2.wseg), 2 * H, G, 2 * H);
-    int* flags = arena.get<int>(3 * (int64_t)cdiv(R, 128) * T);
+    int* flags = arena.get<int>(enc_pair_fwd_flag_ints(T, R));
     LaunchCtx::Scope sc2(&cx, "enc_pair_fwd", 2.0 * T * R * G * 3.0 * H, 4.0 * T * R * (2.0 * G + 2.0 * G + 6.0 * H));
     enc_pair_forward(cx, T, R, H, W1h, W2c, Wp(l2.wseg + 1), l1.mask, l1.gates, l1.c, l1.h, l1.h16, l2.gates, l2.c, l2.h, l2.h16, flags);
     return;
diff --git a/visdial_b200/csrc/kernels.cuh b/visdial_b200/csrc/kernels.cuh
--- a/visdial_b200/csrc/kernels.cuh
+++ b/visdial_b200/csrc/kernels.cuh
@@ -147,6 +147,7 @@
 void gemm_atb16(LaunchCtx& cx, int M, int N, int64_t K, const __half* A, int64_t lda, const __half* B, int64_t ldb, float* C,
                 int64_t ldc, const float* inv_scale);
 bool enc_pair_shape_ok(int64_t R, int H, int sm_count);
+void enc_pair_geometry(int64_t R, int H, int sm_count, int* row_blocks, int* groups);
 void enc_pair_forward(LaunchCtx& cx, int T, int64_t R, int H, const __half* W1h16, const __half* W2cat16, const float* bias2,
                       const int32_t* mask, float* gates1, float* c1, float* h1, __half* h1_16, float* gates2, float* c2, float* h2,
                       __half* h2_16, int* flags);
@@ -154,6 +155,7 @@
                        const float* gates1, const float* c1, const float* gates2, const float* c2, const float* dh_last1,
                        const float* dc_last1, const float* dh_last2, const float* dc_last2, float* da1, __half* da1_16, float* da2,
                        __half* da2_16, int* flags, float* dh1, float* dh2);
+int64_t enc_pair_fwd_flag_ints(int T, int64_t R);
 int64_t enc_pair_bwd_flag_ints(int T, int64_t R, int H);
 bool enc_pair_gate_split(int H);
 }
diff --git a/visdial_b200/csrc/lstm16.cu b/visdial_b200/csrc/lstm16.cu
--- a/visdial_b200/csrc/lstm16.cu
+++ b/visdial_b200/csrc/lstm16.cu
@@ -81,6 +81,7 @@
   float* h32_out;
   int save_gates;
   const __half* gsave; const float* c_cur; float* dc_carry;
+  int* queue;
 };
 struct Lstm16Maps { CUtensorMap g16, c, h16; };
 
@@ -104,6 +105,7 @@
   uint8_t* stg_all = smem + STAGES * STAGE16;
   uint64_t* full = (uint64_t*)(stg_all + C::STG_BYTES);
   uint64_t* empty = full + STAGES;
+  int* tile_of = (int*)(empty + STAGES);
 
   const int warp = threadIdx.x >> 5, lane = threadIdx.x & 31;
   const int H = p.H;
@@ -121,13 +123,23 @@
   if (warp < 4) {
     if (threadIdx.x == 0) {
       int s = 0; uint32_t ph = 0;
-      for (int tile = blockIdx.x; tile < num_tiles; tile += gridDim.x) {
+      for (;;) {
+        const int tile = atomicAdd(p.queue, 1);
+        if (tile >= num_tiles) {
+          mbar_wait(&empty[s], ph ^ 1);
+          tile_of[s] = -1;
+          mbar_arrive(&full[s]);
+          __threadfence();
+          if (atomicAdd(p.queue + 1, 1) == (int)gridDim.x - 1) { atomicExch(p.queue, 0); atomicExch(p.queue + 1, 0); }
+          break;
+        }
         const int m0 = (tile / num_n) * BM16;
         const int nt = tile % num_n;
         for (int kb = 0; kb < num_kb; ++kb) {
           mbar_wait(&empty[s], ph ^ 1);
           uint8_t* sa = smem + s * STAGE16;
           uint8_t* sb = sa + 16384;
+          if (kb == 0) tile_of[s] = tile;
           mbar_expect_tx(&full[s], STAGE16);
           tma_load_2d(sa, &tmA, &full[s], kb * BK16, m0);
           if (MODE == 0) {
@@ -145,6 +157,7 @@
     uint8_t* stg = stg_all + cw * C::STG_PER_WARP;
     const int fr = lane >> 2, fu = 2 * (lane & 3);
     int s = 0; uint32_t ph = 0;
+    auto next_tile = [&]() { mbar_wait(&full[s], ph); return tile_of[s]; };
     auto contract = [&](float (&d)[BN16 / 2]) {
 #pragma unroll
       for (int i = 0; i < BN16 / 2; ++i) d[i] = 0.f;
@@ -169,7 +182,7 @@
     };
     if constexpr (MODE == 0) {
       uint8_t* sG = stg; uint8_t* sH = stg + 4 * T16_BYTES; uint8_t* sC = sH + T16_BYTES;
-      for (int tile = blockIdx.x; tile < num_tiles; tile += gridDim.x) {
+      for (int n = 0, tile = next_tile(); n < num_tiles && tile >= 0; ++n, tile = next_tile()) {
         const int m0 = (tile / num_n) * BM16;
         const int nt = tile % num_n;
         const int r0 = m0 + wg * 64 + (cw & 3) * 16;
@@ -236,7 +249,7 @@
       }
     } else {
       uint8_t* sG = stg; uint8_t* sCP = stg + 4 * T16_BYTES; uint8_t* sCC = sCP + T32_BYTES; uint8_t* sDC = sCC + T32_BYTES;
-      for (int tile = blockIdx.x; tile < num_tiles; tile += gridDim.x) {
+      for (int n = 0, tile = next_tile(); n < num_tiles && tile >= 0; ++n, tile = next_tile()) {
         const int m0 = (tile / num_n) * BM16;
         const int nt = tile % num_n;
         const int r0 = m0 + wg * 64 + (cw & 3) * 16;
@@ -582,7 +595,7 @@
 }
 
 template <int MODE>
-static void launch16(LaunchCtx& cx, const CUtensorMap& tA, const CUtensorMap& tB, const Lstm16Maps& em, const Lstm16Params& p,
+static void launch16(LaunchCtx& cx, const CUtensorMap& tA, const CUtensorMap& tB, const Lstm16Maps& em, Lstm16Params p,
                      int num_tiles) {
   using C = Cfg16<MODE>;
   static bool attr_set = false;
@@ -590,6 +603,12 @@
     VD_CUDA_CHECK(cudaFuncSetAttribute(k_lstm16<MODE>, cudaFuncAttributeMaxDynamicSharedMemorySize, C::TOTAL));
     attr_set = true;
   }
+  if (!cx.tile_counters) {
+    VD_CUDA_CHECK(cudaMalloc((void**)&cx.tile_counters, 4 * sizeof(int)));
+    VD_CUDA_CHECK(cudaMemsetAsync(cx.tile_counters, 0, 4 * sizeof(int), cx.stream));
+    VD_CUDA_CHECK(cudaStreamSynchronize(cx.stream));
+  }
+  p.queue = cx.tile_counters + 2 * MODE;
   const int pmax = cx.sms();
   int grid = num_tiles;
   if (num_tiles > pmax) { const int rounds = cdiv(num_tiles, pmax); grid = cdiv(num_tiles, rounds); }
```

Result: faster. 12830, median of 6 (+1.7%).
